# buctcurry/ICKA

Hardware: AMD Instinct MI355X
Metric: MNER samples/sec (fwd+bwd) at seq=128, 36 regions, bs=32 per GPU (higher is better)
Workload: dtype bf16; 1 GPU; c2: bert(H768,L12,h12,I3072)+36x2048 regions, seq_len 128, per-GPU batch 32, 1 cross layer(s), gated head, 13 labels, train mode p=0.1, token-CE loss; global_batch=32, seq_len=128, regions=36, parallelism=dp1, launch=hipgraph, precision=bf16, accumulate=1

## Files before the change

### icka_amd/_lib.py

```python
from __future__ import annotations

import ctypes as C
import os
from typing import Optional

_HERE = os.path.dirname(os.path.abspath(__file__))
LIB_PATH = os.path.join(_HERE, "libicka_hip.so")

c_vp, c_i32, c_i64, c_u64, c_f32 = C.c_void_p, C.c_int32, C.c_int64, C.c_uint64, C.c_float

ABI_VERSION = 6
GEMM_NT, GEMM_NN, GEMM_TN, GEMM_TT = 0, 1, 2, 3
ATTN_FP8, ATTN_TILED = 1, 2
LSTM_PER_STEP, LSTM_TICKETS, LSTM_NO_BATCH_SPLIT = 1, 2, 4
EPI_NONE, EPI_GELU, EPI_DGELU, EPI_ADD, EPI_GATE, EPI_TANH, EPI_RELU, EPI_ADD_RELU = 0, 1, 2, 3, 4, 5, 6, 7


class GemmDesc(C.Structure):
    _fields_ = [
        ("op", c_i32), ("M", c_i32), ("N", c_i32), ("K", c_i32), ("K1", c_i32),
        ("A", c_vp), ("lda", c_i64), ("B", c_vp), ("ldb", c_i64),
        ("A2", c_vp), ("lda2", c_i64), ("B2", c_vp), ("ldb2", c_i64),
        ("C", c_vp), ("ldc", c_i64), ("c_is_f32", c_i32),
        ("C2", c_vp), ("ldc2", c_i64),
        ("aux", c_vp), ("ldaux", c_i64),
        ("bias", c_vp), ("bias2", c_vp),
        ("alpha", c_f32), ("beta", c_f32),
        ("epilogue", c_i32),
        ("colsum_out", c_vp), ("colsum_accumulate", c_i32),
        ("ab_f16", c_i32), ("C3", c_vp), ("ldc3", c_i64), ("aux_f16", c_i32), ("c3_only", c_i32),
        ("tune", c_u64),
    ]


class SlabReduction(C.Structure):
    _fields_ = [("partials", c_vp), ("slab_stride", c_i64), ("nslab", c_i32), ("H", c_i32), ("nslots", c_i32),
                ("accumulate", c_i32), ("out", c_vp * 4)]


class XGemmDesc(C.Structure):
    _fields_ = [
        ("op", c_i32), ("M", c_i32), ("N", c_i32), ("K", c_i32),
        ("A", c_vp), ("lda", c_i64), ("a_bs0", c_i64), ("a_bs1", c_i64),
        ("B", c_vp), ("ldb", c_i64), ("b_bs0", c_i64), ("b_bs1", c_i64),
        ("C", c_vp), ("ldc", c_i64), ("c_bs0", c_i64), ("c_bs1", c_i64),
        ("nb0", c_i32), ("nb1", c_i32),
        ("bias", c_vp),
        ("alpha", c_f32), ("beta", c_f32),
    ]


PROTOTYPES = {
    "icka_abi_version": (c_i32, []),
    "icka_copy_many": (c_i32, [c_vp, c_vp, c_vp, c_i32, c_vp]),
    "icka_build_arch": (C.c_char_p, []),
    "icka_gemm": (c_i32, [C.POINTER(GemmDesc), c_vp]),
    "icka_gemm_grouped": (c_i32, [C.POINTER(GemmDesc), c_i32, c_vp]),
    "icka_gemm_grouped_ex": (c_i32, [C.POINTER(GemmDesc), c_i32, C.POINTER(SlabReduction), c_i32, c_vp]),
    "icka_gemm_ln": (c_i32, [C.POINTER(GemmDesc), c_vp, c_vp, c_i64, c_i32, c_vp, c_vp, c_vp, c_i64, c_vp, c_i32, c_vp, c_vp, c_f32,
                             c_f32, c_u64, c_vp, c_vp, c_vp]),
    "icka_gemm_qkv_attn": (c_i32, [C.POINTER(GemmDesc), c_vp, c_vp, c_vp, c_i64, c_vp, c_i32, c_i32, c_i32, c_f32, c_f32, c_u64, c_vp, c_vp]),
    "icka_gemm_ln_sync_words": (c_i64, []),
    "icka_gemm_ln_test_hooks": (c_i32, [c_i32, c_i32]),
    "icka_ln_fwd": (c_i32, [c_vp, c_i64, c_i32, c_vp, c_vp, c_i64, c_i32, c_vp, c_vp, c_vp, c_i64, c_vp, c_i64,
                            c_vp, c_vp, c_vp, c_i32, c_i32, c_f32, c_f32, c_u64, c_vp]),
    "icka_ln_fwd_h": (c_i32, [c_vp, c_i64, c_i32, c_vp, c_vp, c_i64, c_i32, c_vp, c_vp, c_vp, c_i64, c_vp, c_i64,
                            c_vp, c_vp, c_vp, c_i32, c_i32, c_f32, c_f32, c_u64, c_vp]),
    "icka_ln_bwd_workspace_floats": (c_i64, [c_i32]),
    "icka_ln_bwd": (c_i32, [c_vp, c_i64, c_vp, c_i64, c_vp, c_vp, c_vp, c_vp, c_i64, c_vp, c_i64, c_vp, c_vp, c_vp,
                            c_vp, c_i32, c_i32, c_f32, c_u64, c_i32, c_vp]),
    "icka_ln_bwd_slabs": (c_i32, [c_vp, c_i64, c_vp, c_i64, c_vp, c_vp, c_vp, c_vp, c_i64, c_vp, c_i64, c_vp, c_i32,
                                  c_i32, c_f32, c_u64, c_vp]),
    "icka_ln_bwd_nslab": (c_i32, [c_i32]),
    "icka_ln_slab_slots": (c_i32, []),
    "icka_embed_fwd": (c_i32, [c_vp, c_vp, c_vp, c_vp, c_vp, c_vp, c_vp, c_vp, c_vp, c_vp, c_vp, c_i32, c_i32,
                               c_i32, c_i32, c_i32, c_f32, c_f32, c_u64, c_vp]),
    "icka_embed_fwd_h": (c_i32, [c_vp, c_vp, c_vp, c_vp, c_vp, c_vp, c_vp, c_vp, c_vp, c_vp, c_vp, c_i32, c_i32,
                               c_i32, c_i32, c_i32, c_f32, c_f32, c_u64, c_vp]),
    "icka_embed_bwd": (c_i32, [c_vp, c_vp, c_vp, c_vp, c_vp, c_vp, c_vp, c_vp, c_vp, c_vp, c_vp, c_vp, c_i32, c_i32,
                               c_i32, c_i32, c_i32, c_i32, c_f32, c_u64, c_i32, c_vp]),
    "icka_embed_bwd_rows": (c_i32, [c_vp, c_vp, c_vp, c_vp, c_vp, c_vp, c_vp, c_vp, c_vp, c_vp, c_vp, c_vp, c_i32, c_i32,
                                    c_i32, c_i32, c_i32, c_i32, c_f32, c_u64, c_i32, c_vp]),
    "icka_embed_scatter_rows": (c_i32, [c_vp, c_i32, c_vp, c_vp, c_i64, c_i32, c_i32, c_i32, c_f32, c_vp]),
    "icka_attn_fwd": (c_i32, [c_vp, c_i64, c_vp, c_i64, c_vp, c_i64, c_vp, c_vp, c_i64, c_vp, c_i32, c_i32, c_i32,
                              c_i32, c_f32, c_f32, c_u64, c_vp]),
    "icka_attn_fwd_ex": (c_i32, [c_vp, c_i64, c_vp, c_i64, c_vp, c_i64, c_vp, c_vp, c_vp, c_i64, c_vp, c_i32, c_i32, c_i32,
                                 c_i32, c_f32, c_f32, c_u64, c_i32, c_vp, c_vp]),
    "icka_attn_keepbits_words": (c_i64, [c_i32, c_i32, c_i32, c_i32]),
    "icka_attn_fwd_fp8": (c_i32, [c_vp, c_i64, c_vp, c_i64, c_vp, c_i64, c_vp, c_vp, c_i64, c_vp, c_i32, c_i32, c_i32,
                              c_i32, c_f32, c_f32, c_u64, c_vp]),
    "icka_cls_head_fwd": (c_i32, [c_vp, c_vp, c_vp, c_vp, c_vp, c_i32, c_i32, c_i32, c_vp]),
    "icka_cls_head_fwd_h": (c_i32, [c_vp, c_vp, c_vp, c_vp, c_vp, c_i32, c_i32, c_i32, c_vp]),
    "icka_cls_head_bwd": (c_i32, [c_vp, c_i64, c_vp, c_vp, c_vp, c_vp, c_vp, c_vp, c_vp, c_vp, c_vp, c_i32, c_i32, c_i32,
                                  c_vp]),
    "icka_cls_head_bwd_slabs": (c_i32, [c_i32]),
    "icka_cls_head_slab_floats": (c_i64, [c_i32, c_i32]),
    "icka_conv_stem_patches": (c_i32, [c_vp, c_vp, c_i32, c_i32, c_i32, c_i64, c_vp]),
    "icka_conv_im2col3x3": (c_i32, [c_vp, c_vp, c_i32, c_i32, c_i32, c_i32, c_i32, c_i64, c_vp]),
    "icka_conv3x3_gemm": (c_i32, [c_vp, c_vp, c_vp, c_vp, c_i64, c_vp, c_i32, c_i32, c_i32, c_i32, c_i32, c_i32, c_i64, c_i32,
                                   c_vp, c_vp]),
    "icka_conv_subsample": (c_i32, [c_vp, c_vp, c_i32, c_i32, c_i32, c_i32, c_i32, c_i64, c_vp]),
    "icka_conv_maxpool3x3s2": (c_i32, [c_vp, c_vp, c_i32, c_i32, c_i32, c_i32, c_i64, c_vp]),
    "icka_conv_features_out": (c_i32, [c_vp, c_vp, c_vp, c_vp, c_i32, c_i32, c_i32, c_vp]),
    "icka_gemm_bn_stats": (c_i32, [c_vp, c_i64, c_vp, c_i64, c_vp, c_i64, c_i32, c_i32, c_i32, c_i64, c_vp, c_vp]),
    "icka_conv3x3_gemm_stats": (c_i32, [c_vp, c_vp, c_vp, c_i32, c_i32, c_i32, c_i32, c_i32, c_i32, c_i64, c_vp, c_vp, c_vp]),
    "icka_bn_finalize": (c_i32, [c_vp, c_i32, c_i32, c_vp, c_vp, c_vp, c_vp, c_vp, c_f32, c_f32, c_vp, c_vp, c_vp]),
    "icka_bn_apply": (c_i32, [c_vp, c_vp, c_vp, c_vp, c_vp, c_vp, c_vp, c_i32, c_i64, c_i64, c_i32, c_vp, c_vp, c_vp]),
    "icka_lstm_fwd": (c_i32, [c_vp, c_i64, c_vp, c_vp, c_vp, c_vp, c_vp, c_i32, c_i32, c_i32, c_i32, c_vp]),
    "icka_lstm_bwd": (c_i32, [c_vp, c_vp, c_vp, c_vp, c_vp, c_i64, c_vp, c_i32, c_i32, c_i32, c_i32, c_vp]),
    "icka_lstm_barrier_error": (c_i32, []),
    "icka_lstm_clear_error": (c_i32, []),
    "icka_lstm_set_reserved_cus": (c_i32, [c_i32]),
    "icka_lstm_test_hooks": (c_i32, [c_i32, c_i32]),
    "icka_linear_small_m": (c_i32, [c_vp, c_i64, c_vp, c_vp, c_vp, c_i64, c_i32, c_i32, c_i32, c_i32, c_vp]),
    "icka_transpose_bf16": (c_i32, [c_vp, c_vp, c_i32, c_i32, c_i32, c_vp]),
    "icka_crf_llh": (c_i32, [c_vp, c_i64, c_vp, c_vp, c_vp, c_vp, c_vp, c_vp, c_i32, c_i32, c_i32, c_vp]),
    "icka_crf_grad": (c_i32, [c_vp, c_i64, c_vp, c_vp, c_vp, c_vp, c_vp, c_vp, c_vp, c_i64, c_vp, c_vp, c_vp, c_i32,
                              c_i32, c_i32, c_vp]),
    "icka_crf_decode": (c_i32, [c_vp, c_i64, c_vp, c_vp, c_vp, c_vp, c_vp, c_vp, c_i32, c_i32, c_i32, c_vp]),
    "icka_crf_score_decode": (c_i32, [c_vp, c_i64, c_vp, c_vp, c_vp, c_vp, c_vp, c_vp, c_vp, c_vp, c_i64, c_i32, c_i32, c_i32,
                                      c_vp]),
    "icka_attn_bwd": (c_i32, [c_vp, c_i64, c_vp, c_i64, c_vp, c_i64, c_vp, c_vp, c_i64, c_vp, c_i64, c_vp, c_vp,
                              c_vp, c_i64, c_vp, c_i64, c_vp, c_i64, c_i32, c_i32, c_i32, c_i32, c_f32, c_f32, c_u64,
                              c_vp, c_i32, c_vp]),
    "icka_cast_f32_to_bf16": (c_i32, [c_vp, c_vp, c_i64, c_vp]),
    "icka_cast_to_f16": (c_i32, [c_vp, c_i32, c_vp, c_i64, c_vp]),
    "icka_cast_f32_to_bf16_f16": (c_i32, [c_vp, c_vp, c_vp, c_i64, c_vp]),
    "icka_cast_bf16_to_f32": (c_i32, [c_vp, c_vp, c_i64, c_vp]),
    "icka_cast_pad_f32_to_bf16": (c_i32, [c_vp, c_i64, c_vp, c_i64, c_i32, c_i32, c_vp]),
    "icka_additive_mask": (c_i32, [c_vp, c_i64, c_vp, c_i32, c_i32, c_vp]),
    "icka_dropout": (c_i32, [c_vp, c_i64, c_vp, c_i64, c_vp, c_i64, c_i32, c_i32, c_f32, c_u64, c_vp]),
    "icka_regions_to_tokens": (c_i32, [c_vp, c_vp, c_i32, c_i32, c_i32, c_i32, c_vp]),
    "icka_regions_to_tokens_h": (c_i32, [c_vp, c_vp, c_vp, c_i32, c_i32, c_i32, c_i32, c_vp]),
    "icka_sample_gate_fwd_h": (c_i32, [c_vp, c_i64, c_vp, c_i32, c_vp, c_vp, c_i64, c_i32, c_i32, c_i32, c_vp]),
    "icka_colsum": (c_i32, [c_vp, c_i64, c_vp, c_vp, c_i32, c_i32, c_i32, c_vp]),
    "icka_colsum_workspace_floats": (c_i64, [c_i32]),
    "icka_gate_bwd": (c_i32, [c_vp, c_i64, c_vp, c_vp, c_i64, c_vp, c_i64, c_vp, c_vp, c_i64, c_i32, c_i32, c_vp]),
    "icka_sample_gate_fwd": (c_i32, [c_vp, c_i64, c_vp, c_i64, c_vp, c_i32, c_vp, c_i64, c_i32, c_i32, c_i32, c_vp]),
    "icka_sample_gate_bwd": (c_i32, [c_vp, c_i64, c_vp, c_i64, c_vp, c_i64, c_vp, c_i32, c_vp, c_i64, c_vp, c_i64, c_vp,
                                     c_i32, c_i32, c_i32, c_vp]),
    "icka_crs_fwd": (c_i32, [c_vp, c_i64, c_vp, c_i64, c_vp, c_vp, c_vp, c_i32, c_i32, c_i32, c_vp]),
    "icka_crs_bwd": (c_i32, [c_vp, c_vp, c_i64, c_vp, c_i64, c_vp, c_vp, c_vp, c_vp, c_vp, c_i32, c_i32, c_i32, c_i32,
                             c_vp]),
    "icka_add_bf16": (c_i32, [c_vp, c_vp, c_vp, c_i64, c_vp]),
    "icka_tanh_bwd": (c_i32, [c_vp, c_vp, c_vp, c_i64, c_vp]),
    "icka_contrastive_workspace_floats": (c_i64, [c_i32]),
    "icka_contrastive_fwd": (c_i32, [c_vp, c_i64, c_vp, c_i64, c_i32, c_i32, c_i32, c_f32, c_f32, c_vp, c_i32, c_vp, c_vp, c_vp]),
    "icka_contrastive_bwd": (c_i32, [c_vp, c_i64, c_vp, c_i64, c_i32, c_i32, c_i32, c_f32, c_f32, c_vp, c_vp, c_vp, c_vp, c_vp,
                                     c_vp, c_i32, c_vp, c_vp]),
    "icka_relu_bwd": (c_i32, [c_vp, c_vp, c_vp, c_i64, c_i32, c_vp]),
    "icka_sample_swap": (c_i32, [c_vp, c_vp, c_i32, c_i64, c_i32, c_vp]),
    "icka_dgelu_bf16": (c_i32, [c_vp, c_vp, c_vp, c_i64, c_vp]),
    "icka_embed_prompt_fwd": (c_i32, [c_vp, c_vp, c_vp, c_vp, c_vp, c_vp, c_vp, c_vp, c_vp, c_vp, c_vp, c_vp, c_i32, c_i32,
                                      c_i32, c_i32, c_i32, c_i32, c_i32, c_f32, c_f32, c_u64, c_vp]),
    "icka_embed_prompt_bwd": (c_i32, [c_vp, c_vp, c_vp, c_vp, c_vp, c_vp, c_vp, c_vp, c_vp, c_vp, c_vp, c_vp, c_vp, c_i32,
                                      c_i32, c_i32, c_i32, c_i32, c_i32, c_i32, c_i32, c_f32, c_u64, c_i32, c_vp]),
    "icka_token_ce": (c_i32, [c_vp, c_i64, c_vp, c_vp, c_vp, c_vp, c_vp, c_i64, c_i32, c_i32, c_vp]),
    "icka_token_ce_workspace_floats": (c_i64, [c_i32]),
    "icka_token_ce_fused": (c_i32, [c_vp, c_i64, c_vp, c_vp, c_vp, c_vp, c_vp, c_i64, c_i32, c_i32, c_i32, c_vp]),
    "icka_zero_f32": (c_i32, [c_vp, c_i64, c_vp]),
    "icka_scale_by_ratio": (c_i32, [c_vp, c_vp, c_vp, c_vp, c_i64, c_vp]),
    "icka_scalar_ratio": (c_i32, [c_vp, c_vp, c_vp, c_vp]),
    "icka_set_dropout_nonce": (c_i32, [c_vp]),
    "icka_bump_dropout_nonce": (c_i32, [c_vp, c_vp]),
    "icka_dropout_mask": (c_i32, [c_vp, c_i64, c_f32, c_u64, c_vp]),
    "icka_attn_dropout_mask": (c_i32, [c_vp, c_i64, c_i32, c_f32, c_u64, c_vp]),
    "icka_pack_plan": (c_i32, [c_vp, c_i32, c_i32, c_i32, c_vp, c_vp, c_vp, c_vp, c_vp, c_vp, c_vp, c_vp]),
    "icka_rows_gather": (c_i32, [c_vp, c_i64, c_i64, c_vp, c_i64, c_i64, c_i32, c_vp, c_i64, C.c_uint32, c_vp]),
    "icka_attn_fwd_packed": (c_i32, [c_vp, c_i64, c_vp, c_i64, c_vp, c_i64, c_vp, c_vp, c_i64, c_vp, c_vp, c_i32, c_i64, c_i32,
                                     c_i32, c_i32, c_i32, c_f32, c_f32, c_u64, c_vp, c_vp]),
    "icka_attn_bwd_packed": (c_i32, [c_vp, c_i64, c_vp, c_i64, c_vp, c_i64, c_vp, c_vp, c_i64, c_vp, c_vp, c_vp, c_i64, c_vp,
                                     c_i64, c_vp, c_i64, c_vp, c_i32, c_i64, c_i32, c_i32, c_i32, c_i32, c_f32, c_f32, c_u64,
                                     c_vp, c_vp]),
    "icka_dp_chunk_elems": (c_i64, []),
    "icka_dp_cast_chunks": (c_i32, [c_vp, c_vp, c_vp, c_i32, c_vp]),
    "icka_dp_cast_back_scaled": (c_i32, [c_vp, c_vp, c_i64, c_f32, c_vp]),
    "icka_dp_init": (c_i32, []),
    "icka_dp_error": (c_i32, []),
    "icka_dp_clear_error": (c_i32, []),
    "icka_dp_step_bump": (c_i32, [c_vp, c_vp]),
    "icka_dp_flag_set": (c_i32, [c_vp, c_vp, c_vp]),
    "icka_dp_flag_wait": (c_i32, [c_vp, C.c_uint32, c_vp, c_i32, c_vp]),
    "icka_dp_poison_if": (c_i32, [c_vp, C.c_uint32, c_vp, c_i32, c_i32, c_vp]),
    "icka_dp_poison_final": (c_i32, [c_vp, c_i32, C.c_uint32, c_vp, c_vp, c_i32, c_vp]),
    "icka_optim_chunk_elems": (c_i64, []),
    "icka_optim_sqnorm": (c_i32, [c_vp, c_vp, c_i32, c_vp, c_vp]),
    "icka_optim_clip": (c_i32, [c_vp, c_i32, c_f32, c_vp, c_vp]),
    "icka_optim_adamw": (c_i32, [c_vp, c_vp, c_vp, c_vp, c_vp, c_vp, c_vp, c_i32, c_vp, c_f32, c_f32, c_f32, c_f32, c_f32,
                                 c_i32, c_vp]),
    "icka_x_gemm": (c_i32, [C.POINTER(XGemmDesc), c_vp]),
    "icka_x_ln_fwd": (c_i32, [c_vp, c_i64, c_vp, c_i64, c_vp, c_vp, c_vp, c_vp, c_vp, c_i32, c_i32, c_f32, c_f32, c_u64,
                              c_vp]),
    "icka_x_ln_bwd": (c_i32, [c_vp, c_i64, c_vp, c_vp, c_vp, c_vp, c_vp, c_i32, c_i32, c_f32, c_u64, c_vp]),
    "icka_x_colsum": (c_i32, [c_vp, c_i64, c_vp, c_i64, c_vp, c_i32, c_i32, c_i32, c_vp]),
    "icka_x_embed_fwd": (c_i32, [c_vp, c_vp, c_vp, c_vp, c_vp, c_vp, c_vp, c_vp, c_vp, c_vp, c_i32, c_i32, c_i32, c_f32,
                                 c_vp]),
    "icka_x_embed_scatter": (c_i32, [c_vp, c_vp, c_vp, c_vp, c_vp, c_vp, c_i32, c_i32, c_i32, c_i32, c_vp]),
    "icka_x_softmax_fwd": (c_i32, [c_vp, c_vp, c_vp, c_i32, c_i32, c_i32, c_i32, c_f32, c_f32, c_u64, c_vp]),
    "icka_x_softmax_bwd": (c_i32, [c_vp, c_vp, c_i32, c_i32, c_i32, c_i32, c_f32, c_f32, c_u64, c_vp]),
    "icka_x_act_fwd": (c_i32, [c_vp, c_vp, c_vp, c_vp, c_i64, c_i32, c_vp]),
    "icka_x_act_bwd": (c_i32, [c_vp, c_vp, c_vp, c_vp, c_vp, c_i64, c_i32, c_vp]),
    "icka_x_dropout": (c_i32, [c_vp, c_vp, c_i64, c_f32, c_u64, c_vp]),
    "icka_x_add": (c_i32, [c_vp, c_i64, c_vp, c_i64, c_vp, c_i64, c_i32, c_i32, c_vp]),
    "icka_x_concat2": (c_i32, [c_vp, c_i64, c_i32, c_vp, c_i64, c_i32, c_vp, c_i32, c_vp]),
    "icka_x_regions_to_tokens": (c_i32, [c_vp, c_vp, c_i32, c_i32, c_i32, c_i32, c_vp]),
    "icka_x_sample_gate_fwd": (c_i32, [c_vp, c_i64, c_vp, c_i64, c_vp, c_i32, c_vp, c_i64, c_i32, c_i32, c_i32, c_vp]),
    "icka_x_sample_gate_bwd": (c_i32, [c_vp, c_i64, c_vp, c_i64, c_vp, c_i64, c_vp, c_i32, c_vp, c_i64, c_vp, c_i64, c_vp,
                                       c_i32, c_i32, c_i32, c_vp]),
    "icka_x_lstm_cell_fwd": (c_i32, [c_vp, c_vp, c_vp, c_vp, c_i32, c_i32, c_i32, c_i32, c_vp]),
    "icka_x_lstm_cell_bwd": (c_i32, [c_vp, c_vp, c_vp, c_vp, c_vp, c_i32, c_i32, c_i32, c_i32, c_i32, c_vp]),
    "icka_x_embed_prompt_fwd": (c_i32, [c_vp, c_vp, c_vp, c_vp, c_vp, c_vp, c_vp, c_vp, c_vp, c_vp, c_vp, c_i32, c_i32, c_i32,
                                        c_i32, c_i32, c_i32, c_f32, c_vp]),
    "icka_x_embed_prompt_scatter": (c_i32, [c_vp, c_vp, c_vp, c_vp, c_vp, c_vp, c_vp, c_i32, c_i32, c_i32, c_i32, c_i32, c_i32,
                                            c_i32, c_vp]),
# ... 40 lines not shown
```

### icka_amd/csrc/elementwise.hip

```cpp
#include <math.h>

#include "common.h"

namespace {

inline bool al16(const void* p) { return (reinterpret_cast<uintptr_t>(p) & 15) == 0; }
inline int grid_for(int64_t n, int per_block = 256, int cap = 4096) {
    int64_t g = (n + per_block - 1) / per_block;
    return (int)(g < 1 ? 1 : (g > cap ? cap : g));
}

__device__ __forceinline__ void ld8(const bf16_t* p, float (&o)[8]) {
    const bf16x8 v = as_bf16x8(*reinterpret_cast<const u32x4*>(p));
#pragma unroll
    for (int e = 0; e < 8; ++e) o[e] = bf2f(v[e]);
}
__device__ __forceinline__ void st8(bf16_t* p, const float (&v)[8]) {
    bf16x8 o;
#pragma unroll
    for (int e = 0; e < 8; ++e) o[e] = f2bf(v[e]);
    *reinterpret_cast<u32x4*>(p) = as_u32x4(o);
}

__global__ void cast_f2b_kernel(const float* __restrict__ src, bf16_t* __restrict__ dst, int64_t n) {
    const int64_t nch = n >> 3;
    for (int64_t c = (int64_t)blockIdx.x * blockDim.x + threadIdx.x; c < nch; c += (int64_t)gridDim.x * blockDim.x) {
        const f32x4 a = *reinterpret_cast<const f32x4*>(src + c * 8), b = *reinterpret_cast<const f32x4*>(src + c * 8 + 4);
        bf16x8 o = {f2bf(a[0]), f2bf(a[1]), f2bf(a[2]), f2bf(a[3]), f2bf(b[0]), f2bf(b[1]), f2bf(b[2]), f2bf(b[3])};
        *reinterpret_cast<u32x4*>(dst + c * 8) = as_u32x4(o);
    }
    if (blockIdx.x == 0 && threadIdx.x < (n & 7)) dst[(nch << 3) + threadIdx.x] = f2bf(src[(nch << 3) + threadIdx.x]);
}
__global__ void cast_f2bh_kernel(const float* __restrict__ src, bf16_t* __restrict__ dst, _Float16* __restrict__ dsth, int64_t n) {
    const int64_t nch = n >> 3;
    for (int64_t c = (int64_t)blockIdx.x * blockDim.x + threadIdx.x; c < nch; c += (int64_t)gridDim.x * blockDim.x) {
        const f32x4 a = *reinterpret_cast<const f32x4*>(src + c * 8), b = *reinterpret_cast<const f32x4*>(src + c * 8 + 4);
        bf16x8 o = {f2bf(a[0]), f2bf(a[1]), f2bf(a[2]), f2bf(a[3]), f2bf(b[0]), f2bf(b[1]), f2bf(b[2]), f2bf(b[3])};
        *reinterpret_cast<u32x4*>(dst + c * 8) = as_u32x4(o);
        f16x8 h;
#pragma unroll
        for (int e = 0; e < 4; ++e) {
            h[e] = (_Float16)fminf(fmaxf(a[e], -65504.f), 65504.f);
            h[4 + e] = (_Float16)fminf(fmaxf(b[e], -65504.f), 65504.f);
        }
        *reinterpret_cast<u32x4*>(dsth + c * 8) = __builtin_bit_cast(u32x4, h);
    }
    if (blockIdx.x == 0 && threadIdx.x < (n & 7)) {
        const float v = src[(nch << 3) + threadIdx.x];
        dst[(nch << 3) + threadIdx.x] = f2bf(v);
        dsth[(nch << 3) + threadIdx.x] = (_Float16)fminf(fmaxf(v, -65504.f), 65504.f);
    }
}
__global__ void cast_to_f16_kernel(const void* __restrict__ src, int kind, _Float16* __restrict__ dst, int64_t n) {
    for (int64_t i = (int64_t)blockIdx.x * blockDim.x + threadIdx.x; i < n; i += (int64_t)gridDim.x * blockDim.x) {
        const float v = kind ? reinterpret_cast<const float*>(src)[i] : bf2f(reinterpret_cast<const bf16_t*>(src)[i]);
        dst[i] = (_Float16)fminf(fmaxf(v, -65504.f), 65504.f);
    }
}
__global__ void cast_b2f_vec_kernel(const bf16_t* __restrict__ src, float* __restrict__ dst, int64_t n) {
    const int64_t nch = n >> 3;
    for (int64_t c = (int64_t)blockIdx.x * blockDim.x + threadIdx.x; c < nch; c += (int64_t)gridDim.x * blockDim.x) {
        const bf16x8 v = as_bf16x8(*reinterpret_cast<const u32x4*>(src + c * 8));
        *reinterpret_cast<f32x4*>(dst + c * 8) = f32x4{bf2f(v[0]), bf2f(v[1]), bf2f(v[2]), bf2f(v[3])};
        *reinterpret_cast<f32x4*>(dst + c * 8 + 4) = f32x4{bf2f(v[4]), bf2f(v[5]), bf2f(v[6]), bf2f(v[7])};
    }
    if (blockIdx.x == 0 && threadIdx.x < (n & 7)) dst[(nch << 3) + threadIdx.x] = bf2f(src[(nch << 3) + threadIdx.x]);
}
__global__ void cast_b2f_kernel(const bf16_t* __restrict__ src, float* __restrict__ dst, int64_t n) {
    for (int64_t i = (int64_t)blockIdx.x * blockDim.x + threadIdx.x; i < n; i += (int64_t)gridDim.x * blockDim.x)
        dst[i] = bf2f(src[i]);
}

__global__ void cast_pad_kernel(const float* __restrict__ src, int64_t lds, bf16_t* __restrict__ dst, int64_t ldd, int M,
                                int N) {
    const int64_t total = (int64_t)M * ldd;
    for (int64_t i = (int64_t)blockIdx.x * blockDim.x + threadIdx.x; i < total; i += (int64_t)gridDim.x * blockDim.x) {
        const int64_t r = i / ldd;
        const int c = (int)(i - r * ldd);
        dst[i] = f2bf(c < N ? src[r * lds + c] : 0.f);
    }
}

__global__ void additive_mask_kernel(const int64_t* __restrict__ mask, int64_t ld, float* __restrict__ out, int B, int T) {
    const int i = blockIdx.x * blockDim.x + threadIdx.x;
    if (i >= B * T) return;
    const int b = i / T, t = i - b * T;
    out[i] = (1.0f - (float)mask[(int64_t)b * ld + t]) * -10000.0f;
}

__global__ void dropout_kernel(const bf16_t* __restrict__ x, int64_t ldx, bf16_t* __restrict__ y, int64_t ldy,
                               bf16_t* __restrict__ y2, int64_t ldy2, int M, int H, DropCfg d_) {
    const DropCfg d = drop_resolve(d_);
    const int cpr = H >> 3;
    const int64_t total = (int64_t)M * cpr;
    for (int64_t i = (int64_t)blockIdx.x * blockDim.x + threadIdx.x; i < total; i += (int64_t)gridDim.x * blockDim.x) {
        const int64_t row = i / cpr;
        const int c = (int)(i - row * cpr);
        float v[8];
        ld8(x + row * ldx + c * 8, v);
        const uint32_t base = (uint32_t)row * (uint32_t)H + c * 8;
#pragma unroll
        for (int e = 0; e < 8; ++e) v[e] *= drop_mul(d, base + e);
        st8(y + row * ldy + c * 8, v);
        if (y2) st8(y2 + row * ldy2 + c * 8, v);
    }
}

__global__ void dropout_mask_kernel(float* out, int64_t n, DropCfg d_) {
    const DropCfg d = drop_resolve(d_);
    for (int64_t i = (int64_t)blockIdx.x * blockDim.x + threadIdx.x; i < n; i += (int64_t)gridDim.x * blockDim.x)
        out[i] = drop_mul(d, (uint32_t)i);
}

__global__ void attn_dropout_mask_kernel(float* out, int64_t rows, int Skv, DropCfg d_) {
    const DropCfg d = drop_resolve(d_);
    const int64_t n = rows * Skv;
    for (int64_t i = (int64_t)blockIdx.x * blockDim.x + threadIdx.x; i < n; i += (int64_t)gridDim.x * blockDim.x) {
        const int64_t row = i / Skv;
        out[i] = d.thr ? drop_mul_key(d, (uint32_t)row * (uint32_t)Skv, (uint32_t)(i - row * Skv)) : d.scale;
    }
}

__global__ __launch_bounds__(256) void regions_t_kernel(const float* __restrict__ src, bf16_t* __restrict__ dst, int B,
                                                        int R, int C, _Float16* __restrict__ dsth = nullptr) {
    extern __shared__ float tile[];
    const int strips = (C + 63) / 64;
    const int b = blockIdx.x / strips, c0 = (blockIdx.x % strips) * 64;
    const int nc = (C - c0) < 64 ? (C - c0) : 64;
    const float* s = src + ((int64_t)b * C + c0) * R;
    for (int i = threadIdx.x; i < nc * R; i += 256) {
        const int c = i / R, r = i - c * R;
        tile[c * (R + 1) + r] = s[i];
    }
    __syncthreads();
    for (int i = threadIdx.x; i < R * 64; i += 256) {
        const int r = i >> 6, c = i & 63;
        if (c < nc) {
            const float v = tile[c * (R + 1) + r];
            dst[((int64_t)b * R + r) * C + c0 + c] = f2bf(v);
            if (dsth) dsth[((int64_t)b * R + r) * C + c0 + c] = (_Float16)fminf(fmaxf(v, -65504.f), 65504.f);
        }
    }
}

constexpr int CS_GROUPS = 256;
__global__ __launch_bounds__(256) void colsum_kernel(const bf16_t* __restrict__ x, int64_t ldx, float* __restrict__ partial,
                                                     int M, int N, int rows_per_group, int vec) {
    __shared__ float red[4][64][8];
    const int cx = threadIdx.x & 63, ry = threadIdx.x >> 6;
    const int col = (blockIdx.x * 64 + cx) * 8;
    const int r0 = blockIdx.y * rows_per_group;
    int r1 = r0 + rows_per_group; r1 = r1 > M ? M : r1;
    float acc[8] = {0.f, 0.f, 0.f, 0.f, 0.f, 0.f, 0.f, 0.f};
    if (col < N) {
        const int nv = (N - col) < 8 ? (N - col) : 8;
        for (int r = r0 + ry; r < r1; r += 4) {
            const bf16_t* p = x + (int64_t)r * ldx + col;
            if (nv == 8 && vec) {
                float v[8];
                ld8(p, v);
#pragma unroll
                for (int e = 0; e < 8; ++e) acc[e] += v[e];
            } else {
                for (int e = 0; e < nv; ++e) acc[e] += bf2f(p[e]);
            }
        }
    }
#pragma unroll
    for (int e = 0; e < 8; ++e) red[ry][cx][e] = acc[e];
    __syncthreads();
    if (ry == 0 && col < N) {
        for (int e = 0; e < 8 && col + e < N; ++e)
            partial[(int64_t)blockIdx.y * N + col + e] = red[0][cx][e] + red[1][cx][e] + red[2][cx][e] + red[3][cx][e];
    }
}
__global__ __launch_bounds__(1024) void colsum_finalize_kernel(const float* __restrict__ partial, float* __restrict__ out,
                                                               int groups, int N, int accumulate) {
    __shared__ float red[16][64];
    const int cx = threadIdx.x & 63, sy = threadIdx.x >> 6;
    const int c = blockIdx.x * 64 + cx;
    float s = 0.f;
    if (c < N)
        for (int g = sy; g < groups; g += 16) s += partial[(int64_t)g * N + c];
    red[sy][cx] = s;
    __syncthreads();
    if (sy == 0 && c < N) {
        float t = 0.f;
// ... 211 lines not shown

extern "C" int icka_copy_many(const void* const* src, void* const* dst, const int64_t* bytes, int32_t n, void* stream) {
    if (n < 0 || n > COPY_MAX || (n > 0 && (!src || !dst || !bytes))) return ICKA_E_ARG;
    if (n == 0) return 0;
    CopyMany t{};
    long long most = 0;
    for (int i = 0; i < n; ++i) {
        if (bytes[i] < 0 || (bytes[i] > 0 && (!src[i] || !dst[i]))) return ICKA_E_ARG;
        t.src[i] = (const char*)src[i];
        t.dst[i] = (char*)dst[i];
        t.bytes[i] = bytes[i];
        most = bytes[i] > most ? bytes[i] : most;
    }
    long long blocks = (most / 16 + 256 * 4 - 1) / (256 * 4);
    blocks = blocks < 1 ? 1 : (blocks > 2048 ? 2048 : blocks);
    hipLaunchKernelGGL(copy_many_kernel, dim3((unsigned)blocks, (unsigned)n), dim3(256), 0, (hipStream_t)stream, t);
    ICKA_CHECK_LAUNCH();
    return 0;
}

extern "C" int icka_cast_f32_to_bf16(const float* src, void* dst, int64_t n, void* stream) {
    if (!src || !dst) return ICKA_E_ARG;
    if (n <= 0) return 0;
    if (!al16(src) || !al16(dst)) return ICKA_E_ALIGN;
    hipLaunchKernelGGL(cast_f2b_kernel, dim3(grid_for((n + 7) / 8, 256, 8192)), dim3(256), 0, (hipStream_t)stream, src,
                       (bf16_t*)dst, n);
    ICKA_CHECK_LAUNCH();
    return 0;
}
extern "C" int icka_cast_f32_to_bf16_f16(const float* src, void* dst_bf16, void* dst_f16, int64_t n, void* stream) {
    if (!src || !dst_bf16 || !dst_f16) return ICKA_E_ARG;
    if (n <= 0) return 0;
    if (!al16(src) || !al16(dst_bf16) || !al16(dst_f16)) return ICKA_E_ALIGN;
    hipLaunchKernelGGL(cast_f2bh_kernel, dim3(grid_for((n + 7) / 8, 256, 8192)), dim3(256), 0, (hipStream_t)stream, src,
                       (bf16_t*)dst_bf16, (_Float16*)dst_f16, n);
    ICKA_CHECK_LAUNCH();
    return 0;
}
extern "C" int icka_cast_to_f16(const void* src, int32_t src_is_f32, void* dst, int64_t n, void* stream) {
    if (!src || !dst) return ICKA_E_ARG;
    if (n <= 0) return 0;
    hipLaunchKernelGGL(cast_to_f16_kernel, dim3(grid_for(n)), dim3(256), 0, (hipStream_t)stream, src, (int)src_is_f32,
                       (_Float16*)dst, n);
    ICKA_CHECK_LAUNCH();
    return 0;
}
extern "C" int icka_cast_bf16_to_f32(const void* src, float* dst, int64_t n, void* stream) {
    if (!src || !dst) return ICKA_E_ARG;
    if (n <= 0) return 0;
    if (al16(src) && al16(dst))
        hipLaunchKernelGGL(cast_b2f_vec_kernel, dim3(grid_for((n + 7) / 8, 256, 8192)), dim3(256), 0, (hipStream_t)stream,
                           (const bf16_t*)src, dst, n);
    else
        hipLaunchKernelGGL(cast_b2f_kernel, dim3(grid_for(n)), dim3(256), 0, (hipStream_t)stream, (const bf16_t*)src, dst, n);
    ICKA_CHECK_LAUNCH();
    return 0;
}
extern "C" int icka_cast_pad_f32_to_bf16(const float* src, int64_t lds, void* dst, int64_t ldd, int32_t M, int32_t N,
                                         void* stream) {
    if (!src || !dst) return ICKA_E_ARG;
    if (M <= 0 || N <= 0 || ldd < N || lds < N) return ICKA_E_SHAPE;
    hipLaunchKernelGGL(cast_pad_kernel, dim3(grid_for((int64_t)M * ldd)), dim3(256), 0, (hipStream_t)stream, src, lds,
                       (bf16_t*)dst, ldd, M, N);
    ICKA_CHECK_LAUNCH();
    return 0;
}
extern "C" int icka_additive_mask(const int64_t* mask, int64_t ld, float* out, int32_t B, int32_t T, void* stream) {
    if (!mask || !out) return ICKA_E_ARG;
    if (B <= 0 || T <= 0 || ld < T) return ICKA_E_SHAPE;
    hipLaunchKernelGGL(additive_mask_kernel, dim3((B * T + 255) / 256), dim3(256), 0, (hipStream_t)stream, mask, ld, out, B, T);
    ICKA_CHECK_LAUNCH();
    return 0;
}
extern "C" int icka_dropout(const void* x, int64_t ldx, void* y, int64_t ldy, void* y2, int64_t ldy2, int32_t M,
                            int32_t H, float p_drop, uint64_t seed, void* stream) {
    if (!x || !y) return ICKA_E_ARG;
    if (M <= 0 || H <= 0 || H % 8) return ICKA_E_SHAPE;
    if (ldx % 8 || ldy % 8 || (y2 && ldy2 % 8) || !al16(x) || !al16(y) || (y2 && !al16(y2))) return ICKA_E_ALIGN;
    hipLaunchKernelGGL(dropout_kernel, dim3(grid_for((int64_t)M * (H / 8))), dim3(256), 0, (hipStream_t)stream,
                       (const bf16_t*)x, ldx, (bf16_t*)y, ldy, (bf16_t*)y2, ldy2, M, H, make_drop(p_drop, seed));
    ICKA_CHECK_LAUNCH();
    return 0;
}
extern "C" int icka_dropout_mask(float* out, int64_t n, float p_drop, uint64_t seed, void* stream) {
    if (!out) return ICKA_E_ARG;
    if (n <= 0) return 0;
    hipLaunchKernelGGL(dropout_mask_kernel, dim3(grid_for(n)), dim3(256), 0, (hipStream_t)stream, out, n,
                       make_drop(p_drop, seed));
    ICKA_CHECK_LAUNCH();
    return 0;
}
extern "C" int icka_attn_dropout_mask(float* out, int64_t rows, int32_t Skv, float p_drop, uint64_t seed, void* stream) {
    if (!out) return ICKA_E_ARG;
    if (rows <= 0 || Skv <= 0) return 0;
    hipLaunchKernelGGL(attn_dropout_mask_kernel, dim3(grid_for(rows * Skv)), dim3(256), 0, (hipStream_t)stream, out, rows, Skv,
                       make_drop(p_drop, seed));
    ICKA_CHECK_LAUNCH();
    return 0;
}
extern "C" int icka_regions_to_tokens(const float* src, void* dst, int32_t B, int32_t R, int32_t C, int32_t layout,
                                      void* stream) {
    if (!src || !dst) return ICKA_E_ARG;
    if (B <= 0 || R <= 0 || C <= 0 || R > 256) return ICKA_E_SHAPE;
    if (layout == 0) return icka_cast_f32_to_bf16(src, dst, (int64_t)B * R * C, stream);
    if (layout != 1) return ICKA_E_ARG;
    hipLaunchKernelGGL(regions_t_kernel, dim3(B * ((C + 63) / 64)), dim3(256), 64 * (R + 1) * sizeof(float),
                       (hipStream_t)stream, src, (bf16_t*)dst, B, R, C);
    ICKA_CHECK_LAUNCH();
    return 0;
}
extern "C" int icka_regions_to_tokens_h(const float* src, void* dst_bf16, void* dst_f16, int32_t B, int32_t R, int32_t C,
                                        int32_t layout, void* stream) {
    if (!src || !dst_bf16 || !dst_f16) return ICKA_E_ARG;
    if (B <= 0 || R <= 0 || C <= 0 || R > 256) return ICKA_E_SHAPE;
    if (layout == 0) return icka_cast_f32_to_bf16_f16(src, dst_bf16, dst_f16, (int64_t)B * R * C, stream);
    if (layout != 1) return ICKA_E_ARG;
    hipLaunchKernelGGL(regions_t_kernel, dim3(B * ((C + 63) / 64)), dim3(256), 64 * (R + 1) * sizeof(float),
                       (hipStream_t)stream, src, (bf16_t*)dst_bf16, B, R, C, (_Float16*)dst_f16);
    ICKA_CHECK_LAUNCH();
    return 0;
}
extern "C" int64_t icka_colsum_workspace_floats(int32_t N) { return (int64_t)CS_GROUPS * N; }
extern "C" int icka_colsum(const void* x, int64_t ldx, float* out, float* partials, int32_t M, int32_t N,
                           int32_t accumulate, void* stream) {
    if (!x || !out || !partials) return ICKA_E_ARG;
    if (M <= 0 || N <= 0) return ICKA_E_SHAPE;
    const int vec = (ldx % 8 == 0) && al16(x);
    int groups = (M + 15) / 16; groups = groups > CS_GROUPS ? CS_GROUPS : groups;
    const int rpg = (M + groups - 1) / groups;
    hipStream_t st = (hipStream_t)stream;
    hipLaunchKernelGGL(colsum_kernel, dim3((N + 511) / 512, groups), dim3(256), 0, st, (const bf16_t*)x, ldx, partials, M,
                       N, rpg, vec);
    ICKA_CHECK_LAUNCH();
    hipLaunchKernelGGL(colsum_finalize_kernel, dim3((N + 63) / 64), dim3(1024), 0, st, partials, out, groups, N, accumulate);
    ICKA_CHECK_LAUNCH();
    return 0;
}
extern "C" int icka_gate_bwd(const void* dout, int64_t lddout, const void* g, const void* cross, int64_t ldcross,
                             const void* dcross_in, int64_t lddci, void* du, void* dcross, int64_t lddc, int32_t M,
                             int32_t H, void* stream) {
    if (!dout || !g || !cross || !du || !dcross) return ICKA_E_ARG;
    if (M <= 0 || H <= 0 || H % 8) return ICKA_E_SHAPE;
    if (lddout % 8 || ldcross % 8 || lddc % 8 || (dcross_in && lddci % 8)) return ICKA_E_ALIGN;
    if (!al16(dout) || !al16(g) || !al16(cross) || !al16(du) || !al16(dcross) || (dcross_in && !al16(dcross_in)))
        return ICKA_E_ALIGN;
    hipLaunchKernelGGL(gate_bwd_kernel, dim3(grid_for((int64_t)M * (H / 8))), dim3(256), 0, (hipStream_t)stream,
                       (const bf16_t*)dout, lddout, (const bf16_t*)g, (const bf16_t*)cross, ldcross,
                       (const bf16_t*)dcross_in, lddci, (bf16_t*)du, (bf16_t*)dcross, lddc, M, H);
    ICKA_CHECK_LAUNCH();
    return 0;
}
extern "C" int icka_add_bf16(const void* a, const void* b, void* c, int64_t n, void* stream) {
    if (!a || !b || !c) return ICKA_E_ARG;
    if (n <= 0) return 0;
    if (!al16(a) || !al16(b) || !al16(c)) return ICKA_E_ALIGN;
    hipLaunchKernelGGL(add_kernel, dim3(grid_for((n + 7) / 8)), dim3(256), 0, (hipStream_t)stream, (const bf16_t*)a,
                       (const bf16_t*)b, (bf16_t*)c, n);
    ICKA_CHECK_LAUNCH();
    return 0;
}
extern "C" int icka_dgelu_bf16(const void* dg, const void* z, void* dz, int64_t n, void* stream) {
    if (!dg || !z || !dz) return ICKA_E_ARG;
    if (n <= 0) return 0;
    if (!al16(dg) || !al16(z) || !al16(dz)) return ICKA_E_ALIGN;
    hipLaunchKernelGGL(dgelu_kernel, dim3(grid_for((n + 7) / 8)), dim3(256), 0, (hipStream_t)stream, (const bf16_t*)dg,
                       (const bf16_t*)z, (bf16_t*)dz, n);
// ... 60 lines not shown
```

### icka_amd/csrc/fusion.hip

```cpp
#include <math.h>

#include "common.h"

namespace {

__device__ __forceinline__ void ld8(const bf16_t* p, float (&o)[8]) {
    const bf16x8 v = as_bf16x8(*reinterpret_cast<const u32x4*>(p));
#pragma unroll
    for (int e = 0; e < 8; ++e) o[e] = bf2f(v[e]);
}
__device__ __forceinline__ void st8(bf16_t* p, const float (&v)[8]) {
    bf16x8 o;
#pragma unroll
    for (int e = 0; e < 8; ++e) o[e] = f2bf(v[e]);
    *reinterpret_cast<u32x4*>(p) = as_u32x4(o);
}
__device__ __forceinline__ float block_sum(float v, float* red) {
    v = wave_sum(v);
    const int w = threadIdx.x >> 6;
    if ((threadIdx.x & 63) == 0) red[w] = v;
    __syncthreads();
    float t = 0.f;
    for (int i = 0; i < (int)(blockDim.x >> 6); ++i) t += red[i];
    __syncthreads();
// ... 201 lines not shown
extern "C" int icka_sample_gate_fwd(const void* a, int64_t lda, const void* c, int64_t ldc, const float* gate,
                                    int32_t mode, void* out, int64_t ldo, int32_t B, int32_t S, int32_t H,
                                    void* stream) {
    if (!a || !gate || !out || (mode != 0 && mode != 1)) return ICKA_E_ARG;
    if (B <= 0 || S <= 0 || H <= 0 || H % 8) return ICKA_E_SHAPE;
    if (!ok16(a, lda) || !ok16(out, ldo) || (c && !ok16(c, ldc))) return ICKA_E_ALIGN;
    hipLaunchKernelGGL(gate_fwd_kernel, dim3(SPLIT, B), dim3(256), 0, (hipStream_t)stream, (const bf16_t*)a, lda,
                       (const bf16_t*)c, ldc, gate, mode, (bf16_t*)out, ldo, S, H);
    ICKA_CHECK_LAUNCH();
    return 0;
}

extern "C" int icka_sample_gate_fwd_h(const void* a16, int64_t lda, const float* gate, int32_t mode, void* out, void* out16,
                                      int64_t ldo, int32_t B, int32_t S, int32_t H, void* stream) {
    if (!a16 || !gate || !out || !out16) return ICKA_E_ARG;
    if (B <= 0 || S <= 0 || H <= 0 || H % 8 != 0 || (mode != 0 && mode != 1)) return ICKA_E_SHAPE;
    if (!ok16(a16, lda) || !ok16(out, ldo) || !ok16(out16, ldo)) return ICKA_E_ALIGN;
    hipLaunchKernelGGL(gate_fwd_h_kernel, dim3(SPLIT, B), dim3(256), 0, (hipStream_t)stream, (const _Float16*)a16, lda, gate,
                       mode, (bf16_t*)out, (_Float16*)out16, ldo, S, H);
    ICKA_CHECK_LAUNCH();
    return 0;
}
extern "C" int icka_sample_gate_bwd(const void* dout, int64_t lddo, const void* a, int64_t lda, const void* c,
                                    int64_t ldc, const float* gate, int32_t mode, void* da, int64_t ldda, void* dc,
                                    int64_t lddc, float* dgate, int32_t B, int32_t S, int32_t H, void* stream) {
    if (!dout || !a || !gate || !da || !dgate || (mode != 0 && mode != 1)) return ICKA_E_ARG;
    if (B <= 0 || S <= 0 || H <= 0 || H % 8) return ICKA_E_SHAPE;
    if (!ok16(dout, lddo) || !ok16(a, lda) || !ok16(da, ldda) || (c && !ok16(c, ldc)) || (dc && !ok16(dc, lddc)))
        return ICKA_E_ALIGN;
    hipLaunchKernelGGL(gate_bwd_kernel, dim3(SPLIT, B), dim3(256), 0, (hipStream_t)stream, (const bf16_t*)dout, lddo,
                       (const bf16_t*)a, lda, (const bf16_t*)c, ldc, gate, mode, (bf16_t*)da, ldda, (bf16_t*)dc, lddc,
                       dgate, S, H);
    ICKA_CHECK_LAUNCH();
    return 0;
}

extern "C" int icka_crs_fwd(const void* seq, int64_t lds, const void* cross, int64_t ldc, const void* W,
                            const float* bias, float* crs, int32_t B, int32_t S, int32_t H, void* stream) {
    if (!seq || !cross || !W || !crs) return ICKA_E_ARG;
    if (B <= 0 || S <= 0 || H <= 0 || H % 8) return ICKA_E_SHAPE;
    if (!ok16(seq, lds) || !ok16(cross, ldc) || !ok16(W, 8)) return ICKA_E_ALIGN;
    hipLaunchKernelGGL(crs_fwd_kernel, dim3(SPLIT, B), dim3(256), 0, (hipStream_t)stream, (const bf16_t*)seq, lds,
                       (const bf16_t*)cross, ldc, (const bf16_t*)W, bias, crs, S, H);
    ICKA_CHECK_LAUNCH();
    return 0;
}

extern "C" int icka_crs_bwd(const float* dcrs, const void* seq, int64_t lds, const void* cross, int64_t ldc,
                            const void* W, void* dseq, void* dcross, float* dW, float* dbias, int32_t B, int32_t S,
                            int32_t H, int32_t accumulate, void* stream) {
    if (!dcrs || !seq || !cross || !W || !dseq || !dcross || !dW) return ICKA_E_ARG;
    if (B <= 0 || S <= 0 || H <= 0 || H % 8) return ICKA_E_SHAPE;
    if (!ok16(seq, lds) || !ok16(cross, ldc) || !ok16(W, 8) || !ok16(dseq, 8) || !ok16(dcross, 8)) return ICKA_E_ALIGN;
    hipStream_t st = (hipStream_t)stream;
    const int64_t n1 = (int64_t)B * S * (H / 8);
    hipLaunchKernelGGL(crs_dgrad_kernel, dim3((unsigned)((n1 + 255) / 256 > 2048 ? 2048 : (n1 + 255) / 256)), dim3(256),
                       0, st, dcrs, (const bf16_t*)W, (bf16_t*)dseq, (bf16_t*)dcross, B, S, H);
    ICKA_CHECK_LAUNCH();
    const int64_t n2 = (int64_t)S * (H / 8) * 2;
    hipLaunchKernelGGL(crs_wgrad_kernel, dim3((unsigned)((n2 + 255) / 256)), dim3(256), 0, st, dcrs,
                       (const bf16_t*)seq, lds, (const bf16_t*)cross, ldc, dW, dbias, B, S, H, accumulate);
    ICKA_CHECK_LAUNCH();
    return 0;
}


namespace {

constexpr int CLS_TB = 16;
constexpr int CLS_MAXC = 16;

__device__ __forceinline__ void cls_ld8(const bf16_t* p, float (&o)[8]) {
    const bf16x8 v = as_bf16x8(*reinterpret_cast<const u32x4*>(p));
#pragma unroll
    for (int e = 0; e < 8; ++e) o[e] = bf2f(v[e]);
}
__device__ __forceinline__ void cls_st8(bf16_t* p, const float (&v)[8]) {
    bf16x8 o;
#pragma unroll
    for (int e = 0; e < 8; ++e) o[e] = f2bf(v[e]);
    *reinterpret_cast<u32x4*>(p) = as_u32x4(o);
}

template <bool F16>
__global__ __launch_bounds__(256) void cls_head_fwd_kernel(const bf16_t* __restrict__ seq, const bf16_t* __restrict__ gated,
                                                           const bf16_t* __restrict__ W, const float* __restrict__ bias,
                                                           float* __restrict__ logits, int M, int H, int C) {
    extern __shared__ __attribute__((aligned(16))) char cls_smem[];
    __shared__ float s_red[4][CLS_MAXC][65];
    bf16_t* sW = reinterpret_cast<bf16_t*>(cls_smem);
    const int tid = threadIdx.x, lane = tid & 63, wave = tid >> 6;
    const int nch = (2 * H) >> 3, hch = H >> 3;
    for (int i = tid; i < C * nch; i += 256)
        *reinterpret_cast<u32x4*>(sW + (int64_t)i * 8) = *reinterpret_cast<const u32x4*>(W + (int64_t)i * 8);
    __syncthreads();
    const int nw = gridDim.x * 4;
    for (int row0 = (blockIdx.x * 4 + wave) * 2; row0 < M; row0 += 2 * nw) {
        u32x4 xr[2][4];
#pragma unroll
        for (int r = 0; r < 2; ++r)
#pragma unroll
            for (int i = 0; i < 4; ++i) {
                const int j = lane + 64 * i, row = row0 + r;
                xr[r][i] = u32x4{0u, 0u, 0u, 0u};
                if (j < nch && row < M)
                    xr[r][i] = *reinterpret_cast<const u32x4*>(j < hch ? seq + (int64_t)row * H + j * 8
                                                                       : gated + (int64_t)row * H + (j - hch) * 8);
            }
        float acc[2][CLS_MAXC];
#pragma unroll
        for (int r = 0; r < 2; ++r)
#pragma unroll
            for (int c = 0; c < CLS_MAXC; ++c) acc[r][c] = 0.f;
#pragma unroll
        for (int i = 0; i < 4; ++i) {
            const int j = lane + 64 * i;
            if (j < nch) {
#pragma unroll
                for (int c = 0; c < CLS_MAXC; ++c) {
                    if (c < C) {
                        float w[8];
                        if constexpr (F16) {
                            const f16x8 wv = __builtin_bit_cast(f16x8, *reinterpret_cast<const u32x4*>(sW + (int64_t)c * 2 * H + j * 8));
#pragma unroll
                            for (int e = 0; e < 8; ++e) w[e] = (float)wv[e];
                        } else {
                            cls_ld8(sW + (int64_t)c * 2 * H + j * 8, w);
                        }
#pragma unroll
                        for (int r = 0; r < 2; ++r) {
                            if constexpr (F16) {
                                const f16x8 xv = __builtin_bit_cast(f16x8, xr[r][i]);
#pragma unroll
                                for (int e = 0; e < 8; ++e) acc[r][c] += (float)xv[e] * w[e];
                            } else {
                                const bf16x8 xv = as_bf16x8(xr[r][i]);
#pragma unroll
                                for (int e = 0; e < 8; ++e) acc[r][c] += bf2f(xv[e]) * w[e];
                            }
                        }
                    }
                }
            }
        }
#pragma unroll
        for (int r = 0; r < 2; ++r) {
#pragma unroll
            for (int c = 0; c < CLS_MAXC; ++c) s_red[wave][c][lane] = acc[r][c];
            __builtin_amdgcn_wave_barrier();
            const int c = lane >> 2, qd = lane & 3;
            float v = 0.f;
#pragma unroll
            for (int i = 0; i < 16; ++i) v += s_red[wave][c][16 * qd + i];
            v += __shfl_xor(v, 1, 64);
            v += __shfl_xor(v, 2, 64);
            if (qd == 0 && c < C && row0 + r < M)
                logits[(int64_t)(row0 + r) * C + c] = v + (bias ? bias[c] : 0.f);
            __builtin_amdgcn_wave_barrier();
        }
    }
}

template <int CC>
__global__ __launch_bounds__(256) void cls_head_bwd_kernel(const bf16_t* __restrict__ dl, int64_t ldd,
                                                           const bf16_t* __restrict__ seq, const bf16_t* __restrict__ gated,
                                                           const bf16_t* __restrict__ gate, const bf16_t* __restrict__ cross,
                                                           const bf16_t* __restrict__ W, bf16_t* __restrict__ dseq,
                                                           bf16_t* __restrict__ du, bf16_t* __restrict__ dcross,
                                                           float* __restrict__ partials, int M, int H, int C) {
    __shared__ float s_dl[CLS_TB][CLS_MAXC];
    const int tid = threadIdx.x;
    const int nch = (2 * H) >> 3, hch = H >> 3;
    const int t0 = blockIdx.x * CLS_TB;
    const int nt = M - t0 < CLS_TB ? M - t0 : CLS_TB;
    for (int i = tid; i < CLS_TB * CLS_MAXC; i += 256) {
        const int t = i / CLS_MAXC, c = i % CLS_MAXC;
        s_dl[t][c] = (t < nt && c < C) ? bf2f(dl[(int64_t)(t0 + t) * ldd + c]) : 0.f;
    }
    __syncthreads();
    const int64_t slab = (int64_t)C * 2 * H + CLS_MAXC;
    float* myslab = partials + (int64_t)blockIdx.x * slab;
    if (tid < CLS_MAXC) {
        float s = 0.f;
        for (int t = 0; t < nt; ++t) s += s_dl[t][tid];
        myslab[(int64_t)C * 2 * H + tid] = s;
    }
    const int j = tid;
    if (j >= nch) return;
    const bool second = j >= hch;
    const int h = (second ? j - hch : j) * 8;
    float Wr[CC][8], dW[CC][8];
#pragma unroll
    for (int c = 0; c < CC; ++c) {
        if (c < C) cls_ld8(W + (int64_t)c * 2 * H + j * 8, Wr[c]);
#pragma unroll
        for (int e = 0; e < 8; ++e) { dW[c][e] = 0.f; if (c >= C) Wr[c][e] = 0.f; }
    }
    for (int tb = 0; tb < nt; tb += 4) {
        u32x4 xr[4], gr[4], cr4[4];
#pragma unroll
        for (int u = 0; u < 4; ++u) {
            const int64_t row = t0 + (tb + u < nt ? tb + u : nt - 1);
            xr[u] = *reinterpret_cast<const u32x4*>((second ? gated : seq) + row * H + h);
            if (second) {
                gr[u] = *reinterpret_cast<const u32x4*>(gate + row * H + h);
                cr4[u] = *reinterpret_cast<const u32x4*>(cross + row * H + h);
            }
        }
#pragma unroll
        for (int u = 0; u < 4; ++u) {
            const int t = tb + u;
            if (t >= nt) break;
            const int64_t row = t0 + t;
            const bf16x8 xv = as_bf16x8(xr[u]);
            float x[8], dx[8];
#pragma unroll
            for (int e = 0; e < 8; ++e) { x[e] = bf2f(xv[e]); dx[e] = 0.f; }
#pragma unroll
            for (int c = 0; c < CC; ++c) {
                const float d = s_dl[t][c];
#pragma unroll
                for (int e = 0; e < 8; ++e) { dx[e] += d * Wr[c][e]; dW[c][e] += d * x[e]; }
            }
            if (!second) {
                cls_st8(dseq + row * H + h, dx);
            } else {
                const bf16x8 gv = as_bf16x8(gr[u]), cv = as_bf16x8(cr4[u]);
                float uu[8], dc[8];
#pragma unroll
                for (int e = 0; e < 8; ++e) {
                    const float g = bf2f(gv[e]);
                    uu[e] = dx[e] * bf2f(cv[e]) * g * (1.f - g);
                    dc[e] = dx[e] * g;
                }
                cls_st8(du + row * H + h, uu);
                cls_st8(dcross + row * H + h, dc);
            }
        }
    }
#pragma unroll
    for (int c = 0; c < CC; ++c)
        if (c < C) {
            float* p = myslab + (int64_t)c * 2 * H + j * 8;
            *reinterpret_cast<f32x4*>(p) = f32x4{dW[c][0], dW[c][1], dW[c][2], dW[c][3]};
            *reinterpret_cast<f32x4*>(p + 4) = f32x4{dW[c][4], dW[c][5], dW[c][6], dW[c][7]};
        }
}

}

extern "C" int32_t icka_cls_head_bwd_slabs(int32_t M) { return (M + CLS_TB - 1) / CLS_TB; }
extern "C" int64_t icka_cls_head_slab_floats(int32_t H, int32_t C) { return (int64_t)C * 2 * H + CLS_MAXC; }

static int cls_head_fwd_impl(bool f16, const void* seq, const void* gated, const void* W, const float* bias, float* logits,
                             int32_t M, int32_t H, int32_t C, void* stream) {
    if (!seq || !gated || !W || !logits) return ICKA_E_ARG;
    if (M <= 0 || H <= 0 || H % 8 || C <= 0 || C > CLS_MAXC || (int64_t)C * 2 * H * 2 > 44 * 1024) return ICKA_E_SHAPE;
    if ((reinterpret_cast<uintptr_t>(seq) | reinterpret_cast<uintptr_t>(gated) | reinterpret_cast<uintptr_t>(W)) & 15)
        return ICKA_E_ALIGN;
    int grid = (M + 7) / 8;
    grid = grid > 512 ? 512 : grid;
    if (f16)
        hipLaunchKernelGGL(cls_head_fwd_kernel<true>, dim3(grid), dim3(256), (size_t)C * 2 * H * 2, (hipStream_t)stream,
                           (const bf16_t*)seq, (const bf16_t*)gated, (const bf16_t*)W, bias, logits, M, H, C);
    else
        hipLaunchKernelGGL(cls_head_fwd_kernel<false>, dim3(grid), dim3(256), (size_t)C * 2 * H * 2, (hipStream_t)stream,
                           (const bf16_t*)seq, (const bf16_t*)gated, (const bf16_t*)W, bias, logits, M, H, C);
    ICKA_CHECK_LAUNCH();
    return 0;
}
extern "C" int icka_cls_head_fwd(const void* seq, const void* gated, const void* W, const float* bias, float* logits,
                                 int32_t M, int32_t H, int32_t C, void* stream) {
    return cls_head_fwd_impl(false, seq, gated, W, bias, logits, M, H, C, stream);
}
extern "C" int icka_cls_head_fwd_h(const void* seq, const void* gated, const void* W, const float* bias, float* logits,
                                   int32_t M, int32_t H, int32_t C, void* stream) {
    return cls_head_fwd_impl(true, seq, gated, W, bias, logits, M, H, C, stream);
}

extern "C" int icka_cls_head_bwd(const void* dl, int64_t ldd, const void* seq, const void* gated, const void* gate,
                                 const void* cross, const void* W, void* dseq, void* du, void* dcross, float* partials,
                                 int32_t M, int32_t H, int32_t C, void* stream) {
    if (!dl || !seq || !gated || !gate || !cross || !W || !dseq || !du || !dcross || !partials) return ICKA_E_ARG;
    if (M <= 0 || H <= 0 || H % 8 || C <= 0 || C > CLS_MAXC || 2 * H / 8 > 256 || ldd < C) return ICKA_E_SHAPE;
    const uintptr_t al = reinterpret_cast<uintptr_t>(seq) | reinterpret_cast<uintptr_t>(gated) |
                         reinterpret_cast<uintptr_t>(gate) | reinterpret_cast<uintptr_t>(cross) |
                         reinterpret_cast<uintptr_t>(W) | reinterpret_cast<uintptr_t>(dseq) |
                         reinterpret_cast<uintptr_t>(du) | reinterpret_cast<uintptr_t>(dcross) |
                         reinterpret_cast<uintptr_t>(partials);
    if (al & 15) return ICKA_E_ALIGN;
    const int grid = icka_cls_head_bwd_slabs(M);
    if (C <= 13)
        hipLaunchKernelGGL((cls_head_bwd_kernel<13>), dim3(grid), dim3(256), 0, (hipStream_t)stream,
                           (const bf16_t*)dl, ldd, (const bf16_t*)seq, (const bf16_t*)gated, (const bf16_t*)gate,
                           (const bf16_t*)cross, (const bf16_t*)W, (bf16_t*)dseq, (bf16_t*)du, (bf16_t*)dcross,
                           partials, M, H, C);
    else
        hipLaunchKernelGGL((cls_head_bwd_kernel<CLS_MAXC>), dim3(grid), dim3(256), 0, (hipStream_t)stream,
                           (const bf16_t*)dl, ldd, (const bf16_t*)seq, (const bf16_t*)gated, (const bf16_t*)gate,
                           (const bf16_t*)cross, (const bf16_t*)W, (bf16_t*)dseq, (bf16_t*)du, (bf16_t*)dcross,
                           partials, M, H, C);
    ICKA_CHECK_LAUNCH();
    return 0;
}
```

### icka_amd/csrc/gemm.hip

```cpp
#include "common.h"
#include "ln_row.h"
#include "attn_core.h"
#include <cstdio>
#include <cstdlib>

namespace {

constexpr int BM = 128, BN = 128, BK = 64;
constexpr int TILE_BYTES = 128 * 64 * 2;

struct GemmArgs {
    int M, N, K, K1;
    const bf16_t* A;  int64_t lda;
    const bf16_t* B;  int64_t ldb;
    const bf16_t* A2; int64_t lda2;
    const bf16_t* B2; int64_t ldb2;
    void* C;  int64_t ldc;
    bf16_t* C2; int64_t ldc2;
    const bf16_t* aux; int64_t ldaux;
    const float* bias; const float* bias2;
    float alpha, beta;
    int epi, c_f32;
    int a_vec, b_vec;
    int abl;
// ... 1511 lines not shown
    return best;
}

template <bool A_KM, bool B_KM, bool F16 = false>
int launch(GemmArgs g, bool aligned, hipStream_t st, const Tune& t) {
    const int nb = ((g.M + BM - 1) / BM) * ((g.N + BN - 1) / BN);
    if constexpr (!A_KM && !B_KM) {
        if (!aligned && g.n64ok && t.ws) {
            hipLaunchKernelGGL((gemm_ws_kernel<false, false, 3, 0, 64, F16>), dim3((g.M / BM) * (g.N / 64)), dim3(512), 0, st, g);
            ICKA_CHECK_LAUNCH();
            return 0;
        }
    }
    if (aligned) {
#ifdef ICKA_GEMM_ABLATE
        if (t.abl == 1 && !t.ws) hipLaunchKernelGGL((gemm_dma_kernel<A_KM, B_KM, 3, 1>), dim3(nb), dim3(256), 0, st, g);
        else if (t.abl == 2 && !t.ws) hipLaunchKernelGGL((gemm_dma_kernel<A_KM, B_KM, 3, 2>), dim3(nb), dim3(256), 0, st, g);
        else
#endif
        {
            if (t.ws || F16) {
#ifdef ICKA_GEMM_ABLATE
                if (t.bn == 96 && g.n96ok) {
                    const int nb96 = (g.M / BM) * (g.N / 96);
                    if (t.abl == 1) { hipLaunchKernelGGL((gemm_ws_kernel<A_KM, B_KM, 3, 1, 96>), dim3(nb96), dim3(512), 0, st, g); ICKA_CHECK_LAUNCH(); return 0; }
                    if (t.abl == 2) { hipLaunchKernelGGL((gemm_ws_kernel<A_KM, B_KM, 3, 2, 96>), dim3(nb96), dim3(512), 0, st, g); ICKA_CHECK_LAUNCH(); return 0; }
                    if (t.abl == 3) { hipLaunchKernelGGL((gemm_ws_kernel<A_KM, B_KM, 3, 3, 96>), dim3(nb96), dim3(512), 0, st, g); ICKA_CHECK_LAUNCH(); return 0; }
                }
                if (t.abl == 1) { hipLaunchKernelGGL((gemm_ws_kernel<A_KM, B_KM, 3, 1>), dim3(nb), dim3(512), 0, st, g); ICKA_CHECK_LAUNCH(); return 0; }
                if (t.abl == 2) { hipLaunchKernelGGL((gemm_ws_kernel<A_KM, B_KM, 3, 2>), dim3(nb), dim3(512), 0, st, g); ICKA_CHECK_LAUNCH(); return 0; }
#endif
                if constexpr (!A_KM) {
                    const int nb3 = (g.M / 256) * (g.N / 192);
                    const int rounds3 = (nb3 + 255) / 256;
                    if (t.w3 && g.M % 256 == 0 && g.N % 192 == 0 && g.K <= 1024 && g.K1 == 0 && nb3 % 8 == 0 &&
                        nb3 >= 128 && 4 * nb3 >= 3 * 256 * rounds3 && g.ksplit == 1) {
                        { const int pm = gemm_w3_grid(g.M, g.N, 192, t.w3grid), pn = 8 / pm;
                          g.w3_sn = (g.N / 192) / pn; g.w3_pnlog = pn == 1 ? 0 : (pn == 2 ? 1 : (pn == 4 ? 2 : 3)); }
                        hipLaunchKernelGGL((gemm_w3_kernel<B_KM, F16>), dim3(nb3), dim3(768), 0, st, g);
                        ICKA_CHECK_LAUNCH();
                        return 0;
                    }
                    const int nb2 = (g.M / 256) * (g.N / 128);
                    if (t.w3 && g.M % 256 == 0 && g.K1 == 0 && g.ksplit == 1 && nb2 % 8 == 0 && nb2 >= 192 && nb2 <= 256 &&
                        !(g.n96ok && t.bn == 96) && !(g.K <= 1024 && g.direct && g.c_f32 && g.epi == ICKA_EPI_NONE && g.beta == 0.f)) {
                        { const int pm = gemm_w3_grid(g.M, g.N, 128, t.w3grid), pn = 8 / pm;
                          g.w3_sn = (g.N / 128) / pn; g.w3_pnlog = pn == 1 ? 0 : (pn == 2 ? 1 : (pn == 4 ? 2 : 3)); }
                        hipLaunchKernelGGL((gemm_w3_kernel<B_KM, F16, 128>), dim3(nb2), dim3(768), 0, st, g);
                        ICKA_CHECK_LAUNCH();
                        return 0;
                    }
                }
                if (g.n96ok && t.bn != 128) {
                    const int nb96 = (g.M / BM) * (g.N / 96);
                    if (t.bn == 96 || (nb < 256 && nb96 <= 256 && nb96 > nb)) {
                        if ((t.ws == 2 || (t.ws == 1 && nb96 >= 448 && g.K <= 1024)) && !A_KM)
                            hipLaunchKernelGGL((gemm_ws2_kernel<A_KM, B_KM, 96, F16>), dim3(nb96), dim3(512), 0, st, g);
                        else if (t.nbuf == 4 && !F16)
                            hipLaunchKernelGGL((gemm_ws_kernel<A_KM, B_KM, 4, 0, 96>), dim3(nb96), dim3(512), 0, st, g);
                        else if (t.nbuf == 5 && !F16)
                            hipLaunchKernelGGL((gemm_ws_kernel<A_KM, B_KM, 5, 0, 96>), dim3(nb96), dim3(512), 0, st, g);
                        else
                            hipLaunchKernelGGL((gemm_ws_kernel<A_KM, B_KM, 3, 0, 96, F16>), dim3(nb96), dim3(512), 0, st, g);
                        ICKA_CHECK_LAUNCH();
                        return 0;
                    }
                }
                if ((t.ws == 2 || (t.ws == 1 && nb >= 448 && g.K <= 1024)) && !A_KM)
                    hipLaunchKernelGGL((gemm_ws2_kernel<A_KM, B_KM, 128, F16>), dim3(nb), dim3(512), 0, st, g);
                else if (t.nbuf == 4 && !F16) hipLaunchKernelGGL((gemm_ws_kernel<A_KM, B_KM, 4>), dim3(nb), dim3(512), 0, st, g);
                else if (t.nbuf == 5 && !F16) hipLaunchKernelGGL((gemm_ws_kernel<A_KM, B_KM, 5>), dim3(nb), dim3(512), 0, st, g);
                else hipLaunchKernelGGL((gemm_ws_kernel<A_KM, B_KM, 3, 0, 128, F16>), dim3(nb), dim3(512), 0, st, g);
                ICKA_CHECK_LAUNCH();
                return 0;
            }
            const int nbuf = t.nbuf > 0 ? t.nbuf : (nb >= 448 ? 2 : 4);
            if (nbuf == 2) hipLaunchKernelGGL((gemm_dma_kernel<A_KM, B_KM, 2, 0>), dim3(nb), dim3(256), 0, st, g);
            else if (nbuf == 3) hipLaunchKernelGGL((gemm_dma_kernel<A_KM, B_KM, 3, 0>), dim3(nb), dim3(256), 0, st, g);
            else hipLaunchKernelGGL((gemm_dma_kernel<A_KM, B_KM, 4, 0>), dim3(nb), dim3(256), 0, st, g);
        }
    } else {
        const int nk = (g.K + BK - 1) / BK;
        int ks = 1;
        if (g.c_f32 && g.epi == ICKA_EPI_NONE && nb < 64 && nk >= 16 && g.M <= 256 && !g.C3) {
            ks = 256 / nb;
            if (ks > nk / 4) ks = nk / 4;
            if (ks < 1) ks = 1;
        }
        if (ks > 1) {
            const int64_t n = (int64_t)g.M * g.N;
            hipLaunchKernelGGL(scale_c_kernel, dim3((unsigned)((n + 255) / 256)), dim3(256), 0, st,
                               reinterpret_cast<float*>(g.C), g.ldc, g.M, g.N, g.beta);
            ICKA_CHECK_LAUNCH();
            g.beta = 0.f;
            g.ksplit = ks;
        }
        hipLaunchKernelGGL((gemm_kernel<A_KM, B_KM, false, F16>), dim3(nb, ks), dim3(256), 0, st, g);
    }
    ICKA_CHECK_LAUNCH();
    return 0;
}

inline bool vec_ok(const void* p, int64_t ld) { return (ld % 8 == 0) && ((reinterpret_cast<uintptr_t>(p) & 15) == 0); }

}

#ifdef ICKA_GEMM_STAMP
extern "C" int icka_diag_gemm_stamp_buffer(void* p) {
    g_stamp = (unsigned long long*)p;
    return 0;
}
#endif

static int site_bit(const icka_gemm_desc* d) {
    const int64_t N = d->N, K = d->K;
    if (d->c_is_f32 == 1 || d->M < 1024) return -1;
    if (d->op == ICKA_GEMM_NT) {
        if (N == 3 * K) return 0;
        if (N == K) return 1;
        if (N == 4 * K) return 2;
        if (K == 4 * N) return 3;
    } else if (d->op == ICKA_GEMM_NN) {
        if (N == 4 * K) return 4;
        if (K == 4 * N) return 5;
        if (N == K) return 6;
        if (K == 3 * N) return 7;
    }
    return -1;
}
static int plain_mask() {
    static int m = -1;
    if (m < 0) {
        const char* e = getenv("ICKA_GEMM_PLAIN_MASK");
        m = e ? (int)strtol(e, nullptr, 0) : 0;
    }
    return m;
}

static int convert(const icka_gemm_desc* d, GemmArgs& g, bool& aligned, Tune& t) {
    if (!d || !d->A || !d->B || !d->C) return ICKA_E_ARG;
    if (!tune_of(d->tune, t)) return ICKA_E_ARG;
    if (d->M <= 0 || d->N <= 0 || d->K <= 0) return ICKA_E_SHAPE;
    if (d->op < ICKA_GEMM_NT || d->op > ICKA_GEMM_TN) return ICKA_E_ARG;
    if (d->K1 != 0 && (d->K1 < 0 || d->K1 >= d->K || d->K1 % BK != 0 || !d->A2 || !d->B2)) return ICKA_E_ARG;
    if ((d->epilogue == ICKA_EPI_GELU) && !d->C2) return ICKA_E_ARG;
    if ((d->epilogue == ICKA_EPI_DGELU || d->epilogue == ICKA_EPI_ADD || d->epilogue == ICKA_EPI_GATE ||
         d->epilogue == ICKA_EPI_ADD_RELU) && !d->aux)
        return ICKA_E_ARG;
    g.M = d->M; g.N = d->N; g.K = d->K; g.K1 = d->K1;
    g.A = (const bf16_t*)d->A; g.lda = d->lda; g.B = (const bf16_t*)d->B; g.ldb = d->ldb;
    g.A2 = (const bf16_t*)d->A2; g.lda2 = d->lda2; g.B2 = (const bf16_t*)d->B2; g.ldb2 = d->ldb2;
    g.C = d->C; g.ldc = d->ldc; g.C2 = (bf16_t*)d->C2; g.ldc2 = d->ldc2;
    g.aux = (const bf16_t*)d->aux; g.ldaux = d->ldaux; g.bias = d->bias; g.bias2 = d->bias2;
    g.alpha = d->alpha; g.beta = d->beta; g.epi = d->epilogue;
    if (d->c_is_f32 < 0 || d->c_is_f32 > 2) return ICKA_E_ARG;
    g.c_f32 = d->c_is_f32 == 1; g.c_f16 = d->c_is_f32 == 2;
    g.f16 = d->ab_f16 != 0; g.C3 = (bf16_t*)d->C3; g.ldc3 = d->ldc3; g.aux_f16 = d->aux_f16 != 0;
    if (g.f16 && d->op != ICKA_GEMM_NT) return ICKA_E_ARG;
    if (g.c_f16 && d->beta != 0.f) return ICKA_E_ARG;
    if (g.C3 && !g.c_f16 && !g.c_f32) return ICKA_E_ARG;
    if (g.C3 && g.c_f32 && d->op != ICKA_GEMM_TN) return ICKA_E_ARG;
    g.c3_only = d->c3_only != 0;
    {
        const int sb = site_bit(d);
        g.plain = (sb >= 0 && ((plain_mask() >> sb) & 1)) ? 1 : 0;
    }
    if (g.c3_only && !(g.C3 && g.c_f32 && d->beta == 0.f && d->epilogue == ICKA_EPI_NONE)) return ICKA_E_ARG;
// ... 768 lines not shown
```

### icka_amd/kernels.py

```python
from __future__ import annotations

import ctypes as C
import math
from typing import Optional

import torch

from . import _lib
from ._lib import (EPI_ADD, EPI_ADD_RELU, EPI_DGELU, EPI_GATE, EPI_GELU, EPI_NONE, EPI_RELU, EPI_TANH, GEMM_NN, GEMM_NT, GEMM_TN,
                   GemmDesc, check)

BF16 = torch.bfloat16
F32 = torch.float32
F16 = torch.float16


_RAW_STREAM = getattr(torch._C, "_cuda_getCurrentRawStream", None)
_CUR_DEVICE = getattr(torch._C, "_cuda_getDevice", None)


def _stream() -> int:
    if _RAW_STREAM is not None and _CUR_DEVICE is not None:
        return _RAW_STREAM(_CUR_DEVICE())
    return torch.cuda.current_stream().cuda_stream
# ... 180 lines not shown
        if tile_n not in (96, 128):
            raise ValueError("tile_n: 96 or 128")
        t |= (1 if tile_n == 96 else 2) << 4
    if wide_tiles is not None:
        t |= (2 if wide_tiles else 1) << 8
    if direct_epilogue is not None:
        t |= (2 if direct_epilogue else 1) << 12
    if warp_specialized is not None:
        if warp_specialized not in (0, 1, 2, 3):
            raise ValueError("warp_specialized: 0 .. 3")
        t |= (warp_specialized + 1) << 16
    if w3_grid is not None:
        if w3_grid not in (1, 2, 4, 8):
            raise ValueError("w3_grid: 1, 2, 4 or 8")
        t |= w3_grid << 20
    if big_tiles is not None:
        if big_tiles not in (0, 1, 2):
            raise ValueError("big_tiles: 0 .. 2")
        t |= (big_tiles + 1) << 24
    if ablation is not None:
        if ablation not in (1, 2, 3):
            raise ValueError("ablation: 1 .. 3 (diagnostic builds)")
        t |= ablation << 28
    return t


def gemm(op: int, A: torch.Tensor, B: torch.Tensor, out: torch.Tensor, **kw) -> torch.Tensor:
    lib = _lib.load()
    d = gemm_desc(op, A, B, out, **kw)
    if _PROF is not None:
        _PROF.append((0, d, 1, [d]))
    check(lib.icka_gemm(C.byref(d), _stream()), "icka_gemm")
    return out


def slab_reduction(partials: torch.Tensor, nslab: int, H: int, outs, accumulate: bool, slab_stride: int = 0,
                   offset: int = 0):
    r = _lib.SlabReduction()
    if slab_stride == 0:
        slab_stride = _lib.load().icka_ln_slab_slots() * H
    r.partials, r.slab_stride, r.nslab, r.H = partials.data_ptr() + 4 * offset, slab_stride, nslab, H
    r.nslots, r.accumulate = len(outs), int(bool(accumulate))
    for i, o in enumerate(outs):
        _dev(o, "reduction output")
        if o.dtype != F32 or o.numel() != H or not o.is_contiguous():
            raise ValueError("reduction outputs must be contiguous f32 with %d elements" % H)
        r.out[i] = o.data_ptr()
    r._keep = (partials,) + tuple(outs)
    return r


def cls_head_fwd(seq, gated, W, bias, logits):
    dt = seq.dtype if seq.dtype == F16 else BF16
    _mat(seq, "seq", dt); _mat(gated, "gated", dt)
    M, H = seq.shape
    Cn = W.shape[0]
    if not (seq.is_contiguous() and gated.is_contiguous() and W.is_contiguous() and logits.is_contiguous()):
        raise ValueError("cls_head_fwd: contiguous operands")
    if W.dtype != dt or tuple(W.shape) != (Cn, 2 * H) or logits.dtype != F32 or tuple(logits.shape) != (M, Cn):
        raise ValueError("cls_head_fwd: W %s [C,2H], logits f32 [M,C]" % dt)
    lib = _lib.load()
    fn = lib.icka_cls_head_fwd_h if dt == F16 else lib.icka_cls_head_fwd
    check(fn(seq.data_ptr(), gated.data_ptr(), W.data_ptr(), _ptr(bias), logits.data_ptr(), M, H, Cn, _stream()),
          "icka_cls_head_fwd")
    return logits


def cls_head_bwd(dl, seq, gated, gate, cross, W, dseq, du, dcross, partials):
    M, H = seq.shape
    Cn = W.shape[0]
    for n, t in (("seq", seq), ("gated", gated), ("gate", gate), ("cross", cross), ("dseq", dseq), ("du", du),
                 ("dcross", dcross)):
        _mat(t, n)
        if not t.is_contiguous() or tuple(t.shape) != (M, H):
            raise ValueError("%s must be contiguous bf16 [M,H]" % n)
    _mat(dl, "dl")
    lib = _lib.load()
    check(lib.icka_cls_head_bwd(dl.data_ptr(), dl.stride(0), seq.data_ptr(), gated.data_ptr(), gate.data_ptr(),
                                cross.data_ptr(), W.data_ptr(), dseq.data_ptr(), du.data_ptr(), dcross.data_ptr(),
                                partials.data_ptr(), M, H, Cn, _stream()), "icka_cls_head_bwd")
    return lib.icka_cls_head_bwd_slabs(M)


def gemm_grouped(descs, reductions=None) -> None:
    reductions = reductions or []
    if not descs and not reductions:
        return
    lib = _lib.load()
    arr = (GemmDesc * max(len(descs), 1))(*descs)
    if _PROF is not None and descs:
        _PROF.append((1, arr, len(descs), list(descs)))
    if not reductions:
        check(lib.icka_gemm_grouped(arr, len(descs), _stream()), "icka_gemm_grouped")
        return
    for i in range(0, len(reductions), 4):
        chunk = reductions[i:i + 4]
        rarr = (_lib.SlabReduction * len(chunk))(*chunk)
        check(lib.icka_gemm_grouped_ex(arr if i == 0 else None, len(descs) if i == 0 else 0, rarr, len(chunk),
                                       _stream()), "icka_gemm_grouped_ex")


def _kind(t: torch.Tensor) -> int:
    return {BF16: 0, F32: 1, F16: 2}[t.dtype]


def ln_fwd(x, bias, residual, gamma, beta, y, *, y2=None, y_f32=None, y_f16=None, xhat=None, rstd=None, eps=1e-12,
           p_drop=0.0, seed=0):
    lib = _lib.load()
    _mat(x, "x", x.dtype if x.dtype in (BF16, F32, F16) else BF16); _mat(y, "y")
    if residual is not None:
        _mat(residual, "residual", residual.dtype if residual.dtype in (BF16, F32, F16) else BF16)
    if y_f32 is not None and y_f16 is not None:
        raise ValueError("one twin copy: y_f32 or y_f16")
    M, H = x.shape
    twin = y_f16 if y_f16 is not None else y_f32
    if twin is not None and (twin.dtype != (F16 if y_f16 is not None else F32) or not twin.is_contiguous()
                             or tuple(twin.shape) != (M, H)):
        raise ValueError("twin output must be contiguous [M,H] f32 (y_f32) / fp16 (y_f16)")
    fn = lib.icka_ln_fwd_h if y_f16 is not None else lib.icka_ln_fwd
    check(fn(x.data_ptr(), x.stride(0), _kind(x), _ptr(bias), _ptr(residual), _ld(residual),
             0 if residual is None else _kind(residual), gamma.data_ptr(), beta.data_ptr(),
             y.data_ptr(), y.stride(0), _ptr(y2), _ld(y2), _ptr(twin), _ptr(xhat), _ptr(rstd),
             M, H, eps, p_drop, seed, _stream()), "icka_ln_fwd")
    return y


class GemmLnHandoffError(RuntimeError):
    """A stripe wait of a fused dense + LayerNorm launch gave up: the rows it finished are NaN."""


_GEMM_LN_ERR = None
_GEMM_LN_ERR_NP = None
_GEMM_LN_ERR_PTR = 0


def _gemm_ln_err_word() -> int:
    global _GEMM_LN_ERR, _GEMM_LN_ERR_NP, _GEMM_LN_ERR_PTR
    if _GEMM_LN_ERR is None:
        _GEMM_LN_ERR = torch.zeros(16, dtype=torch.int32).pin_memory()
        _GEMM_LN_ERR_NP = _GEMM_LN_ERR.numpy()
        _GEMM_LN_ERR_PTR = _GEMM_LN_ERR.data_ptr()
    return _GEMM_LN_ERR_PTR


def gemm_ln_sync(device) -> torch.Tensor:
    return torch.zeros(_lib.load().icka_gemm_ln_sync_words(), dtype=torch.int32, device=device)


def gemm_ln(h, w, o, bias, residual, gamma, beta, y, sync, *, y_f32=None, y_f16=None, xhat=None, rstd=None, eps=1e-12,
            p_drop=0.0, seed=0) -> bool:
    gemm_ln_check_error("detected before the next fused launch")
    lib = _lib.load()
    d = gemm_desc(GEMM_NT, h, w, o)
    _mat(y, "y")
    if residual is not None:
        _mat(residual, "residual", residual.dtype if residual.dtype in (BF16, F32, F16) else BF16)
    twin = y_f16 if y_f16 is not None else y_f32
    M, N = o.shape
    if twin is not None and (twin.dtype != (F16 if y_f16 is not None else F32) or not twin.is_contiguous() or tuple(twin.shape) != (M, N)):
        raise ValueError("twin output must be contiguous [M,N] f32 (y_f32) / fp16 (y_f16)")
    args = (d, _ptr(bias), _ptr(residual), _ld(residual), 0 if residual is None else _kind(residual), gamma.data_ptr(),
            beta.data_ptr(), y.data_ptr(), y.stride(0), _ptr(twin), int(y_f16 is not None), _ptr(xhat), _ptr(rstd), eps,
            p_drop, seed, sync.data_ptr(), _gemm_ln_err_word(), _stream())
    rc = lib.icka_gemm_ln(*args)
    if rc == -1:
        return False
# ... 469 lines not shown


CRF_FLAT_MAX_B = 2048


def crf_score_decode(emissions, tags, mask, start, end, trans, llh, lens, tags_flat):
    B, S, Cn = _crf_check(emissions, start, end, trans)
    _i64(tags, "tags", (B, S)); _i64(mask, "mask", (B, S))
    check_flat_tags(lens, tags_flat, B, S)
    if (tags is None) != (llh is None):
        raise ValueError("crf_score_decode: tags and llh go together")
    if llh is not None:
        _dev(llh, "llh")
        if llh.dtype != F32 or tuple(llh.shape) != (B,) or not llh.is_contiguous():
            raise ValueError("llh must be contiguous f32 [%d]" % B)
    _dev(lens, "lens"); _dev(tags_flat, "tags_flat")
    if B > CRF_FLAT_MAX_B:
        raise ValueError("crf_score_decode: B = %d > %d" % (B, CRF_FLAT_MAX_B))
    check(_lib.load().icka_crf_score_decode(emissions.data_ptr(), Cn, _ptr(tags), _ptr(mask), start.data_ptr(),
                                            end.data_ptr(), trans.data_ptr(), _ptr(llh), lens.data_ptr(),
                                            tags_flat.data_ptr(), tags_flat.numel(), B, S, Cn, _stream()),
          "icka_crf_score_decode")


def check_flat_tags(lens, tags_flat, B, S):
    for n, t in (("lens", lens), ("tags_flat", tags_flat)):
        if t.dtype != torch.int32 or t.dim() != 1 or not t.is_contiguous():
            raise ValueError("%s must be a contiguous 1-D int32 tensor, got %s %s" % (n, t.dtype, tuple(t.shape)))
    if lens.numel() != B:
        raise ValueError("lens holds %d entries for a batch of %d" % (lens.numel(), B))
    if tags_flat.numel() < B * S:
        raise ValueError("tags_flat holds %d tags, a batch of %d x %d needs up to %d" % (tags_flat.numel(), B, S, B * S))


def cast_f32_to_bf16(src: torch.Tensor, dst: torch.Tensor) -> torch.Tensor:
    _dev(src, "src"); _dev(dst, "dst")
    check(_lib.load().icka_cast_f32_to_bf16(src.data_ptr(), dst.data_ptr(), src.numel(), _stream()), "icka_cast")
    return dst


def cast_f32_to_bf16_f16(src: torch.Tensor, dst: torch.Tensor, dsth: torch.Tensor) -> None:
    _dev(src, "src"); _dev(dst, "dst"); _dev(dsth, "dsth")
    if src.dtype != F32 or dst.dtype != BF16 or dsth.dtype != F16 or dst.numel() != src.numel() or dsth.numel() != src.numel():
        raise TypeError("cast_f32_to_bf16_f16: f32 source, bf16 + fp16 destinations of the same length")
    check(_lib.load().icka_cast_f32_to_bf16_f16(src.data_ptr(), dst.data_ptr(), dsth.data_ptr(), src.numel(), _stream()),
          "icka_cast_f32_to_bf16_f16")


def cast_to_f16(src: torch.Tensor, dst: torch.Tensor) -> torch.Tensor:
    _dev(src, "src"); _dev(dst, "dst")
    if src.dtype not in (BF16, F32) or dst.dtype != F16 or not src.is_contiguous() or not dst.is_contiguous() \
            or src.numel() != dst.numel():
        raise TypeError("cast_to_f16: contiguous bf16/f32 source, contiguous fp16 destination of the same size")
    check(_lib.load().icka_cast_to_f16(src.data_ptr(), int(src.dtype == F32), dst.data_ptr(), src.numel(), _stream()),
          "icka_cast_to_f16")
    return dst


def cast_bf16_to_f32(src: torch.Tensor, dst: torch.Tensor) -> torch.Tensor:
    _dev(src, "src"); _dev(dst, "dst")
    check(_lib.load().icka_cast_bf16_to_f32(src.data_ptr(), dst.data_ptr(), src.numel(), _stream()), "icka_cast")
    return dst


def cast_pad_f32_to_bf16(src: torch.Tensor, dst: torch.Tensor) -> torch.Tensor:
    _dev(src, "src"); _dev(dst, "dst")
    if src.dtype != F32 or src.dim() != 2 or src.stride(1) != 1 or dst.dtype != BF16 or not dst.is_contiguous():
        raise TypeError("cast_pad: src f32 [M,N] row-major, dst contiguous bf16 [M,ldd]")
    M, N = src.shape
    check(_lib.load().icka_cast_pad_f32_to_bf16(src.data_ptr(), src.stride(0), dst.data_ptr(), dst.shape[1], M, N,
                                                _stream()), "icka_cast_pad_f32_to_bf16")
    return dst


def additive_mask(mask: torch.Tensor, T: int, out: torch.Tensor) -> torch.Tensor:
    _dev(mask, "mask")
    if mask.dtype != torch.int64 or mask.stride(1) != 1:
        raise TypeError("mask must be int64 row-major")
    check(_lib.load().icka_additive_mask(mask.data_ptr(), mask.stride(0), out.data_ptr(), mask.shape[0], T,
                                         _stream()), "icka_additive_mask")
    return out


def dropout(x, y, *, y2=None, p_drop=0.0, seed=0):
    _mat(x, "x"); _mat(y, "y")
    M, H = x.shape
    check(_lib.load().icka_dropout(x.data_ptr(), x.stride(0), y.data_ptr(), y.stride(0), _ptr(y2), _ld(y2), M, H,
                                   p_drop, seed, _stream()), "icka_dropout")
    return y


def dropout_mask(n: int, p_drop: float, seed: int, device) -> torch.Tensor:
    out = torch.empty(n, dtype=F32, device=device)
    check(_lib.load().icka_dropout_mask(out.data_ptr(), n, p_drop, seed, _stream()), "icka_dropout_mask")
    return out


def attn_dropout_mask(rows: int, Skv: int, p_drop: float, seed: int, device) -> torch.Tensor:
    out = torch.empty(rows, Skv, dtype=F32, device=device)
    check(_lib.load().icka_attn_dropout_mask(out.data_ptr(), rows, Skv, p_drop, seed, _stream()), "icka_attn_dropout_mask")
    return out


def regions_to_tokens(src: torch.Tensor, dst: torch.Tensor, B: int, R: int, Cc: int, layout: int) -> torch.Tensor:
    _dev(src, "src")
    if src.dtype != F32 or not src.is_contiguous():
        raise TypeError("region features must be contiguous f32")
    check(_lib.load().icka_regions_to_tokens(src.data_ptr(), dst.data_ptr(), B, R, Cc, layout, _stream()),
          "icka_regions_to_tokens")
    return dst


def regions_to_tokens_h(src: torch.Tensor, dst: torch.Tensor, dst16: torch.Tensor, B: int, R: int, Cc: int, layout: int) -> None:
    _dev(src, "src"); _dev(dst, "dst"); _dev(dst16, "dst16")
    if src.dtype != F32 or not src.is_contiguous() or dst.dtype != BF16 or dst16.dtype != F16:
        raise TypeError("regions_to_tokens_h: contiguous f32 features, bf16 + fp16 token buffers")
    check(_lib.load().icka_regions_to_tokens_h(src.data_ptr(), dst.data_ptr(), dst16.data_ptr(), B, R, Cc, layout, _stream()),
          "icka_regions_to_tokens_h")


def colsum_workspace(N: int, device) -> torch.Tensor:
    return torch.empty(_lib.load().icka_colsum_workspace_floats(N), dtype=F32, device=device)


def colsum(x, out, partials, accumulate=True):
    _mat(x, "x")
    M, N = x.shape
    check(_lib.load().icka_colsum(x.data_ptr(), x.stride(0), out.data_ptr(), partials.data_ptr(), M, N,
                                  int(accumulate), _stream()), "icka_colsum")
    return out


def gate_bwd(dout, g, cross, du, dcross, dcross_in=None):
    _mat(dout, "dout"); _mat(cross, "cross")
    M, H = dout.shape
    check(_lib.load().icka_gate_bwd(dout.data_ptr(), dout.stride(0), g.data_ptr(), cross.data_ptr(), cross.stride(0),
                                    _ptr(dcross_in), _ld(dcross_in), du.data_ptr(), dcross.data_ptr(),
                                    dcross.stride(0), M, H, _stream()), "icka_gate_bwd")


def add_bf16(a, b, out):
    check(_lib.load().icka_add_bf16(a.data_ptr(), b.data_ptr(), out.data_ptr(), a.numel(), _stream()), "icka_add")
    return out


def token_ce(logits, labels, mask, loss_sum, count, dlogits):
    M, Cn = logits.shape
    check(_lib.load().icka_token_ce(logits.data_ptr(), logits.stride(0), labels.data_ptr(), mask.data_ptr(),
                                    loss_sum.data_ptr(), count.data_ptr(), dlogits.data_ptr(), dlogits.stride(0),
                                    M, Cn, _stream()), "icka_token_ce")


def token_ce_fused(logits, labels, mask, stats, dlogits):
    M, Cn = logits.shape
    lib = _lib.load()
    part = torch.empty(lib.icka_token_ce_workspace_floats(M), dtype=F32, device=logits.device)
    check(lib.icka_token_ce_fused(logits.data_ptr(), logits.stride(0), labels.data_ptr(), mask.data_ptr(),
                                  stats.data_ptr(), part.data_ptr(), dlogits.data_ptr(), dlogits.stride(0),
                                  int(dlogits.dtype == F32), M, Cn, _stream()), "icka_token_ce_fused")


def zero_(t: torch.Tensor) -> torch.Tensor:
    _dev(t, "t")
    if t.dtype != F32 or not t.is_contiguous():
        raise TypeError("zero_: contiguous f32 tensor")
    check(_lib.load().icka_zero_f32(t.data_ptr(), t.numel(), _stream()), "icka_zero_f32")
# ... 263 lines not shown
```

### icka_amd/modeling.py

```python
from __future__ import annotations

import copy
import math
from typing import List, Optional

import torch
import torch.nn as nn

from . import exact as X
from . import kernels as K
from . import ops
from . import packing
from .arena import ArenaModule, ParamArena, arena_of, refresh_shadow_once
from .config import BertConfig, check_config, check_head_size_bf16

BF16, F32 = torch.bfloat16, torch.float32


class _CastFn(torch.autograd.Function):
    @staticmethod
    def forward(ctx, x, to_bf16: bool):
        ctx.to_bf16 = to_bf16
        x = x.contiguous()
        if to_bf16:
# ... 431 lines not shown
    tok = _hidden2d(token_embedding, "token_embedding")
    c0 = cross.view(B, S, H)[:, 0]
    t0 = tok.view(B, S, H)[:, 0]
    feat = ops.AddLayerNormFn.apply(A.anchor, c0, t0, owner.cls_layer.proj_norm, A, float(owner.cls_layer.proj_norm.eps))
    related = ops.LinearFn.apply(A.anchor, feat, owner.cls_layer.proj, A, False, K.EPI_NONE)
    logit = ops.LinearFn.apply(A.anchor, related, owner.aux_head, A, True, K.EPI_NONE)
    out = ops.SampleGateFn.apply(tok, cross, logit.view(B), 0, B, S)
    return out.view(B, S, H)


class BertPreTrainedModel(_IckaModule):

    def __init__(self, config, *inputs, **kwargs):
        super().__init__()
        for f in ("hidden_size", "num_hidden_layers", "num_attention_heads", "intermediate_size",
                  "hidden_dropout_prob", "attention_probs_dropout_prob", "max_position_embeddings",
                  "type_vocab_size", "vocab_size"):
            if not hasattr(config, f):
                raise ValueError("Parameter config in `{}(config)` should expose BertConfig fields (missing `{}`)"
                                 .format(self.__class__.__name__, f))
        self.config = config

    def init_bert_weights(self, module):
        std = getattr(self.config, "initializer_range", 0.02)
        if isinstance(module, (nn.Linear, nn.Embedding)):
            module.weight.data.normal_(mean=0.0, std=std)
        elif isinstance(module, BertLayerNorm):
            module.bias.data.zero_()
            module.weight.data.fill_(1.0)
        if isinstance(module, nn.Linear) and module.bias is not None:
            module.bias.data.zero_()

    @staticmethod
    def convert_legacy_keys(state_dict):
        out = type(state_dict)()
        for key, v in state_dict.items():
            nk = key
            if "gamma" in nk:
                nk = nk.replace("gamma", "weight")
            if "beta" in nk:
                nk = nk.replace("beta", "bias")
            out[nk] = v
        return out

    @classmethod
    def from_pretrained(cls, pretrained_model_name_or_path, *inputs, **kwargs):
        import json
        import os
        state_dict = kwargs.pop("state_dict", None)
        kwargs.pop("cache_dir", None)
        if kwargs.pop("from_tf", False):
            raise NotImplementedError("TensorFlow checkpoints: convert to a PyTorch state_dict first")
        config = kwargs.pop("config", None)
        if config is None:
            for n in ("config.json", "bert_config.json"):
                p = os.path.join(pretrained_model_name_or_path, n)
                if os.path.exists(p):
                    config = BertConfig.from_json_file(p)
                    break
        if config is None:
            raise EnvironmentError("no config.json / bert_config.json under %r" % (pretrained_model_name_or_path,))
        model = cls(config, *inputs, **kwargs)
        if state_dict is None:
            state_dict = torch.load(os.path.join(pretrained_model_name_or_path, "pytorch_model.bin"),
                                    map_location="cpu")
        state_dict = cls.convert_legacy_keys(state_dict)
        if not hasattr(model, "bert") and any(k.startswith("bert.") for k in state_dict):
            state_dict = type(state_dict)((k[5:], v) for k, v in state_dict.items() if k.startswith("bert."))
        missing, unexpected = model.load_state_dict(state_dict, strict=False)
        model._load_report = {"missing": list(missing), "unexpected": list(unexpected)}
        return model


class BertModel(BertPreTrainedModel):

    def __init__(self, config):
        super().__init__(config)
        check_config(config)
        self.embeddings = BertEmbeddings(config)
        self.encoder = BertEncoder(config)
        self.pooler = BertPooler(config)
        self.apply(self.init_bert_weights)

    def encode(self, input_ids, token_type_ids=None, attention_mask=None, output_all_encoded_layers=True):
        if not input_ids.is_cuda:
            raise TypeError("input_ids must be on a ROCm device: icka_amd has no CPU path")
        B, S = input_ids.shape
        self._arena()
        add_mask = torch.zeros(B, S, dtype=F32, device=input_ids.device) if attention_mask is None else \
            K.additive_mask(attention_mask.long() if attention_mask.dtype != torch.int64 else attention_mask, S,
                            torch.empty(B, S, dtype=F32, device=input_ids.device))
        extended_attention_mask = add_mask.view(B, 1, 1, S)
        embedding_output = self.embeddings(input_ids, token_type_ids)
        return self.encoder(embedding_output, extended_attention_mask, output_all_encoded_layers=output_all_encoded_layers)

    def forward(self, input_ids, token_type_ids=None, attention_mask=None, output_all_encoded_layers=True):
        encoded_layers = self.encode(input_ids, token_type_ids, attention_mask, output_all_encoded_layers)
        sequence_output = encoded_layers[-1]
        pooled_output = self.pooler(sequence_output)
        if not output_all_encoded_layers:
            encoded_layers = encoded_layers[-1]
        return encoded_layers, pooled_output


def _packed_text_encoder(self, A, plan, input_ids, segment_ids, input_mask, pool):
    cfg = self.config
    B, S = input_ids.shape
    H, T = cfg.hidden_size, plan.max_tokens
    dev = input_ids.device
    add_mask = K.additive_mask(input_mask if input_mask.dtype == torch.int64 else input_mask.long(), S,
                               torch.empty(B, S, dtype=F32, device=dev))
    emb = self.bert.embeddings(input_ids, segment_ids)
    embf = _twin(emb)
    x = packing.RowsGatherFn.apply(emb.view(B * S, H), plan.p2p, 1, T, plan.pad2pack, 1)
    xf = None
    if embf is not None:
        xf = K.rows_gather(embf, torch.empty(T, H, dtype=embf.dtype, device=dev), plan.p2p)
    d = _dims(cfg, B, S, 0, self.training)
    d.pack = plan
    for layer in self.bert.encoder.layer:
        x, xf = ops.BertLayerFn.apply(A.anchor, x, xf, layer, A, add_mask, d)
    pooled = None
    if pool:
        if torch.is_grad_enabled() and x.requires_grad:
            to_pool, x = ops.FanOutFn.apply(x, 2)
        else:
            to_pool = x
        first = packing.RowsGatherFn.apply(to_pool, plan.pad2pack, S, B, plan.cls_of, 1)
        pooled = ops.LinearFn.apply(A.anchor, first, self.bert.pooler.dense, A, False, K.EPI_TANH)
    return x, xf, pooled


def _mner_trunk(self, input_ids, segment_ids, input_mask, added_attention_mask, visual_embeds_att, pool=False, plan=None):
    cfg = self.config
    B, S = input_ids.shape
    H = cfg.hidden_size
    A = self._arena()
    dev = input_ids.device
    pooled = None
    if plan is not None:
        seq, seqf, pooled = _packed_text_encoder(self, A, plan, input_ids, segment_ids, input_mask, pool)
        sequence_output = None
    elif isinstance(self.bert, BertModel):
        sequence_output = self.bert.encode(input_ids, segment_ids, input_mask, output_all_encoded_layers=False)[-1]
        if pool:
            seqf = _twin(sequence_output)
            if not _is_exact(self) and torch.is_grad_enabled() and sequence_output.requires_grad:
                to_pool, so = ops.FanOutFn.apply(sequence_output.view(B * S, H), 2)
                sequence_output = _with_twin(so, seqf, (B, S, H))
                pooled = self.bert.pooler(to_pool.view(B, S, H))
            else:
                pooled = self.bert.pooler(sequence_output)
    else:
        sequence_output, pooled = self.bert(input_ids, token_type_ids=segment_ids, attention_mask=input_mask,
                                            output_all_encoded_layers=False)
    tail = (pooled,) if pool else ()
    exact = _is_exact(self)
    if exact:
        return _mner_trunk_exact(self, A, sequence_output.view(B * S, H), added_attention_mask, visual_embeds_att, B,
                                 S) + tail
    if plan is None:
        seq = sequence_output.view(B * S, H)
        seqf = _twin(sequence_output)
    if self.training and cfg.hidden_dropout_prob > 0:
        seq = ops.DropoutFn.apply(seq, A, float(cfg.hidden_dropout_prob))
        seqf = None
    v = visual_embeds_att
    R, layout = _region_layout(v)
    rows_p = (B * R + 127) // 128 * 128
    tokens = torch.empty(rows_p, 2048, dtype=BF16, device=dev)
    K.zero_rows_(tokens, B * R)
    vsrc = v.float().contiguous() if v.dtype != F32 or not v.is_contiguous() else v
    mixed = _is_mixed(self)
    vis16 = None
    if mixed:
        tokens16 = torch.empty(rows_p, 2048, dtype=torch.float16, device=dev)
        K.zero_rows_(tokens16, B * R)
        K.regions_to_tokens_h(vsrc, tokens, tokens16, B, R, 2048, layout)
        vis, vis16 = ops.LinearFn.apply(A.anchor, tokens, self.vismap2text, A, False, K.EPI_NONE, tokens16)
    else:
        K.regions_to_tokens(vsrc, tokens, B, R, 2048, layout)
        vis = ops.LinearFn.apply(A.anchor, tokens, self.vismap2text, A, False, K.EPI_NONE)
    img_mask = K.additive_mask(added_attention_mask if added_attention_mask.dtype == torch.int64
                               else added_attention_mask.long(), R, torch.empty(B, R, dtype=F32, device=dev))
    if torch.is_grad_enabled() and seq.requires_grad:
        cross, seq = ops.FanOutFn.apply(seq, 2)
    else:
        cross = seq
    crossf = seqf
    for layer in self.txt2img_attention.layer:
        d = _dims(cfg, B, S, R, self.training, mixed=_is_mixed(layer))
        d.pack = plan
        cross, crossf = ops.CrossLayerFn.apply(A.anchor, cross, crossf, vis, layer, A, img_mask, d,
                                               vis16 if d.h16 else None)
    return (A, seq, seqf, cross, crossf) + tail


def _region_layout(v: torch.Tensor):
    if not v.is_cuda:
        raise TypeError("visual_embeds_att must be on a ROCm device")
    if v.dim() == 4 or (v.dim() == 3 and v.shape[1] == 2048 and v.shape[2] != 2048):
        return (v.shape[2] * v.shape[3] if v.dim() == 4 else v.shape[2]), 1
    return v.shape[1], 0


def _mner_trunk_exact(self, A, seq, added_attention_mask, v, B, S):
    cfg = self.config
    dev = seq.device
    if self.training and cfg.hidden_dropout_prob > 0:
        seq = X.DropoutFn.apply(seq, A, float(cfg.hidden_dropout_prob))
    R, layout = _region_layout(v)
    tokens = X.regions_to_tokens(v if v.dtype == F32 else v.float(), B, R, layout)
    vis = X.LinearFn.apply(A.anchor, tokens, self.vismap2text, A, False)
    img_mask = K.additive_mask(added_attention_mask if added_attention_mask.dtype == torch.int64
                               else added_attention_mask.long(), R, torch.empty(B, R, dtype=F32, device=dev))
    d = _dims(cfg, B, S, R, self.training, True)
    cross = seq
    for layer in self.txt2img_attention.layer:
        cross = X.CrossLayerFn.apply(A.anchor, cross, vis, layer, A, img_mask, d)
    return A, seq, None, cross, None


class MTCCMBertForMMTokenClassificationCRF(BertPreTrainedModel):

    def __init__(self, config, layer_num1=1, layer_num2=1, layer_num3=1, num_labels=2, regions=49, variant="cl",
                 max_seq_length=128, cross_attention_fp8=False, use_crf=False, aux_losses=False):
        super().__init__(config)
        check_config(config)
        if variant not in ("cl", "gate_cl"):
            raise ValueError("variant must be 'cl' (my_bert/cl_modeling.py) or 'gate_cl' (my_bert/gate_cl_modeling.py)")
        self.num_labels = num_labels
        self.regions = regions
        self.variant = variant
        self.bert = BertModel(config)
        self.dropout = nn.Dropout(config.hidden_dropout_prob)
        self.vismap2text = nn.Linear(2048, config.hidden_size)
        self.txt2img_attention = BertCrossEncoder(config, layer_num1)
        if cross_attention_fp8:
            for layer in self.txt2img_attention.layer:
                layer.attention.self.fp8_scores = True
        if variant == "gate_cl":
            self.crs_classifier = nn.Linear(config.hidden_size * 2 * max_seq_length, 2)
        self.Gate_text = nn.Linear(config.hidden_size, config.hidden_size)
        self.Gate_image = nn.Linear(config.hidden_size, config.hidden_size)
        self.classifier = nn.Linear(config.hidden_size * 2, num_labels)
        self.aux_losses = bool(aux_losses)
        if self.aux_losses:
            self.text_dense_cl = nn.Linear(config.hidden_size, config.hidden_size)
            self.text_ouput_cl = nn.Linear(config.hidden_size, config.hidden_size)
            self.image_dense_cl = nn.Linear(2048, config.hidden_size)
            self.image_output_cl = nn.Linear(config.hidden_size, config.hidden_size)
        self.crf = None
        if use_crf:
            from .crf import CRF
            self.crf = CRF(num_labels, batch_first=True)
        self.apply(self.init_bert_weights)

    def logits(self, input_ids, segment_ids, input_mask, added_attention_mask, visual_embeds_att):
        return self._feats(input_ids, segment_ids, input_mask, added_attention_mask, visual_embeds_att)[0]

    def _feats(self, input_ids, segment_ids, input_mask, added_attention_mask, visual_embeds_att, n_swap=0, pool=False):
        cfg = self.config
        B, S = input_ids.shape
        H = cfg.hidden_size
        plan = None
        st = packing.state_of(self)
        if st is not None:
            st.check_error("detected at the next forward")
            packing.validate(self, S)
            plan = st.plan(input_mask)
        trunk = _mner_trunk(self, input_ids, segment_ids, input_mask, added_attention_mask, visual_embeds_att, pool=pool,
                            plan=plan)
        A, seq, seqf, cross, crossf = trunk[:5]
        pooled = trunk[5] if pool else None
        crs = None
        if self.variant == "gate_cl" and n_swap >= 2:
            if crossf is not None and _is_mixed(self):
                cross, crossf = ops.SampleSwapFn.apply(cross, B, n_swap, crossf)
            else:
                cross, crossf = ops.SampleSwapFn.apply(cross, B, n_swap), None
        if self.variant == "gate_cl":
            if self.crs_classifier.weight.shape[1] != 2 * H * S:
                raise ValueError("gate_cl: sequence length %d does not match crs_classifier (built for %d)"
                                 % (S, self.crs_classifier.weight.shape[1] // (2 * H)))
            if _is_exact(self):
                crs = X.CrsFn.apply(A.anchor, seq, cross, self.crs_classifier, A, B, S)
                cross = X.SampleGateFn.apply(cross, None, crs, 1, B, S)
            else:
                if torch.is_grad_enabled() and seq.requires_grad:
                    seq, seq_c = ops.FanOutFn.apply(seq, 2)
                    cross, cross_c = ops.FanOutFn.apply(cross, 2)
                else:
                    seq_c, cross_c = seq, cross
                crs = ops.CrsFn.apply(A.anchor, seq_c, cross_c, self.crs_classifier, A, B, S)
                if _is_mixed(self):
                    d16 = _dims(cfg, B, S, 0, self.training, mixed=True)
                    cross, crossf = ops.SampleGateFn.apply(cross, None, crs, 1, B, S, ops._fwd_twin(A, cross, crossf, d16))
                else:
                    cross = ops.SampleGateFn.apply(cross, None, crs, 1, B, S)
        if _is_exact(self):
            return X.GatedHeadFn.apply(A.anchor, seq, cross, self, A).view(B, S, self.num_labels), crs, pooled
        seq16 = cross16 = None
        if _is_mixed(self):
            d16 = _dims(cfg, B, S, 0, self.training, mixed=True)
            seq16 = ops._fwd_twin(A, seq, seqf, d16)
            cross16 = ops._fwd_twin(A, cross, crossf, d16)
        logits = ops.GatedHeadFn.apply(A.anchor, seq, cross, self, A, seq16, cross16)
        if plan is not None:
            logits = packing.RowsGatherFn.apply(logits, plan.pad2pack, 1, B * S, plan.p2p, 1, packing.F32_NAN_WORD)
        return logits.view(B, S, self.num_labels), crs, pooled

    def forward(self, input_ids, segment_ids=None, input_mask=None, added_attention_mask=None, visual_embeds_mean=None,
                visual_embeds_att=None, temp=None, temp_lamb=None, lamb=None, labels=None, negative_rate=None, *,
                attention_mask=None, visual_feats=None, token_type_ids=None):
        if attention_mask is not None:
            if input_mask is not None:
                raise TypeError("forward() got both input_mask and its alias attention_mask")
            input_mask = attention_mask
        if visual_feats is not None:
            if visual_embeds_att is not None:
                raise TypeError("forward() got both visual_embeds_att and its alias visual_feats")
            visual_embeds_att = visual_feats
        if token_type_ids is not None:
            if segment_ids is not None:
                raise TypeError("forward() got both segment_ids and its alias token_type_ids")
            segment_ids = token_type_ids
        if visual_embeds_att is None:
            raise TypeError("forward() needs the region features (visual_embeds_att / visual_feats)")
        if segment_ids is None:
            segment_ids = torch.zeros_like(input_ids)
        if input_mask is None:
            input_mask = torch.ones_like(input_ids)
        if added_attention_mask is None:
            R = visual_embeds_att.shape[1] if visual_embeds_att.dim() == 3 else visual_embeds_att.shape[2] * visual_embeds_att.shape[3]
            added_attention_mask = torch.cat([torch.ones(input_ids.shape[0], R, dtype=input_mask.dtype, device=input_mask.device),
                                              input_mask], dim=1)
        if labels is not None and self.aux_losses:
            return self._objective(input_ids, segment_ids, input_mask, added_attention_mask, visual_embeds_mean,
                                   visual_embeds_att, temp, temp_lamb, lamb, labels, negative_rate)
        logits = self.logits(input_ids, segment_ids, input_mask, added_attention_mask, visual_embeds_att)
        if labels is None:
            if self.crf is not None:
                return self.crf.decode(logits, mask=input_mask.byte())
            return logits
        if self.crf is not None:
            return -self.crf(logits, labels, mask=input_mask.byte(), reduction="mean")
        return token_ce_loss(logits, labels, input_mask, exact=_is_exact(self))

    def _main_loss(self, logits, labels, input_mask):
        if self.crf is not None:
            return -self.crf(logits, labels, mask=input_mask.byte(), reduction="mean")
        return token_ce_loss(logits, labels, input_mask, exact=_is_exact(self))

    def _objective(self, input_ids, segment_ids, input_mask, added_attention_mask, visual_embeds_mean, visual_embeds_att,
                   temp, temp_lamb, lamb, labels, negative_rate):
        gate = self.variant == "gate_cl"
        for name, val in (("temp", temp), ("temp_lamb", temp_lamb)) + ((("lamb", lamb),) if gate else ()):
            if val is None:
                raise ValueError("aux_losses=True: forward() with labels needs %s" % name)
        if visual_embeds_mean is None:
            raise ValueError("aux_losses=True: forward() with labels needs visual_embeds_mean")
        B = input_ids.shape[0]
        if visual_embeds_mean.shape[0] != B or visual_embeds_mean.shape[-1] != 2048 or not visual_embeds_mean.is_cuda:
            raise ValueError("visual_embeds_mean must be a [B, 2048] ROCm tensor")
        H = self.config.hidden_size
        if not (1 <= B <= 256) or H % 8 or H > 4096:
            raise ValueError("aux_losses: the contrastive loss takes 1 <= B <= 256 samples and hidden sizes that are multiples "
                             "of 8 up to 4096, got B=%d H=%d" % (B, H))
        n_neg = int(negative_rate) if (gate and negative_rate is not None and B > negative_rate) else 0
        logits, crs, pooled = self._feats(input_ids, segment_ids, input_mask, added_attention_mask, visual_embeds_att,
                                          n_swap=n_neg, pool=True)
        main = self._main_loss(logits, labels, input_mask)
        A = arena_of(self)
        vm = visual_embeds_mean.reshape(B, 2048)
        if _is_exact(self):
            vm = vm if vm.dtype == F32 and vm.is_contiguous() else vm.float().contiguous()
            t = X.ReluHeadFn.apply(A.anchor, pooled, self.text_dense_cl, self.text_ouput_cl, A)
            v = X.ReluHeadFn.apply(A.anchor, vm, self.image_dense_cl, self.image_output_cl, A)
        else:
            if vm.dtype != BF16:
                vm = K.cast_f32_to_bf16(vm.float().contiguous(), torch.empty(B, 2048, dtype=BF16, device=vm.device))
            t = ops.ReluHeadFn.apply(A.anchor, pooled, self.text_dense_cl, self.text_ouput_cl, A)
            v = ops.ReluHeadFn.apply(A.anchor, vm.contiguous(), self.image_dense_cl, self.image_output_cl, A)
        cl_loss, crs_loss = ops.ContrastiveFn.apply(t, v, crs if gate else None, n_neg, float(temp), float(temp_lamb))
        if gate:
            lamb = float(lamb)
            return lamb * main + (1.0 - lamb) * (crs_loss + cl_loss)
        return 0.88 * main + 0.12 * cl_loss


class MTCCMBertForMMTokenClassificationCRF_gate_1(BertPreTrainedModel):

    def __init__(self, config, embedding=None, last_encoder=None, layer_num1=1, layer_num2=1, layer_num3=1,
                 num_labels=2):
        super().__init__(config)
        check_config(config)
        from .crf import CRF
        from .lstm import BiLSTM
        self.num_labels = num_labels
        self.last_encoder = last_encoder
        self.bert = embedding if embedding is not None else BertModel(config)
        self.hidden_size = config.hidden_size
        self.dropout = nn.Dropout(config.hidden_dropout_prob)
        self.vismap2text = nn.Linear(2048, config.hidden_size)
        self.txt2img_attention = BertCrossEncoder(config, layer_num1)
        self.lstm = BiLSTM(input_size=config.hidden_size, hidden_size=config.hidden_size, batch_first=True,
                           bidirectional=True)
        self.classifier = nn.Linear(config.hidden_size * 2, num_labels)
        self.crf = CRF(num_tags=num_labels, batch_first=True)
        if embedding is None:
            self.apply(self.init_bert_weights)
            self.lstm.reset_parameters()
            self.crf.reset_parameters()

    def emissions(self, ori_input_ids, ori_segment_ids, ori_input_mask, added_attention_mask, visual_embeds_att):
        B, S = ori_input_ids.shape
        A, _, _, cross, _ = _mner_trunk(self, ori_input_ids, ori_segment_ids, ori_input_mask, added_attention_mask,
                                        visual_embeds_att)
        x, _ = self.lstm(cross.view(B, S, self.hidden_size))
        if _is_exact(self):
            em = X.LinearFn.apply(A.anchor, x.reshape(B * S, 2 * self.hidden_size), self.classifier, A, False)
        else:
# ... 29 lines not shown
```

### icka_amd/ops.py

```python
from __future__ import annotations

from typing import Optional

import torch

from . import kernels as K
from .arena import ParamArena

BF16, F32, F16 = torch.bfloat16, torch.float32, torch.float16
import os as _os
ATTN_KEEPBITS = _os.environ.get("ICKA_ATTN_KEEPBITS", "auto")
FUSE_DENSE_LN = _os.environ.get("ICKA_FUSE_DENSE_LN", "1") != "0"
FUSE_DENSE_LN_MIN_ROWS = 3072
FUSE_QKV_ATTN = _os.environ.get("ICKA_FUSE_QKV_ATTN", "1") != "0"
FUSE_QKV_ATTN_MIN_ROWS = 3072


def _keepbits_on(Sq: int, Skv: int) -> bool:
    if ATTN_KEEPBITS == "auto":
        return Sq > 128 and Skv > 128 and Sq <= 256 and Skv <= 256
    return ATTN_KEEPBITS == "1"


def _empty(ref: torch.Tensor, *shape, dtype=BF16) -> torch.Tensor:
    return torch.empty(*shape, dtype=dtype, device=ref.device)


def _c(t: torch.Tensor) -> torch.Tensor:
    if t.dtype != BF16:
        raise TypeError("expected a bf16 gradient, got %s" % t.dtype)
    return t if t.is_contiguous() else t.contiguous()


class Dims(object):
    __slots__ = ("B", "S", "R", "H", "I", "heads", "eps", "p_hidden", "p_attn", "train", "h16", "pack")

    def __init__(self, B, S, R, H, I, heads, eps, p_hidden, p_attn, train, h16=False, pack=None):
        self.B, self.S, self.R, self.H, self.I, self.heads, self.eps = B, S, R, H, I, heads, eps
        self.p_hidden = p_hidden if train else 0.0
        self.p_attn = p_attn if train else 0.0
        self.train = train
        self.h16 = bool(h16)
        self.pack = pack


def _fwd_twin(A: ParamArena, x, xf, d: Dims):
    if not d.h16:
        return xf
    if A.shadow16 is None:
        A.enable_fp16_shadow()
        A.sync(force=True)
    if xf is not None and xf.dtype == F16:
        return xf
    return K.cast_to_f16(x if xf is None else xf, _empty(x, x.shape[0], x.shape[1], dtype=F16))


def _wgrad(A: ParamArena, dy, x, gout, beta: float, bias=None) -> None:
    bout, bacc = None, False
    if bias is not None:
        bacc = A.grad_beta(bias) > 0
        bout = A.g_cat(bias) if isinstance(bias, tuple) else A.g(bias)
        M, N, Kt = dy.shape[1], x.shape[1], dy.shape[0]
        if M % 128 or N % 128 or Kt % 64:
            csw = A.workspace("colsum", K._lib.load().icka_colsum_workspace_floats(M))
            K.colsum(dy, bout, csw, accumulate=bacc)
            bout = None
    wire = A.wire_of(gout, beta)
    A.pending_wgrad.append((K.gemm_desc(K.GEMM_TN, dy, x, gout, beta=beta, colsum_out=bout, colsum_accumulate=bacc,
                                        **wire), dy, x, gout, bout, wire))


def _flush_wgrad(A: ParamArena) -> None:
    if A.pending_wgrad or A.pending_reductions:
        K.gemm_grouped([t[0] for t in A.pending_wgrad], reductions=A.pending_reductions)
        A.pending_wgrad = []
        A.pending_reductions = []


def _ln_bwd_deferred(A: ParamArena, tag: str, norm, dy, xhat, rstd, *, dy2, dres, dx, p_drop, seed) -> None:
    H = dy.shape[1]
    ws = A.workspace(tag, K._lib.load().icka_ln_bwd_workspace_floats(H))
    acc = A.grad_beta((norm.weight, norm.bias)) > 0
    nslab = K.ln_bwd_slabs(dy, xhat, rstd, norm.weight, ws, dy2=dy2, dres=dres, dx=dx, p_drop=p_drop, seed=seed)
    A.pending_reductions.append(K.slab_reduction(ws, nslab, H, (A.g(norm.weight), A.g(norm.bias)), acc))


def _attn_generic_fwd(qkv, kvbuf, self_attn: bool, add_mask, d: Dims, Skv: int, seed_a: int, ctx, ctx16, save: bool):
    import math
    from . import exact as X
    B, h, S, H = d.B, d.heads, d.S, d.H
    dh = H // h
    q32b = K.cast_bf16_to_f32(qkv, torch.empty(qkv.shape, dtype=F32, device=qkv.device))
    if self_attn:
        q, k, v = q32b[:, :H], q32b[:, H:2 * H], q32b[:, 2 * H:]
        kv32b = None
    else:
        kv32b = K.cast_bf16_to_f32(kvbuf, torch.empty(kvbuf.shape, dtype=F32, device=kvbuf.device))
        q, k, v = q32b, kv32b[:, :H], kv32b[:, H:]
# ... 417 lines not shown
class LinearFn(torch.autograd.Function):

    @staticmethod
    def forward(ctx, anchor, x, lin, A: ParamArena, out_f32: bool, epilogue: int, x16=None):
        M = x.shape[0]
        N = lin.weight.shape[0]
        if x16 is not None:
            if out_f32 or epilogue != K.EPI_NONE:
                raise ValueError("LinearFn: the fp16-operand form is a plain bf16-output projection")
            if A.shadow16 is None:
                A.enable_fp16_shadow()
                A.sync(force=True)
            y = torch.empty(M, N, dtype=BF16, device=x.device)
            y16 = torch.empty(M, N, dtype=F16, device=x.device)
            K.gemm(K.GEMM_NT, x16, A.w16(lin.weight), y16, bias=lin.bias, out3=y)
            ctx.lin, ctx.A, ctx.epi = lin, A, epilogue
            ctx.need_dx = x.requires_grad
            ctx.save_for_backward(x, None)
            ctx.mark_non_differentiable(y16)
            ctx.set_materialize_grads(False)
            return y, y16
        y = torch.empty(M, N, dtype=F32 if out_f32 else BF16, device=x.device)
        if M <= 64 and not out_f32 and x.shape[1] % 128 == 0 and x.stride(0) % 8 == 0 and \
                epilogue in (K.EPI_NONE, K.EPI_TANH):
            K.linear_small_m(x, A.w(lin.weight), lin.bias, y, act=1 if epilogue == K.EPI_TANH else 0)
        else:
            K.gemm(K.GEMM_NT, x, A.w(lin.weight), y, bias=lin.bias, epilogue=epilogue)
        ctx.lin, ctx.A, ctx.epi = lin, A, epilogue
        ctx.need_dx = x.requires_grad
        ctx.save_for_backward(x, y if epilogue == K.EPI_TANH else None)
        return y

    @staticmethod
    def backward(ctx, dy, _dy16=None):
        x, y = ctx.saved_tensors
        lin, A = ctx.lin, ctx.A
        M, N = dy.shape
        if dy.dtype == F32:
            ldd = (N + 7) // 8 * 8
            dyb = torch.empty(M, ldd, dtype=BF16, device=dy.device)
            K.cast_pad_f32_to_bf16(dy if dy.stride(1) == 1 else dy.contiguous(), dyb)
            dyv = dyb[:, :N]
        else:
            dyv = _c(dy)
        if ctx.epi == K.EPI_TANH:
            dyv = K.tanh_bwd(dyv if dyv.is_contiguous() else dyv.contiguous(), y, torch.empty_like(y))
        fused = lin.bias is not None and N % 128 == 0 and x.shape[1] % 128 == 0 and M % 64 == 0
        gw = A.g(lin.weight)
        beta_w = A.grad_beta(lin.weight)
        wire = A.wire_of(gw, beta_w) if (N % 128 == 0 and x.shape[1] % 128 == 0) else {}
        K.gemm(K.GEMM_TN, dyv, x, gw, beta=beta_w,
               colsum_out=A.g(lin.bias) if fused else None,
               colsum_accumulate=fused and A.grad_beta(lin.bias) > 0,
               **wire)
        if lin.bias is not None and not fused:
            csw = A.workspace("colsum", K._lib.load().icka_colsum_workspace_floats(N))
            K.colsum(dyv, A.g(lin.bias), csw, accumulate=A.grad_beta(lin.bias) > 0)
        dx = None
        if ctx.need_dx:
            dx = torch.empty_like(x)
            K.gemm(K.GEMM_NN, dyv, A.w(lin.weight), dx)
        A.flush_final()
        return None, dx, None, None, None, None, None


class DropoutFn(torch.autograd.Function):

    @staticmethod
    def forward(ctx, x, A: ParamArena, p: float):
        seed = A.next_seed()
        y = torch.empty_like(x)
        K.dropout(x, y, p_drop=p, seed=seed)
        ctx.p, ctx.seed = p, seed
        return y

    @staticmethod
    def backward(ctx, dy):
        dy = _c(dy)
        dx = torch.empty_like(dy)
        K.dropout(dy, dx, p_drop=ctx.p, seed=ctx.seed)
        return dx, None, None


class GatedHeadFn(torch.autograd.Function):

    @staticmethod
    def forward(ctx, anchor, seq, cross, head, A: ParamArena, seq16=None, cross16=None):
        M, H = seq.shape
        C = head.classifier.weight.shape[0]
        gate = torch.empty(M, H, dtype=BF16, device=seq.device)
        gated = torch.empty_like(gate)
        h16 = seq16 is not None and cross16 is not None
        ctx.skinny = C <= 16 and H % 8 == 0 and 2 * H // 8 <= 256 and C * 2 * H * 2 <= 44 * 1024
        logits = torch.empty(M, C, dtype=F32, device=seq.device)
        if h16:
            if A.shadow16 is None:
                A.enable_fp16_shadow()
                A.sync(force=True)
            gated16 = torch.empty(M, H, dtype=F16, device=seq.device)
            K.gemm(K.GEMM_NT, seq16, A.w16(head.Gate_text.weight), gated16, A2=cross16, B2=A.w16(head.Gate_image.weight),
                   bias=head.Gate_text.bias, bias2=head.Gate_image.bias, epilogue=K.EPI_GATE, aux=cross16, out2=gate,
                   out3=gated)
            Wc = A.w16(head.classifier.weight)
            if ctx.skinny:
                K.cls_head_fwd(seq16, gated16, Wc, head.classifier.bias, logits)
            else:
                K.gemm(K.GEMM_NT, seq16, Wc[:, :H], logits, A2=gated16, B2=Wc[:, H:], bias=head.classifier.bias)
        else:
            K.gemm(K.GEMM_NT, seq, A.w(head.Gate_text.weight), gated, A2=cross, B2=A.w(head.Gate_image.weight),
                   bias=head.Gate_text.bias, bias2=head.Gate_image.bias, epilogue=K.EPI_GATE, aux=cross, out2=gate)
            Wc = A.w(head.classifier.weight)
            if ctx.skinny:
                K.cls_head_fwd(seq, gated, Wc, head.classifier.bias, logits)
            else:
                K.gemm(K.GEMM_NT, seq, Wc[:, :H], logits, A2=gated, B2=Wc[:, H:], bias=head.classifier.bias)
        ctx.head, ctx.A = head, A
        ctx.save_for_backward(seq, cross, gate, gated)
        return logits

    @staticmethod
    def backward(ctx, dlogits):
        seq, cross, gate, gated = ctx.saved_tensors
        head, A = ctx.head, ctx.A
        M, H = seq.shape
        C = dlogits.shape[1]
        if dlogits.dtype == BF16 and dlogits.stride(1) == 1 and dlogits.stride(0) % 8 == 0:
            dl = dlogits
        else:
            buf = torch.empty(M, (C + 7) // 8 * 8, dtype=BF16, device=seq.device)
            K.cast_pad_f32_to_bf16(dlogits.float() if dlogits.dtype != F32 else
                                   (dlogits if dlogits.stride(1) == 1 else dlogits.contiguous()), buf)
            dl = buf[:, :C]
        cls = head.classifier
        if ctx.skinny:
            lib = K._lib.load()
            nslab, sf = lib.icka_cls_head_bwd_slabs(M), lib.icka_cls_head_slab_floats(H, C)
            ws = A.workspace("cls_head", nslab * sf)
            dseq_c = torch.empty(M, H, dtype=BF16, device=seq.device)
            du = torch.empty_like(dseq_c)
            dcross_d = torch.empty_like(dseq_c)
            K.cls_head_bwd(dl, seq, gated, gate, cross, A.w(cls.weight), dseq_c, du, dcross_d, ws)
            A.pending_reductions.append(K.slab_reduction(ws, nslab, C * 2 * H, (A.g(cls.weight).view(-1),),
                                                         A.grad_beta(cls.weight) > 0, slab_stride=sf))
            A.pending_reductions.append(K.slab_reduction(ws, nslab, C, (A.g(cls.bias),), A.grad_beta(cls.bias) > 0,
                                                         slab_stride=sf, offset=C * 2 * H))
            return GatedHeadFn._gate_tail(A, head, seq, cross, du, dseq_c, dcross_d)
        gW = A.g(cls.weight)
        beta = A.grad_beta(cls.weight)
        K.gemm(K.GEMM_TN, dl, seq, gW[:, :H], beta=beta)
        K.gemm(K.GEMM_TN, dl, gated, gW[:, H:], beta=beta)
        csw = A.workspace("colsum", K._lib.load().icka_colsum_workspace_floats(max(H, C)))
        K.colsum(dl, A.g(cls.bias), csw, accumulate=A.grad_beta(cls.bias) > 0)
        Wc = A.w(cls.weight)
        dseq_c = torch.empty(M, H, dtype=BF16, device=seq.device)
        dgated = torch.empty_like(dseq_c)
        K.gemm(K.GEMM_NN, dl, Wc[:, :H], dseq_c)
        K.gemm(K.GEMM_NN, dl, Wc[:, H:], dgated)
        du = torch.empty_like(dseq_c)
        dcross_d = torch.empty_like(dseq_c)
        K.gate_bwd(dgated, gate, cross, du, dcross_d)
        return GatedHeadFn._gate_tail(A, head, seq, cross, du, dseq_c, dcross_d)

    @staticmethod
    def _gate_tail(A, head, seq, cross, du, dseq_c, dcross_d):
        _wgrad(A, du, seq, A.g(head.Gate_text.weight), A.grad_beta(head.Gate_text.weight), bias=head.Gate_text.bias)
        _wgrad(A, du, cross, A.g(head.Gate_image.weight), A.grad_beta(head.Gate_image.weight),
               bias=head.Gate_image.bias)
        _flush_wgrad(A)
        dseq = torch.empty_like(dseq_c)
        dcross = torch.empty_like(dseq_c)
        K.gemm(K.GEMM_NN, du, A.w(head.Gate_text.weight), dseq, epilogue=K.EPI_ADD, aux=dseq_c)
        K.gemm(K.GEMM_NN, du, A.w(head.Gate_image.weight), dcross, epilogue=K.EPI_ADD, aux=dcross_d)
        A.flush_final()
        return None, dseq, dcross, None, None, None, None


class SampleGateFn(torch.autograd.Function):

    @staticmethod
    def forward(ctx, a, c, gate, mode: int, B: int, S: int, a16=None):
        out = torch.empty_like(a)
        ctx.mode, ctx.B, ctx.S = mode, B, S
        ctx.save_for_backward(a, c, gate)
        if a16 is not None:
            if c is not None:
                raise ValueError("SampleGateFn: the fp16 form has no blend operand")
            out16 = torch.empty(a.shape[0], a.shape[1], dtype=F16, device=a.device)
            K.sample_gate_fwd_h(a16, gate, mode, out, out16, B, S)
            ctx.mark_non_differentiable(out16)
            ctx.set_materialize_grads(False)
            return out, out16
        K.sample_gate_fwd(a, c, gate, mode, out, B, S)
        return out

    @staticmethod
    def backward(ctx, dout, _d16=None):
        a, c, gate = ctx.saved_tensors
        dout = _c(dout)
        da = torch.empty_like(a)
        dc = torch.empty_like(a) if c is not None else None
# ... 278 lines not shown
```

### include/icka_hip.h

```cpp
#ifndef ICKA_HIP_H
#define ICKA_HIP_H

#include <stdint.h>

#ifdef __cplusplus
extern "C" {
#endif

#define ICKA_E_SHAPE (-1)
#define ICKA_E_ALIGN (-2)
#define ICKA_E_ARG (-3)

#define ICKA_ABI_VERSION 6
int icka_abi_version(void);
const char* icka_build_arch(void);

int icka_copy_many(const void* const* src, void* const* dst, const int64_t* bytes, int32_t n, void* stream);

enum { ICKA_GEMM_NT = 0, ICKA_GEMM_NN = 1, ICKA_GEMM_TN = 2 };
enum {
    ICKA_EPI_NONE = 0,
    ICKA_EPI_GELU = 1,
    ICKA_EPI_DGELU = 2,
    ICKA_EPI_ADD = 3,
// ... 57 lines not shown
                  int64_t ldy2, void* y_f16, void* xhat, float* rstd, int32_t M, int32_t H, float eps, float p_drop,
                  uint64_t seed, void* stream);
int64_t icka_ln_bwd_workspace_floats(int32_t H);
int icka_ln_bwd(const void* dy, int64_t lddy, const void* dy2, int64_t lddy2, const void* xhat, const float* rstd,
                const float* gamma, void* dres, int64_t lddres, void* dx, int64_t lddx, float* dgamma, float* dbeta,
                float* dbias, float* partials, int32_t M, int32_t H, float p_drop, uint64_t seed, int32_t accumulate,
                void* stream);
int icka_ln_bwd_slabs(const void* dy, int64_t lddy, const void* dy2, int64_t lddy2, const void* xhat, const float* rstd,
                      const float* gamma, void* dres, int64_t lddres, void* dx, int64_t lddx, float* partials, int32_t M,
                      int32_t H, float p_drop, uint64_t seed, void* stream);
int32_t icka_ln_bwd_nslab(int32_t M);
int32_t icka_ln_slab_slots(void);

int icka_embed_fwd(const int64_t* ids, const int64_t* token_type, const float* word, const float* pos,
                   const float* type, const float* gamma, const float* beta, void* y, float* y_f32, void* xhat,
                   float* rstd, int32_t B, int32_t S, int32_t H, int32_t vocab, int32_t n_type, float eps,
                   float p_drop, uint64_t seed, void* stream);
int icka_embed_fwd_h(const int64_t* ids, const int64_t* token_type, const float* word, const float* pos,
                     const float* type, const float* gamma, const float* beta, void* y, void* y_f16, void* xhat,
                     float* rstd, int32_t B, int32_t S, int32_t H, int32_t vocab, int32_t n_type, float eps,
                     float p_drop, uint64_t seed, void* stream);
int icka_embed_bwd(const void* dy, const int64_t* ids, const int64_t* token_type, const void* xhat,
                   const float* rstd, const float* gamma, float* dword, float* dpos, float* dtype, float* dgamma,
                   float* dbeta, float* partials, int32_t B, int32_t S, int32_t H, int32_t vocab, int32_t n_type,
                   int32_t padding_idx, float p_drop, uint64_t seed, int32_t accumulate, void* stream);
int icka_embed_bwd_rows(const void* dy, const int64_t* ids, const int64_t* token_type, const void* xhat, const float* rstd,
                        const float* gamma, float* dtok, float* dpos, float* dtype, float* dgamma, float* dbeta, float* partials,
                        int32_t B, int32_t S, int32_t H, int32_t vocab, int32_t n_type, int32_t padding_idx, float p_drop,
                        uint64_t seed, int32_t accumulate, void* stream);
int icka_embed_scatter_rows(const void* rows, int32_t rows_are_bf16, const int64_t* ids, float* dword, int64_t T, int32_t H,
                            int32_t vocab, int32_t padding_idx, float scale, void* stream);
int icka_embed_prompt_fwd(const int64_t* ids, const int32_t* src, const void* prompt, const float* word,
                          const float* pos, const float* type, const float* gamma, const float* beta, void* y,
                          float* y_f32, void* xhat, float* rstd, int32_t B, int32_t S_in, int32_t S, int32_t P,
                          int32_t H, int32_t vocab, int32_t pos_offset, float eps, float p_drop, uint64_t seed,
                          void* stream);
int icka_embed_prompt_bwd(const void* dy, const int64_t* ids, const int32_t* src, const void* xhat, const float* rstd,
                          const float* gamma, float* dword, float* dpos, float* dtype, float* dgamma, float* dbeta,
                          void* dprompt, float* partials, int32_t B, int32_t S_in, int32_t S, int32_t P, int32_t H,
                          int32_t vocab, int32_t pos_offset, int32_t padding_idx, float p_drop, uint64_t seed,
                          int32_t accumulate, void* stream);

int icka_attn_fwd(const void* Q, int64_t ldq, const void* K, int64_t ldk, const void* V, int64_t ldv,
                  const float* add_mask, void* O, int64_t ldo, float* lse, int32_t B, int32_t heads, int32_t Sq,
                  int32_t Skv, float scale, float p_drop, uint64_t seed, void* stream);
int icka_attn_fwd_fp8(const void* Q, int64_t ldq, const void* K, int64_t ldk, const void* V, int64_t ldv,
                      const float* add_mask, void* O, int64_t ldo, float* lse, int32_t B, int32_t heads, int32_t Sq,
                      int32_t Skv, float scale, float p_drop, uint64_t seed, void* stream);
int icka_attn_fwd_ex(const void* Q, int64_t ldq, const void* K, int64_t ldk, const void* V, int64_t ldv,
                     const float* add_mask, void* O, void* O_f16, int64_t ldo, float* lse, int32_t B, int32_t heads,
                     int32_t Sq, int32_t Skv, float scale, float p_drop, uint64_t seed, int32_t flags, void* keep_bits,
                     void* stream);
#define ICKA_ATTN_FP8 1
#define ICKA_ATTN_TILED 2
int64_t icka_attn_keepbits_words(int32_t B, int32_t heads, int32_t Sq, int32_t Skv);
int icka_attn_bwd(const void* Q, int64_t ldq, const void* K, int64_t ldk, const void* V, int64_t ldv,
                  const float* add_mask, const void* O, int64_t ldo, const void* dO, int64_t lddo, const float* lse,
                  float* delta, void* dQ, int64_t lddq, void* dK, int64_t lddk, void* dV, int64_t lddv, int32_t B,
                  int32_t heads, int32_t Sq, int32_t Skv, float scale, float p_drop, uint64_t seed, const void* keep_bits,
                  int32_t flags, void* stream);

int icka_pack_plan(const int64_t* mask, int32_t B, int32_t S, int32_t max_tokens, int32_t* lens, int32_t* cu_seqlens,
                   int32_t* packed_to_padded, int32_t* padded_to_packed, int32_t* cls_of, int32_t* status, void* err_word,
                   void* stream);
int icka_rows_gather(const void* src, int64_t ld_src, int64_t src_rows, void* dst, int64_t ld_dst, int64_t dst_rows,
                     int32_t row_words, const int32_t* map, int64_t map_stride, uint32_t fill, void* stream);
int icka_attn_fwd_packed(const void* Q, int64_t ldq, const void* K, int64_t ldk, const void* V, int64_t ldv,
                         const float* add_mask, void* O, int64_t ldo, float* lse, const int32_t* cu_seqlens, int32_t kv_packed,
                         int64_t Mrows, int32_t B, int32_t heads, int32_t Sq, int32_t Skv, float scale, float p_drop,
                         uint64_t seed, void* keep_bits, void* stream);
int icka_attn_bwd_packed(const void* Q, int64_t ldq, const void* K, int64_t ldk, const void* V, int64_t ldv,
                         const float* add_mask, const void* dO, int64_t lddo, const float* lse, float* delta, void* dQ,
                         int64_t lddq, void* dK, int64_t lddk, void* dV, int64_t lddv, const int32_t* cu_seqlens,
                         int32_t kv_packed, int64_t Mrows, int32_t B, int32_t heads, int32_t Sq, int32_t Skv, float scale,
                         float p_drop, uint64_t seed, const void* keep_bits, void* stream);

int icka_cast_f32_to_bf16(const float* src, void* dst, int64_t n, void* stream);
int icka_cast_bf16_to_f32(const void* src, float* dst, int64_t n, void* stream);
int icka_cast_to_f16(const void* src, int32_t src_is_f32, void* dst, int64_t n, void* stream);
int icka_cast_f32_to_bf16_f16(const float* src, void* dst_bf16, void* dst_f16, int64_t n, void* stream);
int icka_cast_pad_f32_to_bf16(const float* src, int64_t lds, void* dst, int64_t ldd, int32_t M, int32_t N,
                              void* stream);
int icka_additive_mask(const int64_t* mask, int64_t ld, float* out, int32_t B, int32_t T, void* stream);
int icka_dropout(const void* x, int64_t ldx, void* y, int64_t ldy, void* y2, int64_t ldy2, int32_t M, int32_t H,
                 float p_drop, uint64_t seed, void* stream);
int icka_regions_to_tokens(const float* src, void* dst, int32_t B, int32_t R, int32_t C, int32_t layout,
                           void* stream);
int icka_regions_to_tokens_h(const float* src, void* dst_bf16, void* dst_f16, int32_t B, int32_t R, int32_t C, int32_t layout,
                             void* stream);
int icka_colsum(const void* x, int64_t ldx, float* out, float* partials, int32_t M, int32_t N, int32_t accumulate,
                void* stream);
int64_t icka_colsum_workspace_floats(int32_t N);
int icka_gate_bwd(const void* dout, int64_t lddout, const void* g, const void* cross, int64_t ldcross,
                  const void* dcross_in, int64_t lddci, void* du, void* dcross, int64_t lddc, int32_t M, int32_t H,
                  void* stream);
int icka_cls_head_fwd(const void* seq, const void* gated, const void* W, const float* bias, float* logits, int32_t M,
                      int32_t H, int32_t C, void* stream);
int icka_cls_head_fwd_h(const void* seq, const void* gated, const void* W, const float* bias, float* logits, int32_t M,
                        int32_t H, int32_t C, void* stream);
int icka_cls_head_bwd(const void* dl, int64_t ldd, const void* seq, const void* gated, const void* gate,
                      const void* cross, const void* W, void* dseq, void* du, void* dcross, float* partials, int32_t M,
                      int32_t H, int32_t C, void* stream);
int32_t icka_cls_head_bwd_slabs(int32_t M);
int64_t icka_cls_head_slab_floats(int32_t H, int32_t C);
int icka_sample_gate_fwd(const void* a, int64_t lda, const void* c, int64_t ldc, const float* gate, int32_t mode,
                         void* out, int64_t ldo, int32_t B, int32_t S, int32_t H, void* stream);
int icka_sample_gate_fwd_h(const void* a16, int64_t lda, const float* gate, int32_t mode, void* out, void* out16, int64_t ldo,
                           int32_t B, int32_t S, int32_t H, void* stream);
int icka_sample_gate_bwd(const void* dout, int64_t lddo, const void* a, int64_t lda, const void* c, int64_t ldc,
                         const float* gate, int32_t mode, void* da, int64_t ldda, void* dc, int64_t lddc, float* dgate,
                         int32_t B, int32_t S, int32_t H, void* stream);
int icka_crs_fwd(const void* seq, int64_t lds, const void* cross, int64_t ldc, const void* W, const float* bias,
                 float* crs, int32_t B, int32_t S, int32_t H, void* stream);
int icka_crs_bwd(const float* dcrs, const void* seq, int64_t lds, const void* cross, int64_t ldc, const void* W,
                 void* dseq, void* dcross, float* dW, float* dbias, int32_t B, int32_t S, int32_t H,
                 int32_t accumulate, void* stream);
int icka_add_bf16(const void* a, const void* b, void* c, int64_t n, void* stream);
int icka_dgelu_bf16(const void* dg, const void* z, void* dz, int64_t n, void* stream);
int icka_tanh_bwd(const void* dy, const void* y, void* dx, int64_t n, void* stream);

int64_t icka_contrastive_workspace_floats(int32_t B);
int icka_contrastive_fwd(const void* t, int64_t ldt, const void* v, int64_t ldv, int32_t dtype, int32_t B, int32_t D,
                         float temp, float temp_lamb, const float* crs, int32_t n_neg, float* stats, float* ws, void* stream);
int icka_contrastive_bwd(const void* t, int64_t ldt, const void* v, int64_t ldv, int32_t dtype, int32_t B, int32_t D,
                         float temp, float temp_lamb, const float* ws, const float* dcl, const float* dcrs_loss, void* dt,
                         void* dv, const float* crs, int32_t n_neg, float* dcrs, void* stream);
int icka_relu_bwd(const void* dy, const void* y, void* dx, int64_t n, int32_t is_f32, void* stream);
int icka_sample_swap(const void* x, void* y, int32_t B, int64_t sample_bytes, int32_t n_neg, void* stream);
int icka_token_ce(const float* logits, int64_t ld, const int64_t* labels, const int64_t* mask, float* loss_sum,
                  float* count, void* dlogits, int64_t ldd, int32_t M, int32_t C, void* stream);
int icka_scale_by_ratio(const void* x, void* y, const float* num, const float* den, int64_t n, void* stream);
int64_t icka_token_ce_workspace_floats(int32_t M);
int icka_token_ce_fused(const float* logits, int64_t ld, const int64_t* labels, const int64_t* mask, float* stats,
                        float* partials, void* dlogits, int64_t ldd, int32_t dl_is_f32, int32_t M, int32_t C, void* stream);
int icka_zero_f32(float* p, int64_t n, void* stream);
int icka_scalar_ratio(float* out, const float* num, const float* den, void* stream);
int icka_crf_llh(const float* emissions, int64_t ld, const int64_t* tags, const int64_t* mask, const float* start,
                 const float* end, const float* trans, float* llh, int32_t B, int32_t S, int32_t C, void* stream);
int icka_crf_grad(const float* emissions, int64_t ld, const int64_t* tags, const int64_t* mask, const float* start,
                  const float* end, const float* trans, const float* gllh, float* d_emissions, int64_t ldd,
                  float* d_start, float* d_end, float* d_trans, int32_t B, int32_t S, int32_t C, void* stream);
int icka_crf_decode(const float* emissions, int64_t ld, const int64_t* mask, const float* start, const float* end,
                    const float* trans, int64_t* best_tags, float* best_score, int32_t B, int32_t S, int32_t C,
                    void* stream);
int icka_crf_score_decode(const float* emissions, int64_t ld, const int64_t* tags, const int64_t* mask,
                          const float* start, const float* end, const float* trans, float* llh, int32_t* lens,
                          int32_t* tags_flat, int64_t capacity, int32_t B, int32_t S, int32_t C, void* stream);
int icka_lstm_fwd(const float* gates_x, int64_t ldg, const void* w_hh, void* y, float* c_all, void* act, void* hprev,
                  int32_t B, int32_t S, int32_t H, int32_t flags, void* stream);
int icka_lstm_bwd(const void* dy, const void* w_hh_t, const void* act, const float* c_all, void* dgates, int64_t ldg,
                  float* dc_carry, int32_t B, int32_t S, int32_t H, int32_t flags, void* stream);
#define ICKA_LSTM_PER_STEP 1
#define ICKA_LSTM_TICKETS 2
#define ICKA_LSTM_NO_BATCH_SPLIT 4
int icka_lstm_barrier_error(void);
int icka_lstm_clear_error(void);
int icka_lstm_set_reserved_cus(int32_t n);
int icka_lstm_test_hooks(int32_t poll_limit, int32_t drop_step);
int icka_linear_small_m(const void* x, int64_t ldx, const void* W, const float* bias, void* y, int64_t ldy, int32_t M,
                        int32_t N, int32_t K, int32_t act, void* stream);
int icka_transpose_bf16(const void* in, void* out, int32_t batch, int32_t R, int32_t C, void* stream);
int icka_conv_stem_patches(const float* image, void* patches, int32_t B, int32_t H, int32_t W, int64_t rows_padded,
                           void* stream);
int icka_conv_im2col3x3(const void* src, void* patches, int32_t B, int32_t H, int32_t W, int32_t C, int32_t stride,
                        int64_t rows_padded, void* stream);
int icka_conv3x3_gemm(const void* x, const void* w, const float* bias, const void* aux, int64_t ldaux, void* y, int32_t B,
                      int32_t H, int32_t W, int32_t C, int32_t Cout, int32_t stride, int64_t rows_padded, int32_t epilogue,
                      const void* zeros, void* stream);
int icka_conv_subsample(const void* src, void* dst, int32_t B, int32_t H, int32_t W, int32_t C, int32_t stride,
                        int64_t rows_padded, void* stream);
int icka_conv_maxpool3x3s2(const void* src, void* dst, int32_t B, int32_t H, int32_t W, int32_t C, int64_t rows_padded,
                           void* stream);
int icka_conv_features_out(const void* x, float* att, float* fc, void* tokens, int32_t B, int32_t P, int32_t C,
                           void* stream);
int icka_gemm_bn_stats(const void* a, int64_t lda, const void* w, int64_t ldw, void* y, int64_t ldy, int32_t M, int32_t N, int32_t K,
                       int64_t rows_valid, float* partials, void* stream);
int icka_conv3x3_gemm_stats(const void* x, const void* w, void* y, int32_t B, int32_t H, int32_t W, int32_t C, int32_t Cout,
                            int32_t stride, int64_t rows_padded, const void* zeros, float* partials, void* stream);
int icka_bn_finalize(const float* partials, int32_t tiles, int32_t C, const float* weight, const float* bias, float* running_mean,
                     float* running_var, const int64_t* num_batches_tracked, float momentum, float eps, float* scale, float* shift,
                     void* stream);
int icka_bn_apply(const void* raw, const float* scale, const float* shift, const void* residual, const float* res_scale,
                  const float* res_shift, void* y, int32_t C, int64_t rows_valid, int64_t rows_padded, int32_t relu, int64_t* nbt_a,
                  int64_t* nbt_b, void* stream);
int icka_set_dropout_nonce(const uint32_t* device_words);
int icka_bump_dropout_nonce(uint32_t* device_words, void* stream);
int icka_dropout_mask(float* out, int64_t n, float p_drop, uint64_t seed, void* stream);
// ... 84 lines not shown
```

Measured before the change: 7002 samples/s.

## Fuse token cross-entropy into gated head kernels and merge small elementwise launches

Result: no change. 7035 samples/s (median of 6 runs) (+0.5%).

```diff
diff --git a/icka_amd/_lib.py b/icka_amd/_lib.py
--- a/icka_amd/_lib.py
+++ b/icka_amd/_lib.py
@@ -94,6 +94,10 @@
     "icka_cls_head_bwd": (c_i32, [c_vp, c_i64, c_vp, c_vp, c_vp, c_vp, c_vp, c_vp, c_vp, c_vp, c_vp, c_i32, c_i32, c_i32,
                                   c_vp]),
     "icka_cls_head_bwd_slabs": (c_i32, [c_i32]),
+    "icka_cls_head_ce_workspace_floats": (c_i64, [c_i32]),
+    "icka_cls_head_ce_fwd": (c_i32, [c_vp, c_vp, c_vp, c_i32, c_vp, c_vp, c_vp, c_vp, c_vp, c_vp, c_vp, c_i32, c_i32, c_i32, c_vp]),
+    "icka_cls_head_ce_bwd": (c_i32, [c_vp, c_vp, c_vp, c_vp, c_vp, c_vp, c_vp, c_vp, c_vp, c_vp, c_vp, c_vp, c_vp, c_vp, c_i32,
+                                     c_i32, c_i32, c_vp]),
     "icka_cls_head_slab_floats": (c_i64, [c_i32, c_i32]),
     "icka_conv_stem_patches": (c_i32, [c_vp, c_vp, c_i32, c_i32, c_i32, c_i64, c_vp]),
     "icka_conv_im2col3x3": (c_i32, [c_vp, c_vp, c_i32, c_i32, c_i32, c_i32, c_i32, c_i64, c_vp]),
@@ -129,7 +133,10 @@
     "icka_cast_bf16_to_f32": (c_i32, [c_vp, c_vp, c_i64, c_vp]),
     "icka_cast_pad_f32_to_bf16": (c_i32, [c_vp, c_i64, c_vp, c_i64, c_i32, c_i32, c_vp]),
     "icka_additive_mask": (c_i32, [c_vp, c_i64, c_vp, c_i32, c_i32, c_vp]),
+    "icka_additive_mask2": (c_i32, [c_vp, c_i64, c_vp, c_i32, c_vp, c_i64, c_vp, c_i32, c_i32, c_vp]),
     "icka_dropout": (c_i32, [c_vp, c_i64, c_vp, c_i64, c_vp, c_i64, c_i32, c_i32, c_f32, c_u64, c_vp]),
+    "icka_dropout_cast": (c_i32, [c_vp, c_vp, c_i32, c_i32, c_f32, c_u64, c_vp, c_vp, c_i64, c_vp]),
+    "icka_add_dropout": (c_i32, [c_vp, c_vp, c_vp, c_i32, c_i32, c_f32, c_u64, c_vp]),
     "icka_regions_to_tokens": (c_i32, [c_vp, c_vp, c_i32, c_i32, c_i32, c_i32, c_vp]),
     "icka_regions_to_tokens_h": (c_i32, [c_vp, c_vp, c_vp, c_i32, c_i32, c_i32, c_i32, c_vp]),
     "icka_sample_gate_fwd_h": (c_i32, [c_vp, c_i64, c_vp, c_i32, c_vp, c_vp, c_i64, c_i32, c_i32, c_i32, c_vp]),
diff --git a/icka_amd/csrc/elementwise.hip b/icka_amd/csrc/elementwise.hip
--- a/icka_amd/csrc/elementwise.hip
+++ b/icka_amd/csrc/elementwise.hip
@@ -86,6 +86,19 @@
     if (i >= B * T) return;
     const int b = i / T, t = i - b * T;
     out[i] = (1.0f - (float)mask[(int64_t)b * ld + t]) * -10000.0f;
+}
+
+__global__ void additive_mask2_kernel(const int64_t* __restrict__ mask0, int64_t ld0, float* __restrict__ out0, int T0,
+                                      const int64_t* __restrict__ mask1, int64_t ld1, float* __restrict__ out1, int T1, int B) {
+    const int i = blockIdx.x * blockDim.x + threadIdx.x;
+    if (i < B * T0) {
+        const int b = i / T0, t = i - b * T0;
+        out0[i] = (1.0f - (float)mask0[(int64_t)b * ld0 + t]) * -10000.0f;
+    } else if (i < B * (T0 + T1)) {
+        const int k = i - B * T0;
+        const int b = k / T1, t = k - b * T1;
+        out1[k] = (1.0f - (float)mask1[(int64_t)b * ld1 + t]) * -10000.0f;
+    }
 }
 
 __global__ void dropout_kernel(const bf16_t* __restrict__ x, int64_t ldx, bf16_t* __restrict__ y, int64_t ldy,
@@ -103,6 +116,51 @@
         for (int e = 0; e < 8; ++e) v[e] *= drop_mul(d, base + e);
         st8(y + row * ldy + c * 8, v);
         if (y2) st8(y2 + row * ldy2 + c * 8, v);
+    }
+}
+
+__global__ void dropout_cast_kernel(const bf16_t* __restrict__ x, bf16_t* __restrict__ y, int M, int H, DropCfg d_,
+                                    int drop_blocks, const float* __restrict__ src, bf16_t* __restrict__ dst, int64_t n) {
+    if ((int)blockIdx.x < drop_blocks) {
+        const DropCfg d = drop_resolve(d_);
+        const int cpr = H >> 3;
+        const int64_t total = (int64_t)M * cpr;
+        for (int64_t i = (int64_t)blockIdx.x * blockDim.x + threadIdx.x; i < total; i += (int64_t)drop_blocks * blockDim.x) {
+            const int64_t row = i / cpr;
+            const int c = (int)(i - row * cpr);
+            float v[8];
+            ld8(x + row * H + c * 8, v);
+            const uint32_t base = (uint32_t)row * (uint32_t)H + c * 8;
+#pragma unroll
+            for (int e = 0; e < 8; ++e) v[e] *= drop_mul(d, base + e);
+            st8(y + row * H + c * 8, v);
+        }
+        return;
+    }
+    const int bid = blockIdx.x - drop_blocks, nb = gridDim.x - drop_blocks;
+    const int64_t nch = n >> 3;
+    for (int64_t c = (int64_t)bid * blockDim.x + threadIdx.x; c < nch; c += (int64_t)nb * blockDim.x) {
+        const f32x4 a = *reinterpret_cast<const f32x4*>(src + c * 8), b = *reinterpret_cast<const f32x4*>(src + c * 8 + 4);
+        bf16x8 o = {f2bf(a[0]), f2bf(a[1]), f2bf(a[2]), f2bf(a[3]), f2bf(b[0]), f2bf(b[1]), f2bf(b[2]), f2bf(b[3])};
+        *reinterpret_cast<u32x4*>(dst + c * 8) = as_u32x4(o);
+    }
+    if (bid == 0 && threadIdx.x < (n & 7)) dst[(nch << 3) + threadIdx.x] = f2bf(src[(nch << 3) + threadIdx.x]);
+}
+
+__global__ void add_dropout_kernel(const bf16_t* __restrict__ a, const bf16_t* __restrict__ b, bf16_t* __restrict__ y, int M, int H,
+                                   DropCfg d_) {
+    const DropCfg d = drop_resolve(d_);
+    const int cpr = H >> 3;
+    const int64_t total = (int64_t)M * cpr;
+    for (int64_t i = (int64_t)blockIdx.x * blockDim.x + threadIdx.x; i < total; i += (int64_t)gridDim.x * blockDim.x) {
+        const int64_t row = i / cpr;
+        const int c = (int)(i - row * cpr);
+        float v[8], w[8];
+        ld8(a + i * 8, v); ld8(b + i * 8, w);
+        const uint32_t base = (uint32_t)row * (uint32_t)H + c * 8;
+#pragma unroll
+        for (int e = 0; e < 8; ++e) v[e] = bf2f(f2bf(v[e] + w[e])) * drop_mul(d, base + e);
+        st8(y + i * 8, v);
     }
 }
 
@@ -480,6 +538,36 @@
     ICKA_CHECK_LAUNCH();
     return 0;
 }
+extern "C" int icka_additive_mask2(const int64_t* mask0, int64_t ld0, float* out0, int32_t T0, const int64_t* mask1, int64_t ld1,
+                                   float* out1, int32_t T1, int32_t B, void* stream) {
+    if (!mask0 || !out0 || !mask1 || !out1) return ICKA_E_ARG;
+    if (B <= 0 || T0 <= 0 || T1 <= 0 || ld0 < T0 || ld1 < T1 || (int64_t)B * ((int64_t)T0 + T1) > (1 << 30)) return ICKA_E_SHAPE;
+    hipLaunchKernelGGL(additive_mask2_kernel, dim3((B * (T0 + T1) + 255) / 256), dim3(256), 0, (hipStream_t)stream, mask0, ld0,
+                       out0, T0, mask1, ld1, out1, T1, B);
+    ICKA_CHECK_LAUNCH();
+    return 0;
+}
+extern "C" int icka_dropout_cast(const void* x, void* y, int32_t M, int32_t H, float p_drop, uint64_t seed, const float* src,
+                                 void* dst, int64_t n, void* stream) {
+    if (!x || !y || !src || !dst) return ICKA_E_ARG;
+    if (M <= 0 || H <= 0 || H % 8 || n <= 0) return ICKA_E_SHAPE;
+    if (!al16(x) || !al16(y) || !al16(src) || !al16(dst)) return ICKA_E_ALIGN;
+    const int gd = grid_for((int64_t)M * (H / 8)), gc = grid_for((n + 7) / 8);
+    hipLaunchKernelGGL(dropout_cast_kernel, dim3(gd + gc), dim3(256), 0, (hipStream_t)stream, (const bf16_t*)x, (bf16_t*)y, M, H,
+                       make_drop(p_drop, seed), gd, src, (bf16_t*)dst, n);
+    ICKA_CHECK_LAUNCH();
+    return 0;
+}
+extern "C" int icka_add_dropout(const void* a, const void* b, void* y, int32_t M, int32_t H, float p_drop, uint64_t seed,
+                                void* stream) {
+    if (!a || !b || !y) return ICKA_E_ARG;
+    if (M <= 0 || H <= 0 || H % 8) return ICKA_E_SHAPE;
+    if (!al16(a) || !al16(b) || !al16(y)) return ICKA_E_ALIGN;
+    hipLaunchKernelGGL(add_dropout_kernel, dim3(grid_for((int64_t)M * (H / 8))), dim3(256), 0, (hipStream_t)stream,
+                       (const bf16_t*)a, (const bf16_t*)b, (bf16_t*)y, M, H, make_drop(p_drop, seed));
+    ICKA_CHECK_LAUNCH();
+    return 0;
+}
 extern "C" int icka_dropout_mask(float* out, int64_t n, float p_drop, uint64_t seed, void* stream) {
     if (!out) return ICKA_E_ARG;
     if (n <= 0) return 0;
diff --git a/icka_amd/csrc/fusion.hip b/icka_amd/csrc/fusion.hip
--- a/icka_amd/csrc/fusion.hip
+++ b/icka_amd/csrc/fusion.hip
@@ -307,21 +307,40 @@
     *reinterpret_cast<u32x4*>(p) = as_u32x4(o);
 }
 
-template <bool F16>
-__global__ __launch_bounds__(256) void cls_head_fwd_kernel(const bf16_t* __restrict__ seq, const bf16_t* __restrict__ gated,
-                                                           const bf16_t* __restrict__ W, const float* __restrict__ bias,
-                                                           float* __restrict__ logits, int M, int H, int C) {
+struct ClsCe {
+    const int64_t* labels;
+    const int64_t* mask;
+    float* rowstat;
+    unsigned int* counter;
+    float* stats;
+};
+__device__ __forceinline__ float cls_ld_sc1(__amdgpu_buffer_rsrc_t r, int byte_off) {
+    return __uint_as_float(__builtin_amdgcn_raw_buffer_load_b32(r, byte_off, 0, 16));
+}
+
+template <bool F16, int WAVES = 4, bool CE = false>
+__global__ __launch_bounds__(WAVES * 64) void cls_head_fwd_kernel(const bf16_t* __restrict__ seq, const bf16_t* __restrict__ gated,
+                                                                  const bf16_t* __restrict__ W, const float* __restrict__ bias,
+                                                                  float* __restrict__ logits, int M, int H, int C, const ClsCe ce) {
     extern __shared__ __attribute__((aligned(16))) char cls_smem[];
-    __shared__ float s_red[4][CLS_MAXC][65];
+    __shared__ float s_red[WAVES][CLS_MAXC][65];
+    __shared__ float s_lg[CE ? WAVES : 1][2][CLS_MAXC];
+    __shared__ int s_last;
     bf16_t* sW = reinterpret_cast<bf16_t*>(cls_smem);
     const int tid = threadIdx.x, lane = tid & 63, wave = tid >> 6;
     const int nch = (2 * H) >> 3, hch = H >> 3;
-    for (int i = tid; i < C * nch; i += 256)
+    for (int i = tid; i < C * nch; i += WAVES * 64)
         *reinterpret_cast<u32x4*>(sW + (int64_t)i * 8) = *reinterpret_cast<const u32x4*>(W + (int64_t)i * 8);
     __syncthreads();
-    const int nw = gridDim.x * 4;
-    for (int row0 = (blockIdx.x * 4 + wave) * 2; row0 < M; row0 += 2 * nw) {
+    const int nw = gridDim.x * WAVES;
+    [[maybe_unused]] __amdgpu_buffer_rsrc_t rs_rsrc;
+    if constexpr (CE) rs_rsrc = __builtin_amdgcn_make_buffer_rsrc(ce.rowstat, 0, 0x7ffffff0, 0x00020000);
+    for (int row0 = (blockIdx.x * WAVES + wave) * 2; row0 < M; row0 += 2 * nw) {
         u32x4 xr[2][4];
+        [[maybe_unused]] int64_t ce_y = 0, ce_m = 0;
+        if constexpr (CE) {
+            if (lane < 2 && row0 + lane < M) { ce_y = ce.labels[row0 + lane]; ce_m = ce.mask[row0 + lane]; }
+        }
 #pragma unroll
         for (int r = 0; r < 2; ++r)
 #pragma unroll
@@ -379,28 +398,143 @@
             for (int i = 0; i < 16; ++i) v += s_red[wave][c][16 * qd + i];
             v += __shfl_xor(v, 1, 64);
             v += __shfl_xor(v, 2, 64);
-            if (qd == 0 && c < C && row0 + r < M)
-                logits[(int64_t)(row0 + r) * C + c] = v + (bias ? bias[c] : 0.f);
+            if (qd == 0 && c < C && row0 + r < M) {
+                const float lg = v + (bias ? bias[c] : 0.f);
+                logits[(int64_t)(row0 + r) * C + c] = lg;
+                if constexpr (CE) s_lg[wave][r][c] = lg;
+            }
             __builtin_amdgcn_wave_barrier();
         }
-    }
-}
-
-template <int CC>
+        if constexpr (CE) {
+            float* sx = &s_red[wave][0][0];
+            {
+                const int r = (lane >> 4) & 1, c = lane & 15;
+                const float pc = (lane < 32 && c < C) ? s_lg[wave][r][c] : -INFINITY;
+                float mx = pc;
+                mx = fmaxf(mx, __shfl_xor(mx, 8, 64));
+                mx = fmaxf(mx, __shfl_xor(mx, 4, 64));
+                mx = fmaxf(mx, __shfl_xor(mx, 2, 64));
+                mx = fmaxf(mx, __shfl_xor(mx, 1, 64));
+                if (lane < 32) {
+                    sx[r * 32 + c] = c < C ? expf(pc - mx) : 0.f;
+                    if (c == 0) sx[r * 32 + 16] = mx;
+                }
+            }
+            __builtin_amdgcn_wave_barrier();
+            if (lane < 2 && row0 + lane < M) {
+                const int row = row0 + lane;
+                const float* p = s_lg[wave][lane];
+                const bool valid = ce_m != 0;
+                const int64_t y = ce_y;
+                float se = 0.f;
+                for (int k = 0; k < C; ++k) se += sx[lane * 32 + k];
+                const float lse = sx[lane * 32 + 16] + logf(se);
+                float loss = 0.f, cnt = 0.f;
+                if (valid && y >= 0 && y < C) { loss = lse - p[y]; cnt = 1.f; }
+                __builtin_amdgcn_raw_buffer_store_b32(__float_as_uint(loss), rs_rsrc, row * 4, 0, 16);
+                __builtin_amdgcn_raw_buffer_store_b32(__float_as_uint(cnt), rs_rsrc, (M + row) * 4, 0, 16);
+            }
+            __builtin_amdgcn_wave_barrier();
+        }
+    }
+    if constexpr (CE) {
+        asm volatile("s_waitcnt vmcnt(0)" ::: "memory");
+        __syncthreads();
+        if (tid == 0)
+            s_last = __hip_atomic_fetch_add(ce.counter, 1u, __ATOMIC_RELAXED, __HIP_MEMORY_SCOPE_AGENT) == gridDim.x - 1;
+        __syncthreads();
+        if (!s_last) return;
+        float* ws = &s_red[0][0][0];
+        const int nblk = (M + 255) >> 8, nchunk = 4 * nblk;
+        for (int k0 = wave; k0 < nchunk; k0 += 8 * WAVES) {
+            float l[8], n[8];
+#pragma unroll
+            for (int u = 0; u < 8; ++u) {
+                const int row = (k0 + u * WAVES) * 64 + lane;
+                l[u] = n[u] = 0.f;
+                if (k0 + u * WAVES < nchunk && row < M) { l[u] = cls_ld_sc1(rs_rsrc, row * 4); n[u] = cls_ld_sc1(rs_rsrc, (M + row) * 4); }
+            }
+#pragma unroll
+            for (int u = 0; u < 8; ++u) {
+                const int k = k0 + u * WAVES;
+                const float ls = wave_sum(l[u]), ns = wave_sum(n[u]);
+                if (lane == 0 && k < nchunk) { ws[k] = ls; ws[nchunk + k] = ns; }
+            }
+        }
+        __syncthreads();
+        if (wave == 0) {
+            float l = 0.f, n = 0.f;
+            for (int b = lane; b < nblk; b += 64) {
+                l += (ws[4 * b] + ws[4 * b + 1]) + (ws[4 * b + 2] + ws[4 * b + 3]);
+                n += (ws[nchunk + 4 * b] + ws[nchunk + 4 * b + 1]) + (ws[nchunk + 4 * b + 2] + ws[nchunk + 4 * b + 3]);
+            }
+            l = wave_sum(l);
+            n = wave_sum(n);
+            if (lane == 0) {
+                ce.stats[0] = l; ce.stats[1] = n; ce.stats[2] = l / fmaxf(n, 1.f);
+                __hip_atomic_store(ce.counter, 0u, __ATOMIC_RELAXED, __HIP_MEMORY_SCOPE_AGENT);
+            }
+        }
+    }
+}
+
+struct ClsCeBwd {
+    const float* logits;
+    const int64_t* labels;
+    const int64_t* mask;
+    const float* stats;
+    const float* dloss;
+};
+template <int CC, bool CE = false>
 __global__ __launch_bounds__(256) void cls_head_bwd_kernel(const bf16_t* __restrict__ dl, int64_t ldd,
                                                            const bf16_t* __restrict__ seq, const bf16_t* __restrict__ gated,
                                                            const bf16_t* __restrict__ gate, const bf16_t* __restrict__ cross,
                                                            const bf16_t* __restrict__ W, bf16_t* __restrict__ dseq,
                                                            bf16_t* __restrict__ du, bf16_t* __restrict__ dcross,
-                                                           float* __restrict__ partials, int M, int H, int C) {
+                                                           float* __restrict__ partials, int M, int H, int C, const ClsCeBwd ce) {
     __shared__ float s_dl[CLS_TB][CLS_MAXC];
     const int tid = threadIdx.x;
     const int nch = (2 * H) >> 3, hch = H >> 3;
     const int t0 = blockIdx.x * CLS_TB;
     const int nt = M - t0 < CLS_TB ? M - t0 : CLS_TB;
-    for (int i = tid; i < CLS_TB * CLS_MAXC; i += 256) {
-        const int t = i / CLS_MAXC, c = i % CLS_MAXC;
-        s_dl[t][c] = (t < nt && c < C) ? bf2f(dl[(int64_t)(t0 + t) * ldd + c]) : 0.f;
+    [[maybe_unused]] u32x4 wraw[CE ? CC : 1];
+    if constexpr (CE) {
+        static_assert(CLS_TB * CLS_MAXC == 256 && CLS_MAXC == 16, "one thread per (row, class)");
+        __shared__ float s_ex[CLS_TB][CLS_MAXC];
+        const int t = tid >> 4, c = tid & 15;
+        const bool live = t < nt && c < C;
+        const int64_t row = t0 + (t < nt ? t : 0);
+        const float pc = live ? ce.logits[row * C + c] : -INFINITY;
+        const bool valid = ce.mask[row] != 0;
+        const int yl = (int)ce.labels[row];
+        const float s = ce.dloss[0] / fmaxf(ce.stats[1], 1.f);
+        if (tid < nch) {
+#pragma unroll
+            for (int k = 0; k < CC; ++k)
+                if (k < C) wraw[k] = *reinterpret_cast<const u32x4*>(W + (int64_t)k * 2 * H + tid * 8);
+        }
+        float mx = pc;
+        mx = fmaxf(mx, __shfl_xor(mx, 8, 64));
+        mx = fmaxf(mx, __shfl_xor(mx, 4, 64));
+        mx = fmaxf(mx, __shfl_xor(mx, 2, 64));
+        mx = fmaxf(mx, __shfl_xor(mx, 1, 64));
+        s_ex[t][c] = live ? expf(pc - mx) : 0.f;
+        __syncthreads();
+        float d = 0.f;
+        if (live) {
+            float se = 0.f;
+            for (int k = 0; k < C; ++k) se += s_ex[t][k];
+            const float lse = mx + logf(se);
+            float gval = 0.f;
+            if (valid) gval = expf(pc - lse) - (c == yl ? 1.f : 0.f);
+            d = bf2f(f2bf(gval * s));
+        }
+        s_dl[t][c] = d;
+    } else {
+        for (int i = tid; i < CLS_TB * CLS_MAXC; i += 256) {
+            const int t = i / CLS_MAXC, c = i % CLS_MAXC;
+            s_dl[t][c] = (t < nt && c < C) ? bf2f(dl[(int64_t)(t0 + t) * ldd + c]) : 0.f;
+        }
     }
     __syncthreads();
     const int64_t slab = (int64_t)C * 2 * H + CLS_MAXC;
@@ -417,7 +551,15 @@
     float Wr[CC][8], dW[CC][8];
 #pragma unroll
     for (int c = 0; c < CC; ++c) {
-        if (c < C) cls_ld8(W + (int64_t)c * 2 * H + j * 8, Wr[c]);
+        if constexpr (CE) {
+            if (c < C) {
+                const bf16x8 wv = as_bf16x8(wraw[c]);
+#pragma unroll
+                for (int e = 0; e < 8; ++e) Wr[c][e] = bf2f(wv[e]);
+            }
+        } else {
+            if (c < C) cls_ld8(W + (int64_t)c * 2 * H + j * 8, Wr[c]);
+        }
 #pragma unroll
         for (int e = 0; e < 8; ++e) { dW[c][e] = 0.f; if (c >= C) Wr[c][e] = 0.f; }
     }
@@ -487,10 +629,10 @@
     grid = grid > 512 ? 512 : grid;
     if (f16)
         hipLaunchKernelGGL(cls_head_fwd_kernel<true>, dim3(grid), dim3(256), (size_t)C * 2 * H * 2, (hipStream_t)stream,
-                           (const bf16_t*)seq, (const bf16_t*)gated, (const bf16_t*)W, bias, logits, M, H, C);
+                           (const bf16_t*)seq, (const bf16_t*)gated, (const bf16_t*)W, bias, logits, M, H, C, ClsCe{});
     else
         hipLaunchKernelGGL(cls_head_fwd_kernel<false>, dim3(grid), dim3(256), (size_t)C * 2 * H * 2, (hipStream_t)stream,
-                           (const bf16_t*)seq, (const bf16_t*)gated, (const bf16_t*)W, bias, logits, M, H, C);
+                           (const bf16_t*)seq, (const bf16_t*)gated, (const bf16_t*)W, bias, logits, M, H, C, ClsCe{});
     ICKA_CHECK_LAUNCH();
     return 0;
 }
@@ -519,12 +661,66 @@
         hipLaunchKernelGGL((cls_head_bwd_kernel<13>), dim3(grid), dim3(256), 0, (hipStream_t)stream,
                            (const bf16_t*)dl, ldd, (const bf16_t*)seq, (const bf16_t*)gated, (const bf16_t*)gate,
                            (const bf16_t*)cross, (const bf16_t*)W, (bf16_t*)dseq, (bf16_t*)du, (bf16_t*)dcross,
-                           partials, M, H, C);
+                           partials, M, H, C, ClsCeBwd{});
     else
         hipLaunchKernelGGL((cls_head_bwd_kernel<CLS_MAXC>), dim3(grid), dim3(256), 0, (hipStream_t)stream,
                            (const bf16_t*)dl, ldd, (const bf16_t*)seq, (const bf16_t*)gated, (const bf16_t*)gate,
                            (const bf16_t*)cross, (const bf16_t*)W, (bf16_t*)dseq, (bf16_t*)du, (bf16_t*)dcross,
-                           partials, M, H, C);
-    ICKA_CHECK_LAUNCH();
-    return 0;
-}
+                           partials, M, H, C, ClsCeBwd{});
+    ICKA_CHECK_LAUNCH();
+    return 0;
+}
+
+extern "C" int64_t icka_cls_head_ce_workspace_floats(int32_t M) { return 2 * (int64_t)M; }
+extern "C" int icka_cls_head_ce_fwd(const void* seq, const void* gated, const void* W, int32_t is_f16, const float* bias,
+                                    float* logits, const int64_t* labels, const int64_t* mask, float* rowstat,
+                                    uint32_t* counter, float* stats, int32_t M, int32_t H, int32_t C, void* stream) {
+    if (!seq || !gated || !W || !logits || !labels || !mask || !rowstat || !counter || !stats) return ICKA_E_ARG;
+    if (M <= 0 || M > 65536 || H <= 0 || H % 8 || C <= 0 || C > CLS_MAXC || (int64_t)C * 2 * H * 2 > 44 * 1024)
+        return ICKA_E_SHAPE;
+    if ((reinterpret_cast<uintptr_t>(seq) | reinterpret_cast<uintptr_t>(gated) | reinterpret_cast<uintptr_t>(W)) & 15)
+        return ICKA_E_ALIGN;
+    if ((reinterpret_cast<uintptr_t>(rowstat) | reinterpret_cast<uintptr_t>(counter)) & 3) return ICKA_E_ALIGN;
+    int grid = (M + 15) / 16;
+    grid = grid > 256 ? 256 : grid;
+    size_t dyn = (size_t)C * 2 * H * 2;
+    dyn = dyn < 50 * 1024 ? 50 * 1024 : dyn;
+    const ClsCe ce{labels, mask, rowstat, counter, stats};
+    if (is_f16)
+        hipLaunchKernelGGL((cls_head_fwd_kernel<true, 8, true>), dim3(grid), dim3(512), dyn, (hipStream_t)stream,
+                           (const bf16_t*)seq, (const bf16_t*)gated, (const bf16_t*)W, bias, logits, M, H, C, ce);
+    else
+        hipLaunchKernelGGL((cls_head_fwd_kernel<false, 8, true>), dim3(grid), dim3(512), dyn, (hipStream_t)stream,
+                           (const bf16_t*)seq, (const bf16_t*)gated, (const bf16_t*)W, bias, logits, M, H, C, ce);
+    ICKA_CHECK_LAUNCH();
+    return 0;
+}
+
+extern "C" int icka_cls_head_ce_bwd(const float* logits, const int64_t* labels, const int64_t* mask, const float* stats,
+                                    const float* dloss, const void* seq, const void* gated, const void* gate,
+                                    const void* cross, const void* W, void* dseq, void* du, void* dcross, float* partials,
+                                    int32_t M, int32_t H, int32_t C, void* stream) {
+    if (!logits || !labels || !mask || !stats || !dloss) return ICKA_E_ARG;
+    if (!seq || !gated || !gate || !cross || !W || !dseq || !du || !dcross || !partials) return ICKA_E_ARG;
+    if (M <= 0 || H <= 0 || H % 8 || C <= 0 || C > CLS_MAXC || 2 * H / 8 > 256) return ICKA_E_SHAPE;
+    const uintptr_t al = reinterpret_cast<uintptr_t>(seq) | reinterpret_cast<uintptr_t>(gated) |
+                         reinterpret_cast<uintptr_t>(gate) | reinterpret_cast<uintptr_t>(cross) |
+                         reinterpret_cast<uintptr_t>(W) | reinterpret_cast<uintptr_t>(dseq) |
+                         reinterpret_cast<uintptr_t>(du) | reinterpret_cast<uintptr_t>(dcross) |
+                         reinterpret_cast<uintptr_t>(partials);
+    if (al & 15) return ICKA_E_ALIGN;
+    const int grid = icka_cls_head_bwd_slabs(M);
+    const ClsCeBwd ce{logits, labels, mask, stats, dloss};
+    if (C <= 13)
+        hipLaunchKernelGGL((cls_head_bwd_kernel<13, true>), dim3(grid), dim3(256), 0, (hipStream_t)stream,
+                           (const bf16_t*)nullptr, (int64_t)0, (const bf16_t*)seq, (const bf16_t*)gated, (const bf16_t*)gate,
+                           (const bf16_t*)cross, (const bf16_t*)W, (bf16_t*)dseq, (bf16_t*)du, (bf16_t*)dcross,
+                           partials, M, H, C, ce);
+    else
+        hipLaunchKernelGGL((cls_head_bwd_kernel<CLS_MAXC, true>), dim3(grid), dim3(256), 0, (hipStream_t)stream,
+                           (const bf16_t*)nullptr, (int64_t)0, (const bf16_t*)seq, (const bf16_t*)gated, (const bf16_t*)gate,
+                           (const bf16_t*)cross, (const bf16_t*)W, (bf16_t*)dseq, (bf16_t*)du, (bf16_t*)dcross,
+                           partials, M, H, C, ce);
+    ICKA_CHECK_LAUNCH();
+    return 0;
+}
diff --git a/icka_amd/csrc/gemm.hip b/icka_amd/csrc/gemm.hip
--- a/icka_amd/csrc/gemm.hip
+++ b/icka_amd/csrc/gemm.hip
@@ -1617,7 +1617,7 @@
     } else {
         const int nk = (g.K + BK - 1) / BK;
         int ks = 1;
-        if (g.c_f32 && g.epi == ICKA_EPI_NONE && nb < 64 && nk >= 16 && g.M <= 256 && !g.C3) {
+        if (A_KM && g.c_f32 && g.epi == ICKA_EPI_NONE && nb < 64 && nk >= 16 && g.M <= 256 && !g.C3) {
             ks = 256 / nb;
             if (ks > nk / 4) ks = nk / 4;
             if (ks < 1) ks = 1;
diff --git a/icka_amd/kernels.py b/icka_amd/kernels.py
--- a/icka_amd/kernels.py
+++ b/icka_amd/kernels.py
@@ -286,6 +286,45 @@
     return lib.icka_cls_head_bwd_slabs(M)
 
 
+def cls_head_ce_fwd(seq, gated, W, bias, logits, labels, mask, rowstat, counter, stats):
+    dt = seq.dtype if seq.dtype == F16 else BF16
+    _mat(seq, "seq", dt); _mat(gated, "gated", dt)
+    M, H = seq.shape
+    Cn = W.shape[0]
+    if not (seq.is_contiguous() and gated.is_contiguous() and W.is_contiguous() and logits.is_contiguous()):
+        raise ValueError("cls_head_ce_fwd: contiguous operands")
+    if W.dtype != dt or tuple(W.shape) != (Cn, 2 * H) or logits.dtype != F32 or tuple(logits.shape) != (M, Cn):
+        raise ValueError("cls_head_ce_fwd: W %s [C,2H], logits f32 [M,C]" % dt)
+    for n, t in (("labels", labels), ("mask", mask)):
+        _dev(t, n)
+        if t.dtype != torch.int64 or t.numel() != M or not t.is_contiguous():
+            raise ValueError("cls_head_ce_fwd: %s must be contiguous int64 with one entry per row" % n)
+    if rowstat.dtype != F32 or rowstat.numel() < 2 * M or counter.dtype != torch.int32 or stats.dtype != F32 or stats.numel() < 3:
+        raise ValueError("cls_head_ce_fwd: rowstat f32 [2M], counter int32 [1], stats f32 [3]")
+    check(_lib.load().icka_cls_head_ce_fwd(seq.data_ptr(), gated.data_ptr(), W.data_ptr(), int(dt == F16), _ptr(bias),
+                                           logits.data_ptr(), labels.data_ptr(), mask.data_ptr(), rowstat.data_ptr(),
+                                           counter.data_ptr(), stats.data_ptr(), M, H, Cn, _stream()), "icka_cls_head_ce_fwd")
+    return logits
+
+
+def cls_head_ce_bwd(logits, labels, mask, stats, dloss, seq, gated, gate, cross, W, dseq, du, dcross, partials):
+    M, H = seq.shape
+    Cn = W.shape[0]
+    for n, t in (("seq", seq), ("gated", gated), ("gate", gate), ("cross", cross), ("dseq", dseq), ("du", du),
+                 ("dcross", dcross)):
+        _mat(t, n)
+        if not t.is_contiguous() or tuple(t.shape) != (M, H):
+            raise ValueError("%s must be contiguous bf16 [M,H]" % n)
+    if logits.dtype != F32 or tuple(logits.shape) != (M, Cn) or not logits.is_contiguous() or dloss.dtype != F32:
+        raise ValueError("cls_head_ce_bwd: logits contiguous f32 [M,C], dloss f32")
+    lib = _lib.load()
+    check(lib.icka_cls_head_ce_bwd(logits.data_ptr(), labels.data_ptr(), mask.data_ptr(), stats.data_ptr(), dloss.data_ptr(),
+                                   seq.data_ptr(), gated.data_ptr(), gate.data_ptr(), cross.data_ptr(), W.data_ptr(),
+                                   dseq.data_ptr(), du.data_ptr(), dcross.data_ptr(), partials.data_ptr(), M, H, Cn,
+                                   _stream()), "icka_cls_head_ce_bwd")
+    return lib.icka_cls_head_bwd_slabs(M)
+
+
 def gemm_grouped(descs, reductions=None) -> None:
     reductions = reductions or []
     if not descs and not reductions:
@@ -921,6 +960,41 @@
     return out
 
 
+def additive_mask2(mask0: torch.Tensor, T0: int, out0: torch.Tensor, mask1: torch.Tensor, T1: int, out1: torch.Tensor):
+    for m in (mask0, mask1):
+        _dev(m, "mask")
+        if m.dtype != torch.int64 or m.stride(1) != 1:
+            raise TypeError("mask must be int64 row-major")
+    if mask0.shape[0] != mask1.shape[0]:
+        raise ValueError("additive_mask2: the two masks must have the same number of rows")
+    check(_lib.load().icka_additive_mask2(mask0.data_ptr(), mask0.stride(0), out0.data_ptr(), T0, mask1.data_ptr(),
+                                          mask1.stride(0), out1.data_ptr(), T1, mask0.shape[0], _stream()), "icka_additive_mask2")
+    return out0, out1
+
+
+def dropout_cast(x, y, src, dst, *, p_drop=0.0, seed=0):
+    _mat(x, "x"); _mat(y, "y")
+    _dev(src, "src"); _dev(dst, "dst")
+    if not (x.is_contiguous() and y.is_contiguous() and src.is_contiguous() and dst.is_contiguous()):
+        raise ValueError("dropout_cast: contiguous operands")
+    if src.dtype != F32 or dst.dtype != BF16 or dst.numel() < src.numel():
+        raise TypeError("dropout_cast: src f32, dst bf16 with room for it")
+    M, H = x.shape
+    check(_lib.load().icka_dropout_cast(x.data_ptr(), y.data_ptr(), M, H, p_drop, seed, src.data_ptr(), dst.data_ptr(),
+                                        src.numel(), _stream()), "icka_dropout_cast")
+    return y
+
+
+def add_dropout(a, b, y, *, p_drop=0.0, seed=0):
+    _mat(a, "a"); _mat(b, "b"); _mat(y, "y")
+    if not (a.is_contiguous() and b.is_contiguous() and y.is_contiguous()) or a.shape != b.shape or a.shape != y.shape:
+        raise ValueError("add_dropout: contiguous operands of one shape")
+    M, H = a.shape
+    check(_lib.load().icka_add_dropout(a.data_ptr(), b.data_ptr(), y.data_ptr(), M, H, p_drop, seed, _stream()),
+          "icka_add_dropout")
+    return y
+
+
 def dropout(x, y, *, y2=None, p_drop=0.0, seed=0):
     _mat(x, "x"); _mat(y, "y")
     M, H = x.shape
diff --git a/icka_amd/modeling.py b/icka_amd/modeling.py
--- a/icka_amd/modeling.py
+++ b/icka_amd/modeling.py
@@ -537,14 +537,15 @@
         self.pooler = BertPooler(config)
         self.apply(self.init_bert_weights)
 
-    def encode(self, input_ids, token_type_ids=None, attention_mask=None, output_all_encoded_layers=True):
+    def encode(self, input_ids, token_type_ids=None, attention_mask=None, output_all_encoded_layers=True, add_mask=None):
         if not input_ids.is_cuda:
             raise TypeError("input_ids must be on a ROCm device: icka_amd has no CPU path")
         B, S = input_ids.shape
         self._arena()
-        add_mask = torch.zeros(B, S, dtype=F32, device=input_ids.device) if attention_mask is None else \
-            K.additive_mask(attention_mask.long() if attention_mask.dtype != torch.int64 else attention_mask, S,
-                            torch.empty(B, S, dtype=F32, device=input_ids.device))
+        if add_mask is None:
+            add_mask = torch.zeros(B, S, dtype=F32, device=input_ids.device) if attention_mask is None else \
+                K.additive_mask(attention_mask.long() if attention_mask.dtype != torch.int64 else attention_mask, S,
+                                torch.empty(B, S, dtype=F32, device=input_ids.device))
         extended_attention_mask = add_mask.view(B, 1, 1, S)
         embedding_output = self.embeddings(input_ids, token_type_ids)
         return self.encoder(embedding_output, extended_attention_mask, output_all_encoded_layers=output_all_encoded_layers)
@@ -593,11 +594,20 @@
     A = self._arena()
     dev = input_ids.device
     pooled = None
+    img_mask = None
     if plan is not None:
         seq, seqf, pooled = _packed_text_encoder(self, A, plan, input_ids, segment_ids, input_mask, pool)
         sequence_output = None
     elif isinstance(self.bert, BertModel):
-        sequence_output = self.bert.encode(input_ids, segment_ids, input_mask, output_all_encoded_layers=False)[-1]
+        text_mask = None
+        if ops.MERGE_MASKS and not _is_exact(self) and input_mask is not None and input_mask.shape == (B, S):
+            im = input_mask if input_mask.dtype == torch.int64 else input_mask.long()
+            am = added_attention_mask if added_attention_mask.dtype == torch.int64 else added_attention_mask.long()
+            Rm = _region_layout(visual_embeds_att)[0]
+            text_mask, img_mask = K.additive_mask2(im, S, torch.empty(B, S, dtype=F32, device=dev),
+                                                   am, Rm, torch.empty(B, Rm, dtype=F32, device=dev))
+        sequence_output = self.bert.encode(input_ids, segment_ids, input_mask, output_all_encoded_layers=False,
+                                           add_mask=text_mask)[-1]
         if pool:
             seqf = _twin(sequence_output)
             if not _is_exact(self) and torch.is_grad_enabled() and sequence_output.requires_grad:
@@ -617,31 +627,44 @@
     if plan is None:
         seq = sequence_output.view(B * S, H)
         seqf = _twin(sequence_output)
-    if self.training and cfg.hidden_dropout_prob > 0:
+    v = visual_embeds_att
+    R, layout = _region_layout(v)
+    mixed = _is_mixed(self)
+    fan_out = torch.is_grad_enabled() and seq.requires_grad
+    drop = self.training and cfg.hidden_dropout_prob > 0
+    seq_drop = drop and fan_out and ops.FUSE_SEQ_DROPOUT and seq.is_contiguous()
+    if drop and not seq_drop:
         seq = ops.DropoutFn.apply(seq, A, float(cfg.hidden_dropout_prob))
         seqf = None
-    v = visual_embeds_att
-    R, layout = _region_layout(v)
     rows_p = (B * R + 127) // 128 * 128
     tokens = torch.empty(rows_p, 2048, dtype=BF16, device=dev)
     K.zero_rows_(tokens, B * R)
     vsrc = v.float().contiguous() if v.dtype != F32 or not v.is_contiguous() else v
-    mixed = _is_mixed(self)
     vis16 = None
+    cross = None
+    if seq_drop:
+        if not mixed and layout == 0:
+            cross, seq = ops.SeqDropoutFn.apply(seq, A, float(cfg.hidden_dropout_prob), vsrc, tokens)
+        else:
+            cross, seq = ops.SeqDropoutFn.apply(seq, A, float(cfg.hidden_dropout_prob))
+        seqf = None
     if mixed:
         tokens16 = torch.empty(rows_p, 2048, dtype=torch.float16, device=dev)
         K.zero_rows_(tokens16, B * R)
         K.regions_to_tokens_h(vsrc, tokens, tokens16, B, R, 2048, layout)
         vis, vis16 = ops.LinearFn.apply(A.anchor, tokens, self.vismap2text, A, False, K.EPI_NONE, tokens16)
     else:
-        K.regions_to_tokens(vsrc, tokens, B, R, 2048, layout)
+        if not (seq_drop and layout == 0):
+            K.regions_to_tokens(vsrc, tokens, B, R, 2048, layout)
         vis = ops.LinearFn.apply(A.anchor, tokens, self.vismap2text, A, False, K.EPI_NONE)
-    img_mask = K.additive_mask(added_attention_mask if added_attention_mask.dtype == torch.int64
-                               else added_attention_mask.long(), R, torch.empty(B, R, dtype=F32, device=dev))
-    if torch.is_grad_enabled() and seq.requires_grad:
-        cross, seq = ops.FanOutFn.apply(seq, 2)
-    else:
-        cross = seq
+    if img_mask is None:
+        img_mask = K.additive_mask(added_attention_mask if added_attention_mask.dtype == torch.int64
+                                   else added_attention_mask.long(), R, torch.empty(B, R, dtype=F32, device=dev))
+    if cross is None:
+        if fan_out:
+            cross, seq = ops.FanOutFn.apply(seq, 2)
+        else:
+            cross = seq
     crossf = seqf
     for layer in self.txt2img_attention.layer:
         d = _dims(cfg, B, S, R, self.training, mixed=_is_mixed(layer))
@@ -714,7 +737,8 @@
     def logits(self, input_ids, segment_ids, input_mask, added_attention_mask, visual_embeds_att):
         return self._feats(input_ids, segment_ids, input_mask, added_attention_mask, visual_embeds_att)[0]
 
-    def _feats(self, input_ids, segment_ids, input_mask, added_attention_mask, visual_embeds_att, n_swap=0, pool=False):
+    def _feats(self, input_ids, segment_ids, input_mask, added_attention_mask, visual_embeds_att, n_swap=0, pool=False,
+               ce_labels=None):
         cfg = self.config
         B, S = input_ids.shape
         H = cfg.hidden_size
@@ -760,10 +784,13 @@
             d16 = _dims(cfg, B, S, 0, self.training, mixed=True)
             seq16 = ops._fwd_twin(A, seq, seqf, d16)
             cross16 = ops._fwd_twin(A, cross, crossf, d16)
+        if ce_labels is not None and plan is None and ops.head_ce_ok(self, seq, ce_labels, input_mask):
+            loss, logits = ops.GatedHeadCEFn.apply(A.anchor, seq, cross, self, A, ce_labels, input_mask, seq16, cross16)
+            return logits.view(B, S, self.num_labels), crs, pooled, loss
         logits = ops.GatedHeadFn.apply(A.anchor, seq, cross, self, A, seq16, cross16)
         if plan is not None:
             logits = packing.RowsGatherFn.apply(logits, plan.pad2pack, 1, B * S, plan.p2p, 1, packing.F32_NAN_WORD)
-        return logits.view(B, S, self.num_labels), crs, pooled
+        return (logits.view(B, S, self.num_labels), crs, pooled) + ((None,) if ce_labels is not None else ())
 
     def forward(self, input_ids, segment_ids=None, input_mask=None, added_attention_mask=None, visual_embeds_mean=None,
                 visual_embeds_att=None, temp=None, temp_lamb=None, lamb=None, labels=None, negative_rate=None, *,
@@ -793,6 +820,10 @@
         if labels is not None and self.aux_losses:
             return self._objective(input_ids, segment_ids, input_mask, added_attention_mask, visual_embeds_mean,
                                    visual_embeds_att, temp, temp_lamb, lamb, labels, negative_rate)
+        if labels is not None and self.crf is None and not _is_exact(self):
+            logits, _, _, loss = self._feats(input_ids, segment_ids, input_mask, added_attention_mask, visual_embeds_att,
+                                             ce_labels=labels)
+            return loss if loss is not None else token_ce_loss(logits, labels, input_mask)
         logits = self.logits(input_ids, segment_ids, input_mask, added_attention_mask, visual_embeds_att)
         if labels is None:
             if self.crf is not None:
diff --git a/icka_amd/ops.py b/icka_amd/ops.py
--- a/icka_amd/ops.py
+++ b/icka_amd/ops.py
@@ -14,6 +14,10 @@
 FUSE_DENSE_LN_MIN_ROWS = 3072
 FUSE_QKV_ATTN = _os.environ.get("ICKA_FUSE_QKV_ATTN", "1") != "0"
 FUSE_QKV_ATTN_MIN_ROWS = 3072
+FUSE_HEAD_CE = _os.environ.get("ICKA_FUSE_HEAD_CE", "1") != "0"
+FUSE_SEQ_DROPOUT = _os.environ.get("ICKA_FUSE_SEQ_DROPOUT", "1") != "0"
+MERGE_MASKS = _os.environ.get("ICKA_MERGE_MASKS", "1") != "0"
+HEAD_CE_MAX_ROWS = 65536
 
 
 def _keepbits_on(Sq: int, Skv: int) -> bool:
@@ -597,10 +601,95 @@
         return dx, None, None
 
 
+def _head_ce_ws(A: ParamArena, M: int):
+    ctr = A._ws.get("cls_head_ce_counter")
+    if ctr is None:
+        ctr = A._ws["cls_head_ce_counter"] = torch.zeros(16, dtype=torch.int32, device=A.device)
+    return A.workspace("cls_head_ce", K._lib.load().icka_cls_head_ce_workspace_floats(M)), ctr
+
+
+class SeqDropoutFn(torch.autograd.Function):
+
+    @staticmethod
+    def forward(ctx, x, A: ParamArena, p: float, cast_src=None, cast_dst=None):
+        ctx.set_materialize_grads(False)
+        seed = A.next_seed()
+        y = torch.empty_like(x)
+        if cast_src is not None:
+            K.dropout_cast(x, y, cast_src, cast_dst, p_drop=p, seed=seed)
+        else:
+            K.dropout(x, y, p_drop=p, seed=seed)
+        ctx.p, ctx.seed = p, seed
+        return y.view_as(y), y.view_as(y)
+
+    @staticmethod
+    def backward(ctx, g0, g1):
+        if g0 is None and g1 is None:
+            return None, None, None, None, None
+        if g0 is None or g1 is None:
+            dy = _c(g1 if g0 is None else g0)
+            return K.dropout(dy, torch.empty_like(dy), p_drop=ctx.p, seed=ctx.seed), None, None, None, None
+        g0, g1 = _c(g0), _c(g1)
+        return K.add_dropout(g0, g1, torch.empty_like(g0), p_drop=ctx.p, seed=ctx.seed), None, None, None, None
+
+
+def head_ce_ok(head, seq, labels, mask) -> bool:
+    M, H = seq.shape
+    C = head.classifier.weight.shape[0]
+    return (FUSE_HEAD_CE and C <= 16 and H % 8 == 0 and 2 * H // 8 <= 256 and C * 2 * H * 2 <= 44 * 1024 and
+            M <= HEAD_CE_MAX_ROWS and labels.dtype == torch.int64 and mask.dtype == torch.int64 and labels.is_cuda and
+            mask.is_cuda and labels.numel() == M and mask.numel() == M)
+
+
+class GatedHeadCEFn(torch.autograd.Function):
+
+    @staticmethod
+    def forward(ctx, anchor, seq, cross, head, A: ParamArena, labels, mask, seq16=None, cross16=None):
+        ctx.set_materialize_grads(False)
+        labels = labels.reshape(-1).contiguous()
+        mask = mask.reshape(-1).contiguous()
+        stats = torch.empty(3, dtype=F32, device=seq.device)
+        logits = GatedHeadFn._forward(ctx, seq, cross, head, A, seq16, cross16, (labels, mask, stats))
+        ctx.save_for_backward(*ctx.__dict__.pop("saved_head"), logits, labels, mask, stats)
+        ctx.mark_non_differentiable(logits)
+        return stats[2:3].view(()), logits
+
+    @staticmethod
+    def backward(ctx, dloss, _dlogits):
+        seq, cross, gate, gated, logits, labels, mask, stats = ctx.saved_tensors
+        head, A = ctx.head, ctx.A
+        M, H = seq.shape
+        C = logits.shape[1]
+        if dloss is None:
+            return (None,) * 9
+        g = dloss.reshape(1)
+        if g.dtype != F32:
+            raise TypeError("loss gradient must be f32")
+        lib = K._lib.load()
+        cls = head.classifier
+        nslab, sf = lib.icka_cls_head_bwd_slabs(M), lib.icka_cls_head_slab_floats(H, C)
+        ws = A.workspace("cls_head", nslab * sf)
+        dseq_c = torch.empty(M, H, dtype=BF16, device=seq.device)
+        du = torch.empty_like(dseq_c)
+        dcross_d = torch.empty_like(dseq_c)
+        K.cls_head_ce_bwd(logits, labels, mask, stats, g, seq, gated, gate, cross, A.w(cls.weight), dseq_c, du, dcross_d, ws)
+        A.pending_reductions.append(K.slab_reduction(ws, nslab, C * 2 * H, (A.g(cls.weight).view(-1),),
+                                                     A.grad_beta(cls.weight) > 0, slab_stride=sf))
+        A.pending_reductions.append(K.slab_reduction(ws, nslab, C, (A.g(cls.bias),), A.grad_beta(cls.bias) > 0,
+                                                     slab_stride=sf, offset=C * 2 * H))
+        return GatedHeadFn._gate_tail(A, head, seq, cross, du, dseq_c, dcross_d) + (None, None)
+
+
 class GatedHeadFn(torch.autograd.Function):
 
     @staticmethod
     def forward(ctx, anchor, seq, cross, head, A: ParamArena, seq16=None, cross16=None):
+        logits = GatedHeadFn._forward(ctx, seq, cross, head, A, seq16, cross16, None)
+        ctx.save_for_backward(*ctx.__dict__.pop("saved_head"))
+        return logits
+
+    @staticmethod
+    def _forward(ctx, seq, cross, head, A, seq16, cross16, ce):
         M, H = seq.shape
         C = head.classifier.weight.shape[0]
         gate = torch.empty(M, H, dtype=BF16, device=seq.device)
@@ -617,7 +706,9 @@
                    bias=head.Gate_text.bias, bias2=head.Gate_image.bias, epilogue=K.EPI_GATE, aux=cross16, out2=gate,
                    out3=gated)
             Wc = A.w16(head.classifier.weight)
-            if ctx.skinny:
+            if ce is not None:
+                K.cls_head_ce_fwd(seq16, gated16, Wc, head.classifier.bias, logits, ce[0], ce[1], *_head_ce_ws(A, M), ce[2])
+            elif ctx.skinny:
                 K.cls_head_fwd(seq16, gated16, Wc, head.classifier.bias, logits)
             else:
                 K.gemm(K.GEMM_NT, seq16, Wc[:, :H], logits, A2=gated16, B2=Wc[:, H:], bias=head.classifier.bias)
@@ -625,12 +716,14 @@
             K.gemm(K.GEMM_NT, seq, A.w(head.Gate_text.weight), gated, A2=cross, B2=A.w(head.Gate_image.weight),
                    bias=head.Gate_text.bias, bias2=head.Gate_image.bias, epilogue=K.EPI_GATE, aux=cross, out2=gate)
             Wc = A.w(head.classifier.weight)
-            if ctx.skinny:
+            if ce is not None:
+                K.cls_head_ce_fwd(seq, gated, Wc, head.classifier.bias, logits, ce[0], ce[1], *_head_ce_ws(A, M), ce[2])
+            elif ctx.skinny:
                 K.cls_head_fwd(seq, gated, Wc, head.classifier.bias, logits)
             else:
                 K.gemm(K.GEMM_NT, seq, Wc[:, :H], logits, A2=gated, B2=Wc[:, H:], bias=head.classifier.bias)
         ctx.head, ctx.A = head, A
-        ctx.save_for_backward(seq, cross, gate, gated)
+        ctx.saved_head = (seq, cross, gate, gated)
         return logits
 
     @staticmethod
diff --git a/include/icka_hip.h b/include/icka_hip.h
--- a/include/icka_hip.h
+++ b/include/icka_hip.h
@@ -163,6 +163,11 @@
 int icka_cast_pad_f32_to_bf16(const float* src, int64_t lds, void* dst, int64_t ldd, int32_t M, int32_t N,
                               void* stream);
 int icka_additive_mask(const int64_t* mask, int64_t ld, float* out, int32_t B, int32_t T, void* stream);
+int icka_additive_mask2(const int64_t* mask0, int64_t ld0, float* out0, int32_t T0, const int64_t* mask1, int64_t ld1,
+                        float* out1, int32_t T1, int32_t B, void* stream);
+int icka_dropout_cast(const void* x, void* y, int32_t M, int32_t H, float p_drop, uint64_t seed, const float* src, void* dst,
+                      int64_t n, void* stream);
+int icka_add_dropout(const void* a, const void* b, void* y, int32_t M, int32_t H, float p_drop, uint64_t seed, void* stream);
 int icka_dropout(const void* x, int64_t ldx, void* y, int64_t ldy, void* y2, int64_t ldy2, int32_t M, int32_t H,
                  float p_drop, uint64_t seed, void* stream);
 int icka_regions_to_tokens(const float* src, void* dst, int32_t B, int32_t R, int32_t C, int32_t layout,
@@ -184,6 +189,14 @@
                       int32_t H, int32_t C, void* stream);
 int32_t icka_cls_head_bwd_slabs(int32_t M);
 int64_t icka_cls_head_slab_floats(int32_t H, int32_t C);
+int64_t icka_cls_head_ce_workspace_floats(int32_t M);
+int icka_cls_head_ce_fwd(const void* seq, const void* gated, const void* W, int32_t is_f16, const float* bias, float* logits,
+                         const int64_t* labels, const int64_t* mask, float* rowstat, uint32_t* counter, float* stats,
+                         int32_t M, int32_t H, int32_t C, void* stream);
+int icka_cls_head_ce_bwd(const float* logits, const int64_t* labels, const int64_t* mask, const float* stats,
+                         const float* dloss, const void* seq, const void* gated, const void* gate, const void* cross,
+                         const void* W, void* dseq, void* du, void* dcross, float* partials, int32_t M, int32_t H, int32_t C,
+                         void* stream);
 int icka_sample_gate_fwd(const void* a, int64_t lda, const void* c, int64_t ldc, const float* gate, int32_t mode,
                          void* out, int64_t ldo, int32_t B, int32_t S, int32_t H, void* stream);
 int icka_sample_gate_fwd_h(const void* a16, int64_t lda, const float* gate, int32_t mode, void* out, void* out16, int64_t ldo,
```
